# lukasino1214/soc_real_time_renderer

Hardware: AMD Instinct MI355X
Metric: frames/sec + ms/pass, Sponza 3840x2160 deferred+SSAO+TAA (higher is better)
Workload: dtype f32 (fp16/unorm8/d32 storage)

## Files before the change

### soc_real_time_renderer_amd/csrc/bloom.hip

```cpp
#include <cstdlib>
#include <type_traits>

#include "bloom_common.hpp"

namespace soc {

namespace {

__global__ __launch_bounds__(kWorkgroup) void bloom_down_generic(DImg src, DImg dst, float sxt, float syt) {
    const int x = blockIdx.x * BX + threadIdx.x, y = blockIdx.y * BY + threadIdx.y;
    if (x >= dst.w || y >= dst.h) return;
    const float u = centre_uv(x, dst.w), v = centre_uv(y, dst.h);
    const float X = sxt, Y = syt;
    auto S = [&](float uu, float vv) {
        return tap(src, axis_from_fixed(fixed_from_uv(uu, src.w), src.w), axis_from_fixed(fixed_from_uv(vv, src.h), src.h));
    };
    f3 a = S(u - 2 * X, v + 2 * Y), b = S(u, v + 2 * Y), c = S(u + 2 * X, v + 2 * Y);
    f3 d = S(u - 2 * X, v), e = S(u, v), f = S(u + 2 * X, v);
    f3 g = S(u - 2 * X, v - 2 * Y), h = S(u, v - 2 * Y), i = S(u + 2 * X, v - 2 * Y);
    f3 j = S(u - X, v + Y), k = S(u + X, v + Y), l = S(u - X, v - Y), m = S(u + X, v - Y);
    store_rgb1(dst, x, y, SOC_DOWN13(a, b, c, d, e, f, g, h, i, j, k, l, m));
}

__global__ __launch_bounds__(kWorkgroup) void bloom_up_generic(DImg src, DImg dst, float X, float Y) {
    const int x = blockIdx.x * BX + threadIdx.x, y = blockIdx.y * BY + threadIdx.y;
    if (x >= dst.w || y >= dst.h) return;
    const float u = centre_uv(x, dst.w), v = centre_uv(y, dst.h);
    auto S = [&](float uu, float vv) {
        return tap(src, axis_from_fixed(fixed_from_uv(uu, src.w), src.w), axis_from_fixed(fixed_from_uv(vv, src.h), src.h));
    };
    f3 a = S(u - X, v + Y), b = S(u, v + Y), c = S(u + X, v + Y);
    f3 d = S(u - X, v), e = S(u, v), f = S(u + X, v);
    f3 g = S(u - X, v - Y), h = S(u, v - Y), i = S(u + X, v - Y);
    store_rgb1(dst, x, y, SOC_UP9(a, b, c, d, e, f, g, h, i));
}

__global__ __launch_bounds__(kWorkgroup) void bloom_up_double(DImg src, DImg dst) {
    const int x = blockIdx.x * BX + threadIdx.x, y = blockIdx.y * BY + threadIdx.y;
    if (x >= dst.w || y >= dst.h) return;
    auto AX = [&](int k) { return axis_from_fixed(128 * x - 64 + 256 * k, src.w); };
    auto AY = [&](int k) { return axis_from_fixed(128 * y - 64 + 256 * k, src.h); };
    const Axis xm = AX(-1), x0 = AX(0), xp = AX(1), ym = AY(-1), y0 = AY(0), yp = AY(1);
    f3 a = tap(src, xm, yp), b = tap(src, x0, yp), c = tap(src, xp, yp);
    f3 d = tap(src, xm, y0), e = tap(src, x0, y0), f = tap(src, xp, y0);
    f3 g = tap(src, xm, ym), h = tap(src, x0, ym), i = tap(src, xp, ym);
    store_rgb1(dst, x, y, SOC_UP9(a, b, c, d, e, f, g, h, i));
}

__global__ __launch_bounds__(kWorkgroup) void bloom_down_same_q(DImg src, DImg dst, bool vec) {
    const int m = blockIdx.x * BX + threadIdx.x, n = blockIdx.y * BY + threadIdx.y;
    const int X0 = 2 * m, Y0 = 2 * n;
    if (X0 >= dst.w || Y0 >= dst.h) return;
    uint2 T[6][6];
#pragma unroll
    for (int r = 0; r < 6; ++r)
#pragma unroll
        for (int c = 0; c < 6; ++c) T[r][c] = texel_clamped(src, X0 - 2 + c, Y0 - 2 + r);
    float out[2][2][3];
    auto run = [&](auto CH) {
        constexpr int C = decltype(CH)::value;
        float V[6][6];
#pragma unroll
        for (int r = 0; r < 6; ++r)
#pragma unroll
            for (int c = 0; c < 6; ++c) V[r][c] = chan<C>(T[r][c]);
#pragma unroll
        for (int py = 0; py < 2; ++py)
#pragma unroll
            for (int px = 0; px < 2; ++px) {
                auto P = [&](int ox, int oy) { return V[oy + 2 + py][ox + 2 + px]; };
                out[py][px][C] = down13(P(-2, 2), P(0, 2), P(2, 2), P(-2, 0), P(0, 0), P(2, 0), P(-2, -2), P(0, -2),
                                        P(2, -2), P(-1, 1), P(1, 1), P(-1, -1), P(1, -1));
            }
    };
    run(std::integral_constant<int, 0>{});
    run(std::integral_constant<int, 1>{});
    run(std::integral_constant<int, 2>{});
    store_quad_row(dst, X0, Y0, out[0], vec);
    store_quad_row(dst, X0, Y0 + 1, out[1], vec);
}

__global__ __launch_bounds__(kWorkgroup) void bloom_up_same_q(DImg src, DImg dst, bool vec) {
    const int m = blockIdx.x * BX + threadIdx.x, n = blockIdx.y * BY + threadIdx.y;
    const int X0 = 2 * m, Y0 = 2 * n;
    if (X0 >= dst.w || Y0 >= dst.h) return;
    uint2 T[4][4];
#pragma unroll
    for (int r = 0; r < 4; ++r)
#pragma unroll
        for (int c = 0; c < 4; ++c) T[r][c] = texel_clamped(src, X0 - 1 + c, Y0 - 1 + r);
    float out[2][2][3];
    auto run = [&](auto CH) {
        constexpr int C = decltype(CH)::value;
#pragma unroll
        for (int py = 0; py < 2; ++py)
#pragma unroll
            for (int px = 0; px < 2; ++px) {
                auto P = [&](int ox, int oy) { return chan<C>(T[oy + 1 + py][ox + 1 + px]); };
                out[py][px][C] = up9(P(-1, 1), P(0, 1), P(1, 1), P(-1, 0), P(0, 0), P(1, 0), P(-1, -1), P(0, -1), P(1, -1));
            }
    };
    run(std::integral_constant<int, 0>{});
    run(std::integral_constant<int, 1>{});
    run(std::integral_constant<int, 2>{});
    store_quad_row(dst, X0, Y0, out[0], vec);
    store_quad_row(dst, X0, Y0 + 1, out[1], vec);
}

__global__ __launch_bounds__(kWorkgroup) void bloom_down_half_w(DImg src, DImg dst) {
    const int x = blockIdx.x * BX + threadIdx.x, y = blockIdx.y * BY + threadIdx.y;
    if (x >= dst.w || y >= dst.h) return;
    const bool interior = 2 * x - 2 >= 0 && 2 * x + 3 <= src.w - 1 && 2 * y - 2 >= 0 && 2 * y + 3 <= src.h - 1;
    if (!interior) {
        auto AX = [&](int k) { return axis_from_fixed(256 * (2 * x + k) + 128, src.w); };
        auto AY = [&](int k) { return axis_from_fixed(256 * (2 * y + k) + 128, src.h); };
        const Axis xm2 = AX(-2), xm1 = AX(-1), x0 = AX(0), xp1 = AX(1), xp2 = AX(2);
        const Axis ym2 = AY(-2), ym1 = AY(-1), y0 = AY(0), yp1 = AY(1), yp2 = AY(2);
        f3 a = tap(src, xm2, yp2), b = tap(src, x0, yp2), c = tap(src, xp2, yp2);
        f3 d = tap(src, xm2, y0), e = tap(src, x0, y0), f = tap(src, xp2, y0);
        f3 g = tap(src, xm2, ym2), h = tap(src, x0, ym2), i = tap(src, xp2, ym2);
        f3 j = tap(src, xm1, yp1), k = tap(src, xp1, yp1), l = tap(src, xm1, ym1), m = tap(src, xp1, ym1);
        store_rgb1(dst, x, y, SOC_DOWN13(a, b, c, d, e, f, g, h, i, j, k, l, m));
        return;
    }
    uint2 T[6][6];
    const uint2* base = row_ptr<uint2>(src, 2 * y - 2) + (2 * x - 2);
    const int pitch8 = src.pitch / 8;
#pragma unroll
    for (int r = 0; r < 6; ++r)
#pragma unroll
        for (int c = 0; c < 6; ++c) T[r][c] = base[r * pitch8 + c];
    float out[3];
    auto run = [&](auto CH) {
        constexpr int C = decltype(CH)::value;
        float Hl[6][5];
#pragma unroll
        for (int r = 0; r < 6; ++r)
#pragma unroll
            for (int k = 0; k < 5; ++k) Hl[r][k] = lerp_c(chan<C>(T[r][k]), chan<C>(T[r][k + 1]), 0.5f);
        auto S = [&](int kx, int ky) { return lerp_c(Hl[ky + 2][kx + 2], Hl[ky + 3][kx + 2], 0.5f); };
        out[C] = down13(S(-2, 2), S(0, 2), S(2, 2), S(-2, 0), S(0, 0), S(2, 0), S(-2, -2), S(0, -2), S(2, -2), S(-1, 1),
                        S(1, 1), S(-1, -1), S(1, -1));
    };
    run(std::integral_constant<int, 0>{});
    run(std::integral_constant<int, 1>{});
    run(std::integral_constant<int, 2>{});
    store_rgb1_c(dst, x, y, out[0], out[1], out[2]);
}

__global__ __launch_bounds__(kWorkgroup) void bloom_up_double_q(DImg src, DImg dst, bool vec) {
    const int m = blockIdx.x * BX + threadIdx.x, n = blockIdx.y * BY + threadIdx.y;
    if (m >= src.w || n >= src.h) return;
    const int X0 = 2 * m, Y0 = 2 * n;
    const bool interior = m - 2 >= 0 && m + 2 <= src.w - 1 && n - 2 >= 0 && n + 2 <= src.h - 1;
    if (!interior) {
#pragma unroll 1
        for (int k = 0; k < 4; ++k) {
                const int px = k & 1, py = k >> 1;
                const int x = X0 + px, y = Y0 + py;
                auto AX = [&](int k) { return axis_from_fixed(128 * x - 64 + 256 * k, src.w); };
                auto AY = [&](int k) { return axis_from_fixed(128 * y - 64 + 256 * k, src.h); };
                const Axis xm = AX(-1), x0 = AX(0), xp = AX(1), ym = AY(-1), y0 = AY(0), yp = AY(1);
                f3 a = tap(src, xm, yp), b = tap(src, x0, yp), c = tap(src, xp, yp);
                f3 d = tap(src, xm, y0), e = tap(src, x0, y0), f = tap(src, xp, y0);
                f3 g = tap(src, xm, ym), h = tap(src, x0, ym), i = tap(src, xp, ym);
                store_rgb1(dst, x, y, SOC_UP9(a, b, c, d, e, f, g, h, i));
            }
        return;
    }
    uint2 T[5][5];
    const uint2* base = row_ptr<uint2>(src, n - 2) + (m - 2);
    const int pitch8 = src.pitch / 8;
#pragma unroll
    for (int r = 0; r < 5; ++r)
#pragma unroll
        for (int c = 0; c < 5; ++c) T[r][c] = base[r * pitch8 + c];
    float out[2][2][3];
    auto run = [&](auto CH) {
        constexpr int C = decltype(CH)::value;
        float V[5][5];
#pragma unroll
        for (int r = 0; r < 5; ++r)
#pragma unroll
            for (int c = 0; c < 5; ++c) V[r][c] = chan<C>(T[r][c]);
        float H0[5][3], H1[5][3];
#pragma unroll
        for (int r = 0; r < 5; ++r)
#pragma unroll
            for (int k = 0; k < 3; ++k) {
                H0[r][k] = t_w34(V[r][k], V[r][k + 1]);
                H1[r][k] = t_w14(V[r][k + 1], V[r][k + 2]);
            }
#pragma unroll
        for (int px = 0; px < 2; ++px) {
            const float (&Hl)[5][3] = px ? H1 : H0;
            float S0[3][3], S1[3][3];
#pragma unroll
            for (int ky = -1; ky <= 1; ++ky)
#pragma unroll
                for (int kx = -1; kx <= 1; ++kx) {
                    const float p = v_prod(Hl[ky + 2][kx + 1]);
                    S0[ky + 1][kx + 1] = __builtin_fmaf(Hl[ky + 1][kx + 1], 0.0625f, p);
                    S1[ky + 1][kx + 1] = __builtin_fmaf(Hl[ky + 3][kx + 1], 0.0625f, p);
                }
            out[0][px][C] = up9(S0[2][0], S0[2][1], S0[2][2], S0[1][0], S0[1][1], S0[1][2], S0[0][0], S0[0][1], S0[0][2]);
            out[1][px][C] = up9(S1[2][0], S1[2][1], S1[2][2], S1[1][0], S1[1][1], S1[1][2], S1[0][0], S1[0][1], S1[0][2]);
        }
        __builtin_amdgcn_sched_barrier(0);
    };
    run(std::integral_constant<int, 0>{});
    run(std::integral_constant<int, 1>{});
    run(std::integral_constant<int, 2>{});
    store_quad_row(dst, X0, Y0, out[0], vec);
    store_quad_row(dst, X0, Y0 + 1, out[1], vec);
}

constexpr int kFastMax = 8192;

long quad_min_px() {
    static const long v = [] {
        const char* e = getenv("SOC_BLOOM_QUAD_MIN_PX");
        return e ? atol(e) : 1L << 20;
    }();
    return v;
}

bool vec16(const soc_img& im) { return im.pitch_bytes % 16 == 0 && reinterpret_cast<uintptr_t>(im.data) % 16 == 0; }

}

int launch_bloom_down(const soc_img& hi, const soc_img& lo, hipStream_t s, int force_generic) {
    dim3 blk(BX, BY), grd(ceil_div(lo.width, BX), ceil_div(lo.height, BY));
    DImg src = dimg(hi), dst = dimg(lo);
    const bool small = hi.width <= kFastMax && hi.height <= kFastMax;
    if (!force_generic && small && hi.width == lo.width && hi.height == lo.height) {
        dim3 g2(ceil_div(ceil_div(lo.width, 2), BX), ceil_div(ceil_div(lo.height, 2), BY));
        launch("bloom_down_same_q", kWorkgroup, bloom_down_same_q, g2, blk, 0, s, src, dst, vec16(lo));
    } else if (!force_generic && small && hi.width == 2 * lo.width && hi.height == 2 * lo.height) {
        launch("bloom_down_half_w", kWorkgroup, bloom_down_half_w, grd, blk, 0, s, src, dst);
    } else {
        launch("bloom_down_generic", kWorkgroup, bloom_down_generic, grd, blk, 0, s, src, dst, 1.0f / (float)hi.width, 1.0f / (float)hi.height);
    }
    return check_launch("bloom_downsample");
}

int launch_bloom_up(const soc_img& lo, const soc_img& hi, hipStream_t s, int force_generic) {
    dim3 blk(BX, BY), grd(ceil_div(hi.width, BX), ceil_div(hi.height, BY));
    DImg src = dimg(lo), dst = dimg(hi);
    const bool small = hi.width <= kFastMax && hi.height <= kFastMax;
    if (!force_generic && small && hi.width == lo.width && hi.height == lo.height) {
        dim3 g2(ceil_div(ceil_div(hi.width, 2), BX), ceil_div(ceil_div(hi.height, 2), BY));
        launch("bloom_up_same_q", kWorkgroup, bloom_up_same_q, g2, blk, 0, s, src, dst, vec16(hi));
    } else if (!force_generic && small && hi.width == 2 * lo.width && hi.height == 2 * lo.height) {
        if ((long)hi.width * hi.height < quad_min_px()) {
            launch("bloom_up_double", kWorkgroup, bloom_up_double, grd, blk, 0, s, src, dst);
        } else {
            dim3 g2(ceil_div(lo.width, BX), ceil_div(lo.height, BY));
            launch("bloom_up_double_q", kWorkgroup, bloom_up_double_q, g2, blk, 0, s, src, dst, vec16(hi));
        }
    } else {
        launch("bloom_up_generic", kWorkgroup, bloom_up_generic, grd, blk, 0, s, src, dst, 1.0f / (float)lo.width, 1.0f / (float)lo.height);
    }
    return check_launch("bloom_upsample");
}

}

using namespace soc;

static int bloom_args(const soc_img& a, const soc_img& b, const char* pass) {
    int rc = check_img(a, SOC_FMT_RGBA16F, pass, "source");
    if (rc) return rc;
    rc = check_img(b, SOC_FMT_RGBA16F, pass, "target");
    if (rc) return rc;
    if (a.data == b.data) return set_error(SOC_E_INVALID_ARG, "%s: source and target alias", pass);
    return SOC_OK;
}

extern "C" int soc_bloom_downsample(const soc_globals* g, soc_img higher_mip, soc_img lower_mip, soc_stream stream) {
    (void)g;
    int rc = bloom_args(higher_mip, lower_mip, "soc_bloom_downsample");
    if (rc) return rc;
    return launch_bloom_down(higher_mip, lower_mip, hs(stream), 0);
}

extern "C" int soc_bloom_upsample(const soc_globals* g, soc_img lower_mip, soc_img higher_mip, soc_stream stream) {
    (void)g;
    int rc = bloom_args(lower_mip, higher_mip, "soc_bloom_upsample");
    if (rc) return rc;
    return launch_bloom_up(lower_mip, higher_mip, hs(stream), 0);
}

extern "C" int soc_debug_bloom_generic(int32_t up, soc_img a, soc_img b, soc_stream stream) {
    int rc = bloom_args(a, b, "soc_debug_bloom_generic");
    if (rc) return rc;
    return up ? launch_bloom_up(a, b, hs(stream), 1) : launch_bloom_down(a, b, hs(stream), 1);
}

extern "C" int soc_bloom_weighted_stage(const soc_globals* g, soc_img emissive, const soc_img* mips, int32_t mip_count,
                                        soc_img output, int32_t stage, soc_stream stream) {
    (void)g;
    static const char* P = "soc_bloom_weighted_stage";
    if (!mips) return set_error(SOC_E_INVALID_ARG, "%s: null mips", P);
    if (stage < 0 || stage > 4) return set_error(SOC_E_INVALID_ARG, "%s: stage %d not in 0..4", P, stage);
    int rc = check_img(emissive, SOC_FMT_RGBA16F, P, "emissive");
    if (!rc) rc = check_img(output, SOC_FMT_RGBA16F, P, "output");
    for (int i = 0; !rc && i < mip_count; ++i) rc = check_img(mips[i], SOC_FMT_RGBA16F, P, "mip");
    if (rc) return rc;
    if (!bloom_fused_applicable(emissive, mips, mip_count, output))
        return set_error(SOC_E_UNSUPPORTED, "%s: needs 4 mips halving exactly from the emissive extent (<= 8192)", P);
    if ((stage == 0 || stage == 4) && output.data == mips[1].data)
        return set_error(SOC_E_INVALID_ARG, "%s: output aliases mip 1", P);
    return launch_bloom_weighted(emissive, mips, output, hs(stream), stage);
}

extern "C" int soc_bloom_chain(const soc_globals* g, soc_img emissive, const soc_img* mips, int32_t mip_count,
                               soc_stream stream) {
    if (!mips || mip_count < 1) return set_error(SOC_E_INVALID_ARG, "soc_bloom_chain: need >= 1 mip");
    int rc = soc_bloom_downsample(g, emissive, mips[0], stream);
    for (int i = 0; !rc && i < mip_count - 1; ++i) rc = soc_bloom_downsample(g, mips[i], mips[i + 1], stream);
    for (int i = mip_count - 1; !rc && i > 0; --i) rc = soc_bloom_upsample(g, mips[i], mips[i - 1], stream);
    if (!rc) rc = soc_bloom_upsample(g, mips[0], emissive, stream);
    return rc;
}
```

### soc_real_time_renderer_amd/csrc/bloom_w.hip

```cpp
#include "bloom_w.hpp"

namespace soc {
bool bloom_fused_applicable(const soc_img& emissive, const soc_img* mips, int mip_count, const soc_img& output) {
    if (mip_count != 4 || output.width != emissive.width || output.height != emissive.height) return false;
    if (emissive.width > 8192 || emissive.height > 8192) return false;
    if (mips[0].width != emissive.width || mips[0].height != emissive.height) return false;
    for (int i = 1; i < 4; ++i)
        if (mips[i - 1].width != 2 * mips[i].width || mips[i - 1].height != 2 * mips[i].height || mips[i].width < 2 ||
            mips[i].height < 2)
            return false;
    return true;
}
}

namespace soc {
namespace {

__device__ __forceinline__ void store2(const DImg& im, int x, int y, uint2 a, uint2 b, bool vec) {
    uint2* row = row_ptr_w<uint2>(im, y);
    if (vec && x + 1 < im.w) {
        *reinterpret_cast<uint4*>(row + x) = uint4{a.x, a.y, b.x, b.y};
        return;
    }
    row[x] = a;
    if (x + 1 < im.w) row[x + 1] = b;
}

template <int TW>
__device__ __forceinline__ C3 down11(const uint2 (*t)[TW], int cx, int cy) {
    C3 a{0.0f, 0.0f, 0.0f};
    madd(a, t[cy][cx], 0.125f);
    madd(a, t[cy - 2][cx - 2], 0.03125f);
    madd(a, t[cy - 2][cx + 2], 0.03125f);
    madd(a, t[cy + 2][cx - 2], 0.03125f);
    madd(a, t[cy + 2][cx + 2], 0.03125f);
    madd(a, t[cy - 2][cx], 0.0625f);
    madd(a, t[cy][cx - 2], 0.0625f);
    madd(a, t[cy][cx + 2], 0.0625f);
    madd(a, t[cy + 2][cx], 0.0625f);
    madd(a, t[cy - 1][cx - 1], 0.125f);
    madd(a, t[cy - 1][cx + 1], 0.125f);
    madd(a, t[cy + 1][cx - 1], 0.125f);
    madd(a, t[cy + 1][cx + 1], 0.125f);
    return a;
}

__device__ __forceinline__ constexpr float d21_w(int i, int j) {
    constexpr int A[6] = {1, 1, 2, 2, 1, 1}, B[6] = {0, 1, 1, 1, 1, 0};
    return (float)(A[i] * A[j] + 4 * B[i] * B[j]) * (1.0f / 128.0f);
}
template <int TW>
__device__ __forceinline__ C3 down21(const uint2 (*t)[TW], int c0, int r0) {
    C3 a{0.0f, 0.0f, 0.0f};
#pragma unroll
    for (int j = 0; j < 6; ++j)
#pragma unroll
        for (int i = 0; i < 6; ++i) madd(a, t[r0 + j][c0 + i], d21_w(i, j));
    return a;
}

template <int TW>
__device__ __forceinline__ void up12_pair(const uint2 (*t)[TW], int c0, int r0, int py, C3& even, C3& odd) {
    even = C3{0.0f, 0.0f, 0.0f};
    odd = C3{0.0f, 0.0f, 0.0f};
#pragma unroll
    for (int j = 0; j < 4; ++j) {
        const float wy = u12_w(py, j);
#pragma unroll
        for (int i = 0; i < 5; ++i) {
            const uint2 v = t[r0 + j][c0 + i];
            if (i < 4) madd(even, v, u12_w(0, i) * wy);
            if (i > 0) madd(odd, v, u12_w(1, i - 1) * wy);
        }
    }
}

template <int TW>
__device__ __forceinline__ void up11_pair(const uint2 (*t)[TW], int cx, int cy, C3& a, C3& b) {
    a = C3{0.0f, 0.0f, 0.0f};
    b = C3{0.0f, 0.0f, 0.0f};
    constexpr float w[3] = {1.0f, 2.0f, 1.0f};
#pragma unroll
    for (int j = 0; j < 3; ++j)
#pragma unroll
        for (int i = 0; i < 4; ++i) {
            const uint2 v = t[cy - 1 + j][cx - 1 + i];
            if (i < 3) madd(a, v, w[i] * w[j] * (1.0f / 16.0f));
            if (i > 0) madd(b, v, w[i - 1] * w[j] * (1.0f / 16.0f));
        }
}

template <int MODE>
struct W1 {
    static constexpr int OW = MODE ? 30 : 32, OH = MODE == 2 ? 16 : 8;
    static constexpr int MW = 2 * OW + 4, MH = 2 * OH + 4;
    static constexpr int EW = MW + 4, EH = MH + 4;
    static constexpr int RUN = MH / 4;
    static_assert(!MODE || (MW == 64 && MH % 4 == 0), "down11_runs: 64 columns x 2 row parities x 2 runs");
};

template <int TW, int MW, int RUN>
__device__ __forceinline__ void down11_runs(const uint2 (*t)[TW], uint2 (*mt)[MW], int c, int r, int cx) {
    uint2 e0[3], o1[2], e2[3], o3[2], e4[3];
    const int cy0 = r + 2;
    auto even = [&](int y, uint2 (&e)[3]) { e[0] = t[y][cx - 2]; e[1] = t[y][cx]; e[2] = t[y][cx + 2]; };
    auto odd = [&](int y, uint2 (&o)[2]) { o[0] = t[y][cx - 1]; o[1] = t[y][cx + 1]; };
    even(cy0 - 2, e0);
    odd(cy0 - 1, o1);
    even(cy0, e2);
    odd(cy0 + 1, o3);
    even(cy0 + 2, e4);
#pragma unroll
    for (int j = 0; j < RUN; ++j) {
        C3 a{0.0f, 0.0f, 0.0f};
        madd(a, e2[1], 0.125f);
        madd(a, e0[0], 0.03125f);
        madd(a, e0[2], 0.03125f);
        madd(a, e4[0], 0.03125f);
        madd(a, e4[2], 0.03125f);
        madd(a, e0[1], 0.0625f);
        madd(a, e2[0], 0.0625f);
        madd(a, e2[2], 0.0625f);
        madd(a, e4[1], 0.0625f);
        madd(a, o1[0], 0.125f);
        madd(a, o1[1], 0.125f);
        madd(a, o3[0], 0.125f);
        madd(a, o3[1], 0.125f);
        mt[r + 2 * j][c] = pack3(a);
        if (j < RUN - 1) {
#pragma unroll
            for (int k = 0; k < 3; ++k) {
                e0[k] = e2[k];
                e2[k] = e4[k];
            }
            o1[0] = o3[0];
            o1[1] = o3[1];
            const int cy = cy0 + 2 * (j + 1);
            odd(cy + 1, o3);
            even(cy + 2, e4);
        }
    }
}

template <int TW>
__device__ __forceinline__ void down21_vpair(const uint2 (*t)[TW], int c0, int r0, C3& a, C3& b) {
    a = C3{0.0f, 0.0f, 0.0f};
    b = C3{0.0f, 0.0f, 0.0f};
#pragma unroll
    for (int j = 0; j < 8; ++j) {
        uint2 v[6];
#pragma unroll
        for (int i = 0; i < 6; ++i) v[i] = t[r0 + j][c0 + i];
#pragma unroll
        for (int i = 0; i < 6; ++i) {
            if (j < 6) madd(a, v[i], d21_w(i, j));
            if (j >= 2) madd(b, v[i], d21_w(i, j - 2));
        }
        asm volatile("" : "+v"(a.r), "+v"(a.g), "+v"(a.b), "+v"(b.r), "+v"(b.g), "+v"(b.b)::"memory");
    }
}

template <int MODE, bool ZS>
__global__ __launch_bounds__(kWorkgroup) void bloomw_down01p(DImg E, DImg M1, int ntx, int nty) {
    constexpr int W1_OW = W1<MODE>::OW, W1_OH = W1<MODE>::OH, W1_MW = W1<MODE>::MW, W1_MH = W1<MODE>::MH,
                  W1_EW = W1<MODE>::EW, W1_EH = W1<MODE>::EH, RUN = W1<MODE>::RUN;
    static_assert(kWorkgroup == 256, "four waves: one vote word each");
    __shared__ uint2 et[W1_EH][W1_EW];
    __shared__ uint2 mt[W1_MH][W1_MW];
    __shared__ uint4 zv[2];
    constexpr int NT = W1_EW * W1_EH, KR = (NT + 255) / 256;
    const int tid = threadIdx.x, n = ntx * nty, G = (int)gridDim.x;
    int er[KR], ec[KR];
#pragma unroll
    for (int k = 0; k < KR; ++k) {
        const int i = tid + 256 * k;
        er[k] = i / W1_EW;
        ec[k] = i - er[k] * W1_EW;
    }
    auto tile_origin = [&](int t, int& X0, int& Y0) {
        const int q = n >> 3, r = n & 7, k = t & 7;
        const int id = k * q + min(k, r) + (t >> 3);
        const int ty = id / ntx;
        X0 = (id - ty * ntx) * W1_OW;
        Y0 = ty * W1_OH;
    };
    uint2 v[KR];
    auto fetch = [&](int t) {
        int X0, Y0;
        tile_origin(t, X0, Y0);
        const int ex0 = 2 * X0 - 4, ey0 = 2 * Y0 - 4;
#pragma unroll
        for (int k = 0; k < KR; ++k)
            if (tid + 256 * k < NT)
                v[k] = row_ptr<uint2>(E, clampi(ey0 + er[k], 0, E.h - 1))[clampi(ex0 + ec[k], 0, E.w - 1)];
    };
    auto vote = [&](int slot) {
        uint32_t nz = 0u;
#pragma unroll
        for (int k = 0; k < KR; ++k)
            if (tid + 256 * k < NT) nz |= v[k].x | (v[k].y & 0xffffu);
        const bool any = __ballot(nz != 0u) != 0ull;
        if ((tid & 63) == 0) reinterpret_cast<uint32_t*>(&zv[slot])[tid >> 6] = any ? 1u : 0u;
    };
    auto voted = [&](int slot) {
        const uint4 z = zv[slot];
        return __builtin_amdgcn_readfirstlane((int)(z.x | z.y | z.z | z.w)) == 0;
    };
    int t = (int)blockIdx.x;
    int slot = 0;
    const uint2 zpx = pack3(C3{0.0f, 0.0f, 0.0f});
    if (t < n) fetch(t);
    for (; t < n; t += G) {
#pragma unroll
        for (int k = 0; k < KR; ++k)
            if (tid + 256 * k < NT) et[er[k]][ec[k]] = v[k];
        if constexpr (ZS) vote(slot);
        __syncthreads();
        if (t + G < n) fetch(t + G);
        int X0, Y0;
        tile_origin(t, X0, Y0);
        if constexpr (ZS) {
            const bool zero = voted(slot);
            slot ^= 1;
            if (zero) {
                if constexpr (MODE == 2) {
                    if (tid < W1_OW * W1_OH / 2) {
                        const int q = tid / W1_OW, ox = tid - q * W1_OW;
                        const int X = X0 + ox, Y = Y0 + 2 * q;
                        if (X < M1.w && Y < M1.h) row_ptr_w<uint2>(M1, Y)[X] = zpx;
                        if (X < M1.w && Y + 1 < M1.h) row_ptr_w<uint2>(M1, Y + 1)[X] = zpx;
                    }
                } else {
                    const int oy = tid / W1_OW, ox = tid - oy * W1_OW;
                    const int X = X0 + ox, Y = Y0 + oy;
                    if (oy < W1_OH && X < M1.w && Y < M1.h) row_ptr_w<uint2>(M1, Y)[X] = zpx;
                }
                continue;
            }
        }
        const int mx0 = 2 * X0 - 2, my0 = 2 * Y0 - 2, ex0 = mx0 - 2, ey0 = my0 - 2;
        if (MODE && my0 >= 0 && my0 + W1_MH <= E.h) {
            const int c = tid & 63, par = (tid >> 6) & 1, half = tid >> 7;
            if constexpr (MODE != 0)
                down11_runs<W1_EW, W1_MW, RUN>(et, mt, c, par + 2 * RUN * half, clampi(mx0 + c, 0, E.w - 1) - ex0);
        } else
        for (int i = tid; i < W1_MW * W1_MH; i += 256) {
            const int r = i / W1_MW, c = i - r * W1_MW;
            const int cx = clampi(mx0 + c, 0, E.w - 1) - ex0, cy = clampi(my0 + r, 0, E.h - 1) - ey0;
            mt[r][c] = pack3(down11<W1_EW>(et, cx, cy));
        }
        __syncthreads();
        if constexpr (MODE == 2) {
            if (tid < W1_OW * W1_OH / 2) {
                const int q = tid / W1_OW, ox = tid - q * W1_OW;
                const int X = X0 + ox, Y = Y0 + 2 * q;
                C3 a, b;
                down21_vpair<W1_MW>(mt, 2 * ox, 4 * q, a, b);
                if (X < M1.w && Y < M1.h) row_ptr_w<uint2>(M1, Y)[X] = pack3(a);
                if (X < M1.w && Y + 1 < M1.h) row_ptr_w<uint2>(M1, Y + 1)[X] = pack3(b);
            }
        } else {
            const int oy = tid / W1_OW, ox = tid - oy * W1_OW;
            const int X = X0 + ox, Y = Y0 + oy;
            if (oy < W1_OH && X < M1.w && Y < M1.h) row_ptr_w<uint2>(M1, Y)[X] = pack3(down21<W1_MW>(mt, 2 * ox, 2 * oy));
        }
        __syncthreads();
    }
}

constexpr int W2_OW = 16, W2_OH = 8;
constexpr int W2_MW = 2 * W2_OW + 4, W2_MH = 2 * W2_OH + 4;
constexpr int W2_SW = 2 * W2_MW + 4, W2_SH = 2 * W2_MH + 4;

template <int TW, int MW, int K>
__device__ __forceinline__ void down21_runs(const uint2 (*t)[TW], uint2 (*mt)[MW], int c, int r0, int n, int sc) {
    C3 acc[K];
#pragma unroll
    for (int e = 0; e < K; ++e) acc[e] = C3{0.0f, 0.0f, 0.0f};
#pragma unroll
    for (int R = 0; R < 6 + 2 * (K - 1); ++R) {
        if (R >= 6 + 2 * (n - 1)) continue;
        uint2 v[6];
#pragma unroll
        for (int i = 0; i < 6; ++i) v[i] = t[2 * r0 + R][sc + i];
#pragma unroll
        for (int e = 0; e < K; ++e) {
            const int j = R - 2 * e;
            if (j >= 0 && j < 6) {
#pragma unroll
                for (int i = 0; i < 6; ++i) madd(acc[e], v[i], d21_w(i, j));
            }
        }
#pragma unroll
        for (int e = 0; e < K; ++e) asm volatile("" : "+v"(acc[e].r), "+v"(acc[e].g), "+v"(acc[e].b)::"memory");
    }
#pragma unroll
    for (int e = 0; e < K; ++e)
        if (e < n) mt[r0 + e][c] = pack3(acc[e]);
}

template <bool REG>
__global__ __launch_bounds__(kWorkgroup) void bloomw_down23(DImg S1, DImg M3, int W2, int H2, int swz) {
    __shared__ uint2 st[W2_SH][W2_SW];
    __shared__ uint2 mt[W2_MH][W2_MW];
    const int tid = threadIdx.x;
    int tbx, tby;
    xcd_order(swz, tbx, tby);
    const int X0 = tbx * W2_OW, Y0 = tby * W2_OH;
    const int mx0 = 2 * X0 - 2, my0 = 2 * Y0 - 2, sx0 = 2 * mx0 - 2, sy0 = 2 * my0 - 2;
    load_tile<W2_SW, W2_SH>(S1, sx0, sy0, st, tid);
    __syncthreads();
    constexpr int K = 3, NR = (W2_MH + K - 1) / K;
    static_assert(W2_MW * NR <= 256, "one run per lane");
    if (REG && my0 >= 0 && my0 + W2_MH <= H2) {
        if (tid < W2_MW * NR) {
            const int c = tid % W2_MW, k = tid / W2_MW, r0 = k * K;
            const int qx = clampi(mx0 + c, 0, W2 - 1);
            down21_runs<W2_SW, W2_MW, K>(st, mt, c, r0, min(K, W2_MH - r0), 2 * qx - 2 - sx0);
        }
    } else
    for (int i = tid; i < W2_MW * W2_MH; i += 256) {
        const int r = i / W2_MW, c = i - r * W2_MW;
        const int qx = clampi(mx0 + c, 0, W2 - 1), qy = clampi(my0 + r, 0, H2 - 1);
        mt[r][c] = pack3(down21<W2_SW>(st, 2 * qx - 2 - sx0, 2 * qy - 2 - sy0));
    }
    __syncthreads();
    if (tid < W2_OW * W2_OH) {
        const int ox = tid % W2_OW, oy = tid / W2_OW;
        const int X = X0 + ox, Y = Y0 + oy;
        if (X < M3.w && Y < M3.h) row_ptr_w<uint2>(M3, Y)[X] = pack3(down21<W2_MW>(mt, 2 * ox, 2 * oy));
    }
}

constexpr int U_OW = 64, U_OH = 16;
constexpr int W3_MW = U_OW / 2 + 4, W3_MH = U_OH / 2 + 4;
constexpr int W3_SW = W3_MW / 2 + 4, W3_SH = W3_MH / 2 + 4;

template <int SW, int MW>
__device__ __forceinline__ void up12_into(const uint2 (*s)[SW], int sx0, int sy0, uint2 (*m)[MW], int c, int r, int qx, int qy,
                                          int Wq, int Hq) {
    const int cy = clampi(qy, 0, Hq - 1), py = cy & 1;
    const int q0 = clampi(qx, 0, Wq - 1), q1 = clampi(qx + 1, 0, Wq - 1);
    const int r0 = (cy >> 1) - 2 + py - sy0;
    if ((q0 & 1) == 0 && q1 == q0 + 1) {
        C3 e, o;
        up12_pair<SW>(s, (q0 >> 1) - 2 - sx0, r0, py, e, o);
        m[r][c] = pack3(e);
        m[r][c + 1] = pack3(o);
    } else {
#pragma unroll
        for (int k = 0; k < 2; ++k) {
            const int q = k ? q1 : q0;
            C3 e, o;
            up12_pair<SW>(s, ((q & ~1) >> 1) - 2 - sx0, r0, py, e, o);
            m[r][c + k] = pack3((q & 1) ? o : e);
        }
    }
}

__global__ __launch_bounds__(kWorkgroup) void bloomw_up32(DImg S3, DImg M1, int W2, int H2, bool vec, int swz) {
    __shared__ uint2 st[W3_SH][W3_SW];
    __shared__ uint2 mt[W3_MH][W3_MW];
    const int tid = threadIdx.x;
    int tbx, tby;
    xcd_order(swz, tbx, tby);
    const int X0 = tbx * U_OW, Y0 = tby * U_OH;
    const int mx0 = X0 / 2 - 2, my0 = Y0 / 2 - 2;
    const int sx0 = mx0 / 2 - 2, sy0 = my0 / 2 - 2;
    load_tile<W3_SW, W3_SH>(S3, sx0, sy0, st, tid);
    __syncthreads();
    for (int i = tid; i < (W3_MW / 2) * W3_MH; i += 256) {
        const int r = i / (W3_MW / 2), c = 2 * (i - r * (W3_MW / 2));
        up12_into<W3_SW, W3_MW>(st, sx0, sy0, mt, c, r, mx0 + c, my0 + r, W2, H2);
    }
    __syncthreads();
    for (int i = tid; i < (U_OW / 2) * U_OH; i += 256) {
        const int r = i / (U_OW / 2), pc = i - r * (U_OW / 2);
        const int x = X0 + 2 * pc, y = Y0 + r;
        if (x >= M1.w || y >= M1.h) continue;
        const int py = y & 1;
        C3 e, o;
        up12_pair<W3_MW>(mt, (x >> 1) - 2 - mx0, (y >> 1) - 2 + py - my0, py, e, o);
        store2(M1, x, y, pack3(e), pack3(o), vec);
    }
}

struct P3u {
    float r[W3_MH][U_OW], g[W3_MH][U_OW], b[W3_MH][U_OW];
};
template <bool RUNS>
__global__ __launch_bounds__(kWorkgroup) void bloomw_up32s(DImg S3, DImg M1, int W2, int H2, bool vec, int swz) {
    __shared__ uint2 st[W3_SH][W3_SW];
    __shared__ uint2 mt[W3_MH][W3_MW];
    __shared__ P3u hp;
    const int tid = threadIdx.x;
    int tbx, tby;
    xcd_order(swz, tbx, tby);
    const int X0 = tbx * U_OW, Y0 = tby * U_OH;
    const int mx0 = X0 / 2 - 2, my0 = Y0 / 2 - 2;
    const int sx0 = mx0 / 2 - 2, sy0 = my0 / 2 - 2;
    load_tile<W3_SW, W3_SH>(S3, sx0, sy0, st, tid);
    __syncthreads();
    for (int i = tid; i < W3_SH * W3_MW; i += 256) {
        const int sr = i / W3_MW, c = i - sr * W3_MW;
        const int q = clampi(mx0 + c, 0, W2 - 1), px = q & 1, c0 = (q >> 1) - 2 + px - sx0;
        C3 a{0.0f, 0.0f, 0.0f};
#pragma unroll
        for (int k = 0; k < 4; ++k) madd(a, st[sr][c0 + k], u12_w(px, k));
        hp.r[sr][c] = a.r;
        hp.g[sr][c] = a.g;
        hp.b[sr][c] = a.b;
    }
    __syncthreads();
    for (int i = tid; i < W3_MH * W3_MW; i += 256) {
        const int r = i / W3_MW, c = i - r * W3_MW;
        const int cy = clampi(my0 + r, 0, H2 - 1), py = cy & 1, r0 = (cy >> 1) - 2 + py - sy0;
        C3 a{0.0f, 0.0f, 0.0f};
#pragma unroll
        for (int k = 0; k < 4; ++k) {
            const float w = u12_w(py, k);
            a.r = __builtin_fmaf(hp.r[r0 + k][c], w, a.r);
            a.g = __builtin_fmaf(hp.g[r0 + k][c], w, a.g);
            a.b = __builtin_fmaf(hp.b[r0 + k][c], w, a.b);
        }
        mt[r][c] = pack3(a);
    }
    __syncthreads();
    for (int i = tid; i < W3_MH * U_OW; i += 256) {
        const int r = i / U_OW, ox = i - r * U_OW;
        const int x = X0 + ox, px = x & 1, c0 = (x >> 1) - 2 + px - mx0;
        C3 a{0.0f, 0.0f, 0.0f};
#pragma unroll
        for (int k = 0; k < 4; ++k) madd(a, mt[r][c0 + k], u12_w(px, k));
        hp.r[r][ox] = a.r;
        hp.g[r][ox] = a.g;
        hp.b[r][ox] = a.b;
    }
    __syncthreads();
    if constexpr (RUNS) {
        static_assert(U_OW == 64 && U_OH == 16, "64 columns x 4 runs of 4 output rows");
        const int ox = tid & 63, m = tid >> 6, x = X0 + ox;
        float hr[6], hg[6], hb[6];
#pragma unroll
        for (int k = 0; k < 6; ++k) {
            hr[k] = hp.r[2 * m + k][ox];
            hg[k] = hp.g[2 * m + k][ox];
            hb[k] = hp.b[2 * m + k][ox];
        }
#pragma unroll
        for (int i = 0; i < 4; ++i) {
            const int y = Y0 + 4 * m + i, py = i & 1, rr = (i >> 1) + (i & 1);
            C3 a{0.0f, 0.0f, 0.0f};
#pragma unroll
            for (int j = 0; j < 4; ++j) {
                const float w = u12_w(py, j);
                a.r = __builtin_fmaf(hr[rr + j], w, a.r);
                a.g = __builtin_fmaf(hg[rr + j], w, a.g);
                a.b = __builtin_fmaf(hb[rr + j], w, a.b);
            }
            if (x < M1.w && y < M1.h) row_ptr_w<uint2>(M1, y)[x] = pack3(a);
        }
        return;
    }
    for (int i = tid; i < (U_OW / 2) * U_OH; i += 256) {
        const int r = i / (U_OW / 2), pc = i - r * (U_OW / 2);
        const int x = X0 + 2 * pc, y = Y0 + r;
        if (x >= M1.w || y >= M1.h) continue;
        const int py = y & 1, r0 = (y >> 1) - 2 + py - my0;
        C3 o[2];
#pragma unroll
        for (int k = 0; k < 2; ++k) {
            const int c = 2 * pc + k;
            C3 a{0.0f, 0.0f, 0.0f};
#pragma unroll
            for (int j = 0; j < 4; ++j) {
                const float w = u12_w(py, j);
                a.r = __builtin_fmaf(hp.r[r0 + j][c], w, a.r);
                a.g = __builtin_fmaf(hp.g[r0 + j][c], w, a.g);
                a.b = __builtin_fmaf(hp.b[r0 + j][c], w, a.b);
            }
            o[k] = a;
        }
        store2(M1, x, y, pack3(o[0]), pack3(o[1]), vec);
    }
}

constexpr int W4_MW = U_OW + 2, W4_MH = U_OH + 2;
constexpr int W4_SW = U_OW / 2 + 6, W4_SH = U_OH / 2 + 6;

__global__ __launch_bounds__(kWorkgroup) void bloomw_up10(DImg S1, DImg O, bool vec, int swz) {
    __shared__ uint2 st[W4_SH][W4_SW];
    __shared__ uint2 mt[W4_MH][W4_MW + 2];
    const int tid = threadIdx.x;
    int tbx, tby;
    xcd_order(swz, tbx, tby);
    const int X0 = tbx * U_OW, Y0 = tby * U_OH;
    const int mx0 = X0 - 1, my0 = Y0 - 1;
    const int sx0 = X0 / 2 - 3, sy0 = Y0 / 2 - 3;
    const int W0 = O.w, H0 = O.h;
    load_tile<W4_SW, W4_SH>(S1, sx0, sy0, st, tid);
    __syncthreads();
    for (int i = tid; i < (W4_MW / 2) * W4_MH; i += 256) {
        const int r = i / (W4_MW / 2), k = i - r * (W4_MW / 2);
        const int c = 2 * k + 1;
        up12_into<W4_SW, W4_MW + 2>(st, sx0, sy0, mt, c, r, mx0 + c, my0 + r, W0, H0);
    }
    for (int r = tid; r < W4_MH; r += 256) {
        const int cy = clampi(my0 + r, 0, H0 - 1), py = cy & 1;
        const int q = clampi(mx0, 0, W0 - 1);
        C3 e, o;
        up12_pair<W4_SW>(st, ((q & ~1) >> 1) - 2 - sx0, (cy >> 1) - 2 + py - sy0, py, e, o);
        mt[r][0] = pack3((q & 1) ? o : e);
    }
    __syncthreads();
    for (int i = tid; i < (U_OW / 2) * U_OH; i += 256) {
        const int r = i / (U_OW / 2), pc = i - r * (U_OW / 2);
        const int x = X0 + 2 * pc, y = Y0 + r;
        if (x >= O.w || y >= O.h) continue;
        C3 a, b;
        up11_pair<W4_MW + 2>(mt, x - mx0, y - my0, a, b);
        store2(O, x, y, pack3(a), pack3(b), vec);
    }
}

__global__ __launch_bounds__(kWorkgroup) void bloomw_up10s(DImg S1, DImg O, bool vec, int swz, bool zs) {
    __shared__ Up10Tile<U_OW, U_OH> t;
    const int tid = threadIdx.x;
    int tbx, tby;
    xcd_order(swz, tbx, tby);
    const int X0 = tbx * U_OW, Y0 = tby * U_OH;
    const bool zero = t.build(S1, X0, Y0, O.w, O.h, tid, zs);
    const uint2 zpx = pack3(C3{0.0f, 0.0f, 0.0f});
    for (int i = tid; i < (U_OW / 2) * U_OH; i += 256) {
        const int r = i / (U_OW / 2), pc = i - r * (U_OW / 2);
        const int x = X0 + 2 * pc, y = Y0 + r;
        if (x >= O.w || y >= O.h) continue;
        if (zero) {
            store2(O, x, y, zpx, zpx, vec);
            continue;
        }
        C3 o[2];
        t.out(r, 2 * pc, o);
        store2(O, x, y, pack3(o[0]), pack3(o[1]), vec);
    }
}

#ifndef SOC_BLOOM_UP10_ROWS
#define SOC_BLOOM_UP10_ROWS 16
#endif
constexpr int R_OW = 62, R_TH = SOC_BLOOM_UP10_ROWS;
__device__ __forceinline__ uint32_t up_from_left(uint32_t v) {
    return (uint32_t)__builtin_amdgcn_update_dpp(0, (int)v, 0x138, 0xf, 0xf, false);
}
__device__ __forceinline__ uint32_t up_from_right(uint32_t v) {
    return (uint32_t)__builtin_amdgcn_update_dpp(0, (int)v, 0x130, 0xf, 0xf, false);
}
template <bool ZS>
__global__ __launch_bounds__(kWorkgroup) void bloomw_up10r(DImg S1, DImg O, int nwx, int nwaves) {
    const int lane = (int)(threadIdx.x & 63);
    const int wid = (int)blockIdx.x * (kWorkgroup / 64) + (int)(threadIdx.x >> 6);
    if (wid >= nwaves) return;
    const int W0 = O.w, H0 = O.h, W1 = S1.w, H1 = S1.h;
    const int wx = wid % nwx, Y0 = (wid / nwx) * R_TH;
    const int x = wx * R_OW - 1 + lane;
    const int cx = clampi(x, 0, W0 - 1);
    const int px = cx & 1, c0 = (cx >> 1) - 2 + px;
    int tc[4];
    float wk[4];
#pragma unroll
    for (int k = 0; k < 4; ++k) {
        tc[k] = clampi(c0 + k, 0, W1 - 1);
        wk[k] = px ? u12_w(1, k) : u12_w(0, k);
    }
    auto taps = [&](int s, uint2 (&t)[4]) {
        const uint2* row = row_ptr<uint2>(S1, clampi(s, 0, H1 - 1));
#pragma unroll
        for (int k = 0; k < 4; ++k) t[k] = row[tc[k]];
    };
    auto h12 = [&](const uint2 (&t)[4]) {
        C3 a{0.0f, 0.0f, 0.0f};
#pragma unroll
        for (int k = 0; k < 4; ++k) madd(a, t[k], wk[k]);
        return a;
    };
    auto rgb_or = [&](const uint2 (&t)[4]) {
        return t[0].x | t[1].x | t[2].x | t[3].x | ((t[0].y | t[1].y | t[2].y | t[3].y) & 0xffffu);
    };
    C3 ring[5];
    uint2 pend[4];
    uint32_t nz = 0u;
    int base = (max(Y0 - 1, 0) >> 1) - 2;
#pragma unroll
    for (int i = 0; i < 5; ++i) {
        taps(base + i, pend);
        ring[i] = h12(pend);
        if constexpr (ZS) nz |= rgb_or(pend);
    }
    taps(base + 5, pend);
    auto hrow = [&](int cy) {
        const int jb = (cy >> 1) - 2;
        if (jb > base) {
#pragma unroll
            for (int i = 0; i < 4; ++i) ring[i] = ring[i + 1];
            ring[4] = h12(pend);
            base = jb;
            taps(base + 5, pend);
        }
        const int py = cy & 1;
        C3 a{0.0f, 0.0f, 0.0f};
#pragma unroll
        for (int k = 0; k < 4; ++k) {
            const float w = u12_w(py, k);
            const C3 h = py ? ring[k + 1] : ring[k];
            a.r = __builtin_fmaf(h.r, w, a.r);
            a.g = __builtin_fmaf(h.g, w, a.g);
            a.b = __builtin_fmaf(h.b, w, a.b);
        }
        const uint2 m = pack3(a);
        const uint2 l = uint2{up_from_left(m.x), up_from_left(m.y)}, r = uint2{up_from_right(m.x), up_from_right(m.y)};
        C3 hs{0.0f, 0.0f, 0.0f};
        madd(hs, l, 1.0f);
        madd(hs, m, 2.0f);
        madd(hs, r, 1.0f);
        return hs;
    };
    const bool out_lane = lane >= 1 && lane <= R_OW && x < W0;
    int y0 = Y0;
    if constexpr (ZS) {
        if (__ballot(nz != 0u) == 0ull) {
            const uint2 zpx = pack3(C3{0.0f, 0.0f, 0.0f});
            const int ns = min(Y0 + R_TH, H0) - Y0 + 2;
            int s = 0;
            for (; s < ns; ++s) {
                const int jb = (clampi(Y0 - 1 + s, 0, H0 - 1) >> 1) - 2;
                if (jb > base) {
                    if (__ballot(rgb_or(pend) != 0u) != 0ull) break;
                    base = jb;
                    taps(base + 5, pend);
                }
                if (s >= 2 && out_lane) row_ptr_w<uint2>(O, Y0 + s - 2)[x] = zpx;
            }
            y0 = Y0 + max(s - 2, 0);
        }
    }
    C3 hq0 = hrow(max(y0 - 1, 0)), hq1 = hrow(min(y0, H0 - 1));
    for (int y = y0; y < min(Y0 + R_TH, H0); ++y) {
        const C3 hq2 = hrow(min(y + 1, H0 - 1));
        C3 o;
        o.r = __builtin_fmaf(hq2.r, 1.0f / 16.0f, __builtin_fmaf(hq1.r, 2.0f / 16.0f, hq0.r * (1.0f / 16.0f)));
        o.g = __builtin_fmaf(hq2.g, 1.0f / 16.0f, __builtin_fmaf(hq1.g, 2.0f / 16.0f, hq0.g * (1.0f / 16.0f)));
        o.b = __builtin_fmaf(hq2.b, 1.0f / 16.0f, __builtin_fmaf(hq1.b, 2.0f / 16.0f, hq0.b * (1.0f / 16.0f)));
        if (out_lane) row_ptr_w<uint2>(O, y)[x] = pack3(o);
        hq0 = hq1;
        hq1 = hq2;
    }
}

template <int MODE, bool ZS>
int down01p_resident_set() {
    constexpr int kMaxDevices = 64;
    static int cached[kMaxDevices] = {};
    int dev = 0, cus = 256, per = 0;
    (void)hipGetDevice(&dev);
    if (dev >= 0 && dev < kMaxDevices && cached[dev]) return cached[dev];
    (void)hipDeviceGetAttribute(&cus, hipDeviceAttributeMultiprocessorCount, dev);
    (void)hipOccupancyMaxActiveBlocksPerMultiprocessor(&per, bloomw_down01p<MODE, ZS>, 256, 0);
    const int n = std::max(per, 1) * cus;
    if (dev >= 0 && dev < kMaxDevices) cached[dev] = n;
    return n;
}

bool a16(const soc_img& im) { return im.pitch_bytes % 16 == 0 && reinterpret_cast<uintptr_t>(im.data) % 16 == 0; }

}

int launch_bloom_weighted(const soc_img& emissive, const soc_img* mips, const soc_img& output, hipStream_t s, int stage) {
    const DImg E = dimg(emissive), M1 = dimg(mips[1]), M3 = dimg(mips[3]), O = dimg(output);
    const int swz = 1;
    const bool zero_skip = tuning_knob("SOC_BLOOM_ZERO_SKIP", 1) != 0;
    if (stage == 0 || stage == 1) {
        auto w1 = [&](auto mode, auto zs) {
            constexpr int R = decltype(mode)::value;
            constexpr bool Z = decltype(zs)::value;
            const int ntx = ceil_div(mips[1].width, W1<R>::OW), nty = ceil_div(mips[1].height, W1<R>::OH);
            const int grid = std::max(8, (std::min(ntx * nty, down01p_resident_set<R, Z>()) / 8) * 8);
            launch("bloomw_down01p", kWorkgroup, bloomw_down01p<R, Z>, grid, kWorkgroup, 0, s, E, M1, ntx, nty);
        };
        auto w1z = [&](auto mode) {
            if (zero_skip) w1(mode, std::true_type{});
            else w1(mode, std::false_type{});
        };
        const int mode = tuning_knob("SOC_BLOOM_W1_REG", 1);
        if (mode == 2) w1z(std::integral_constant<int, 2>{});
        else if (mode == 1) w1z(std::integral_constant<int, 1>{});
        else w1z(std::integral_constant<int, 0>{});
    }
    if (stage == 0 || stage == 2) {
        dim3 g(ceil_div(mips[3].width, W2_OW), ceil_div(mips[3].height, W2_OH));
        if (tuning_knob("SOC_BLOOM_W2_REG", 1))
            launch("bloomw_down23", kWorkgroup, bloomw_down23<true>, g, kWorkgroup, 0, s, M1, M3, mips[2].width, mips[2].height, swz);
        else
            launch("bloomw_down23", kWorkgroup, bloomw_down23<false>, g, kWorkgroup, 0, s, M1, M3, mips[2].width, mips[2].height, swz);
    }
    if (stage == 0 || stage == 3) {
        dim3 g(ceil_div(mips[1].width, U_OW), ceil_div(mips[1].height, U_OH));
        if (tuning_knob("SOC_BLOOM_UP_SEP", 1))
            if (tuning_knob("SOC_BLOOM_W3_RUNS", 1))
                launch("bloomw_up32s", kWorkgroup, bloomw_up32s<true>, g, kWorkgroup, 0, s, M3, M1, mips[2].width, mips[2].height, a16(mips[1]), swz);
            else
                launch("bloomw_up32s", kWorkgroup, bloomw_up32s<false>, g, kWorkgroup, 0, s, M3, M1, mips[2].width, mips[2].height, a16(mips[1]), swz);
        else
            launch("bloomw_up32", kWorkgroup, bloomw_up32, g, kWorkgroup, 0, s, M3, M1, mips[2].width, mips[2].height, a16(mips[1]), swz);
    }
    if (stage == 0 || stage == 4) {
        dim3 g(ceil_div(output.width, U_OW), ceil_div(output.height, U_OH));
        if (tuning_knob("SOC_BLOOM_UP10_REG", 1)) {
            const int nwx = ceil_div(output.width, R_OW), nwaves = nwx * ceil_div(output.height, R_TH);
            if (zero_skip)
                launch("bloomw_up10r", kWorkgroup, bloomw_up10r<true>, ceil_div(nwaves, kWorkgroup / 64), kWorkgroup, 0, s, M1, O, nwx, nwaves);
            else
                launch("bloomw_up10r", kWorkgroup, bloomw_up10r<false>, ceil_div(nwaves, kWorkgroup / 64), kWorkgroup, 0, s, M1, O, nwx, nwaves);
        } else if (tuning_knob("SOC_BLOOM_UP_SEP", 1))
            launch("bloomw_up10s", kWorkgroup, bloomw_up10s, g, kWorkgroup, 0, s, M1, O, a16(output), swz, zero_skip);
        else
            launch("bloomw_up10", kWorkgroup, bloomw_up10, g, kWorkgroup, 0, s, M1, O, a16(output), swz);
    }
    return check_launch("bloom_weighted");
}

}
```

### soc_real_time_renderer_amd/csrc/bloom_w.hpp

```cpp
#pragma once

#include "soc_internal.hpp"

namespace soc {
namespace {

__device__ __forceinline__ int clampi(int v, int lo, int hi) { return min(max(v, lo), hi); }

struct C3 {
    float r, g, b;
};
__device__ __forceinline__ float lo16(uint32_t u) { return (float)__builtin_bit_cast(_Float16, (uint16_t)(u & 0xffffu)); }
__device__ __forceinline__ float hi16(uint32_t u) { return (float)__builtin_bit_cast(_Float16, (uint16_t)(u >> 16)); }
__device__ __forceinline__ void madd(C3& a, uint2 t, float w) {
    a.r = __builtin_fmaf(lo16(t.x), w, a.r);
    a.g = __builtin_fmaf(hi16(t.x), w, a.g);
    a.b = __builtin_fmaf(lo16(t.y), w, a.b);
}
__device__ __forceinline__ uint2 pack3(const C3& c) { return pack_h4(f4{c.r, c.g, c.b, 1.0f}); }

template <int TW, int TH>
__device__ __forceinline__ uint32_t load_tile(const DImg& im, int ox, int oy, uint2 (*t)[TW], int tid) {
    constexpr int N = TW * TH;
    auto at = [&](int i) {
        const int r = i / TW, c = i - r * TW;
        return row_ptr<uint2>(im, clampi(oy + r, 0, im.h - 1)) + clampi(ox + c, 0, im.w - 1);
    };
    uint32_t nz = 0u;
    for (int i0 = tid; i0 < N; i0 += 4 * 256) {
        const int i1 = i0 + 256, i2 = i1 + 256, i3 = i2 + 256;
        const uint2 a = *at(i0);
        uint2 b = uint2{0u, 0u}, c = b, d = b;
        if (i1 < N) b = *at(i1);
        if (i2 < N) c = *at(i2);
        if (i3 < N) d = *at(i3);
        t[i0 / TW][i0 % TW] = a;
        if (i1 < N) t[i1 / TW][i1 % TW] = b;
        if (i2 < N) t[i2 / TW][i2 % TW] = c;
        if (i3 < N) t[i3 / TW][i3 % TW] = d;
        nz |= a.x | b.x | c.x | d.x | ((a.y | b.y | c.y | d.y) & 0xffffu);
    }
    return nz;
}

__device__ __forceinline__ constexpr float u12_w(int parity, int k) {
    constexpr int E[4] = {1, 5, 7, 3}, O[4] = {3, 7, 5, 1};
    return (float)(parity ? O[k] : E[k]) * (1.0f / 16.0f);
}

template <int OW, int OH>
struct Up10Tile {
    static constexpr int MW = OW + 2, MH = OH + 2;
    static constexpr int SW = OW / 2 + 6, SH = OH / 2 + 6;
    static constexpr int HR = SH > MH ? SH : MH;
    union {
        uint2 st[SH][SW];
        uint2 mt[MH][MW];
    };
    float hr[HR][MW], hg[HR][MW], hb[HR][MW];
    uint32_t zv[4];

    __device__ __forceinline__ bool build(const DImg& S1, int X0, int Y0, int W0, int H0, int tid, bool zs) {
        const int mx0 = X0 - 1, my0 = Y0 - 1;
        const int sx0 = X0 / 2 - 3, sy0 = Y0 / 2 - 3;
        const uint32_t nz = load_tile<SW, SH>(S1, sx0, sy0, st, tid);
        if (zs) {
            const bool any = __ballot(nz != 0u) != 0ull;
            if ((tid & 63) == 0) zv[tid >> 6] = any ? 1u : 0u;
        }
        __syncthreads();
        if (zs && __builtin_amdgcn_readfirstlane((int)(zv[0] | zv[1] | zv[2] | zv[3])) == 0) return true;
        for (int i = tid; i < SH * MW; i += 256) {
            const int sr = i / MW, c = i - sr * MW;
            const int q = clampi(mx0 + c, 0, W0 - 1), px = q & 1, c0 = (q >> 1) - 2 + px - sx0;
            C3 a{0.0f, 0.0f, 0.0f};
#pragma unroll
            for (int k = 0; k < 4; ++k) madd(a, st[sr][c0 + k], u12_w(px, k));
            hr[sr][c] = a.r;
            hg[sr][c] = a.g;
            hb[sr][c] = a.b;
        }
        __syncthreads();
        for (int i = tid; i < MH * MW; i += 256) {
            const int r = i / MW, c = i - r * MW;
            const int cy = clampi(my0 + r, 0, H0 - 1), py = cy & 1, r0 = (cy >> 1) - 2 + py - sy0;
            C3 a{0.0f, 0.0f, 0.0f};
#pragma unroll
            for (int k = 0; k < 4; ++k) {
                const float w = u12_w(py, k);
                a.r = __builtin_fmaf(hr[r0 + k][c], w, a.r);
                a.g = __builtin_fmaf(hg[r0 + k][c], w, a.g);
                a.b = __builtin_fmaf(hb[r0 + k][c], w, a.b);
            }
            mt[r][c] = pack3(a);
        }
        __syncthreads();
        for (int i = tid; i < MH * OW; i += 256) {
            const int r = i / OW, c = i - r * OW;
            C3 a{0.0f, 0.0f, 0.0f};
            madd(a, mt[r][c], 1.0f);
            madd(a, mt[r][c + 1], 2.0f);
            madd(a, mt[r][c + 2], 1.0f);
            hr[r][c] = a.r;
            hg[r][c] = a.g;
            hb[r][c] = a.b;
        }
        __syncthreads();
        return false;
    }
    __device__ __forceinline__ void out(int r, int c, C3 (&o)[2]) const {
#pragma unroll
        for (int k = 0; k < 2; ++k) {
            const int cc = c + k;
            o[k].r = __builtin_fmaf(hr[r + 2][cc], 1.0f / 16.0f, __builtin_fmaf(hr[r + 1][cc], 2.0f / 16.0f, hr[r][cc] * (1.0f / 16.0f)));
            o[k].g = __builtin_fmaf(hg[r + 2][cc], 1.0f / 16.0f, __builtin_fmaf(hg[r + 1][cc], 2.0f / 16.0f, hg[r][cc] * (1.0f / 16.0f)));
            o[k].b = __builtin_fmaf(hb[r + 2][cc], 1.0f / 16.0f, __builtin_fmaf(hb[r + 1][cc], 2.0f / 16.0f, hb[r][cc] * (1.0f / 16.0f)));
        }
    }
};

}
}
```

### soc_real_time_renderer_amd/csrc/capi.cpp

```cpp
#include <hip/hip_runtime.h>

#include <cmath>
#include <cstdarg>
#include <cstdlib>
#include <cstdio>
#include <cstring>
#include <functional>
#include <string>
#include <mutex>
#include <vector>

#include "soc_internal.hpp"

namespace soc {

static thread_local std::string t_error;

int set_error(int code, const char* fmt, ...) {
    char buf[512];
    va_list ap;
    va_start(ap, fmt);
    vsnprintf(buf, sizeof buf, fmt, ap);
    va_end(ap);
    t_error = buf;
// ... 302 lines not shown
    const float Vec3[4] = {m(1, 3), m(0, 3), m(0, 3), m(0, 3)};
    float Inv[4][4];
    for (int i = 0; i < 4; ++i) {
        Inv[0][i] = Vec1[i] * Fac0[i] - Vec2[i] * Fac1[i] + Vec3[i] * Fac2[i];
        Inv[1][i] = Vec0[i] * Fac0[i] - Vec2[i] * Fac3[i] + Vec3[i] * Fac4[i];
        Inv[2][i] = Vec0[i] * Fac1[i] - Vec1[i] * Fac3[i] + Vec3[i] * Fac5[i];
        Inv[3][i] = Vec0[i] * Fac2[i] - Vec1[i] * Fac4[i] + Vec2[i] * Fac5[i];
    }
    const float SignA[4] = {+1.0f, -1.0f, +1.0f, -1.0f}, SignB[4] = {-1.0f, +1.0f, -1.0f, +1.0f};
    float Inverse[4][4];
    for (int i = 0; i < 4; ++i) {
        Inverse[0][i] = Inv[0][i] * SignA[i];
        Inverse[1][i] = Inv[1][i] * SignB[i];
        Inverse[2][i] = Inv[2][i] * SignA[i];
        Inverse[3][i] = Inv[3][i] * SignB[i];
    }
    const float Row0[4] = {Inverse[0][0], Inverse[1][0], Inverse[2][0], Inverse[3][0]};
    const float Dot0[4] = {m(0, 0) * Row0[0], m(0, 1) * Row0[1], m(0, 2) * Row0[2], m(0, 3) * Row0[3]};
    const float Dot1 = (Dot0[0] + Dot0[1]) + (Dot0[2] + Dot0[3]);
    const float OneOverDeterminant = 1.0f / Dot1;
    for (int c = 0; c < 4; ++c)
        for (int r = 0; r < 4; ++r) out[c * 4 + r] = Inverse[c][r] * OneOverDeterminant;
#undef m
}

static inline float radians(float deg) { return deg * 0.01745329251994329576923690768489f; }

static V3h rotate_x(V3h v, float a) { float c = std::cos(a), s = std::sin(a); return V3h{v.x, v.y * c - v.z * s, v.y * s + v.z * c}; }
static V3h rotate_y(V3h v, float a) { float c = std::cos(a), s = std::sin(a); return V3h{v.x * c + v.z * s, v.y, -v.x * s + v.z * c}; }
static V3h rotate_z(V3h v, float a) { float c = std::cos(a), s = std::sin(a); return V3h{v.x * c - v.y * s, v.x * s + v.y * c, v.z}; }

extern "C" void soc_tuning_reload(void) {
    std::lock_guard<std::mutex> lock(g_knob_mu);
    g_knobs.clear();
}

extern "C" int soc_globals_init_defaults(soc_globals* g, int32_t width, int32_t height) {
    if (!g || width <= 0 || height <= 0) return set_error(SOC_E_INVALID_ARG, "soc_globals_init_defaults: bad args");
    std::memset(g, 0, sizeof *g);
    g->terrain_offset[0] = g->terrain_offset[1] = g->terrain_offset[2] = 0.0f;
    g->terrain_scale[0] = g->terrain_scale[1] = 100.0f;
    g->terrain_height_scale = 70.0f;
    g->terrain_midpoint = 0.2f;
    g->terrain_delta = 8.0f;
    g->terrain_min_depth = 1.0f;
    g->terrain_max_depth = 100.0f;
    g->terrain_min_tess_level = 1;
    g->terrain_max_tess_level = 3;
    g->ssao_bias = 0.025f;
    g->ssao_radius = 0.3f;
    g->ssao_kernel_size = 26;
    g->ambient[0] = g->ambient[1] = g->ambient[2] = 0.1f;
    g->ambient_occlussion_strength = 1.2f;
    g->emissive_bloom_strength = 2.0f;
    g->focal_length = 5.0f;
    g->plane_in_focus = 1.0f;
    g->aperture = 8.0f;
    g->adjustment_speed = 1.0f;
    g->log_min_luminance = -15.0f;
    g->log_max_luminance = 15.0f;
    g->target_luminance = 0.2140f;
    g->elapsed_time = 0.0f;
    g->log_min_luminance = std::log2(g->target_luminance / std::exp2(g->log_min_luminance));
    g->log_max_luminance = std::log2(g->target_luminance / std::exp2(g->log_max_luminance));
    g->saturation = 1.0f;
    g->agxDs_linear_section = 0.18f;
    g->peak = 1.0f;
    g->compression = 0.15f;
    g->frame_counter = 0;
    const V3h light_position{-3.2f, 40.0f, -4.0f};
    const float planes = 16.0f;
    float light_projection[16];
    soc_mat4_ortho_rh_no(light_projection, -planes, planes, -planes, planes, -planes, planes);
    V3h dir{0.0f, -1.0f, 0.0f};
    dir = rotate_x(dir, radians(4.0f));
    dir = rotate_y(dir, radians(0.0f));
    dir = rotate_z(dir, radians(0.0f));
    const float eye[3] = {light_position.x, light_position.y, light_position.z};
    const float center[3] = {light_position.x + dir.x, light_position.y + dir.y, light_position.z + dir.z};
    const float up[3] = {0.0f, -1.0f, 0.0f};
    float light_view[16], pv[16];
    soc_mat4_look_at_rh(light_view, eye, center, up);
    mat4_mul_host(pv, light_projection, light_view);
    std::memcpy(g->sun_info.projection_matrix, light_projection, sizeof light_projection);
    std::memcpy(g->sun_info.view_matrix, light_view, sizeof light_view);
    std::memcpy(g->sun_info.projection_view_matrix, pv, sizeof pv);
    for (int r = 0; r < 4; ++r) g->sun_info.terrain_y_clip_trick[r] = pv[1 * 4 + r];
    g->sun_info.position[0] = light_position.x; g->sun_info.position[1] = light_position.y; g->sun_info.position[2] = light_position.z;
    g->sun_info.direction[0] = dir.x; g->sun_info.direction[1] = dir.y; g->sun_info.direction[2] = dir.z;
    g->sun_info.exponential_factor = -80.0f;
    g->sun_info.darkening_factor = 1.0f;
    g->sun_info.bias = 0.0001f;
    g->sun_info.intensity = 1.0f;
    g->resolution[0] = width;
    g->resolution[1] = height;
    g->camera_near_clip = 0.1f;
    g->camera_far_clip = 1000.0f;
    return SOC_OK;
}

extern "C" int soc_globals_frame_update(soc_globals* g, const soc_camera* cam, int32_t width, int32_t height, float delta_time,
                                        uint32_t* jitter_index) {
    if (!g || !cam || !jitter_index || width <= 0 || height <= 0)
        return set_error(SOC_E_INVALID_ARG, "soc_globals_frame_update: bad args");
    float proj[16];
    const float aspect = (float)width / (float)height;
    soc_mat4_perspective_rh_no(proj, radians(cam->fov_degrees), aspect, cam->near_clip, cam->far_clip);
    proj[1 * 4 + 1] *= -1.0f;
    float ry = cam->rotation[1];
    const float MAX_ROT = 1.56825555556f;
    if (ry > MAX_ROT) ry = MAX_ROT;
    if (ry < -MAX_ROT) ry = -MAX_ROT;
    const float rx = cam->rotation[0];
    const V3h fwd = normalize(V3h{std::cos(rx) * std::cos(ry), -std::sin(ry), std::sin(rx) * std::cos(ry)});
    const float eye[3] = {cam->position[0], cam->position[1], cam->position[2]};
    const float center[3] = {eye[0] + fwd.x, eye[1] + fwd.y, eye[2] + fwd.z};
    const float up[3] = {0.0f, 1.0f, 0.0f};
    float view[16];
    soc_mat4_look_at_rh(view, eye, center, up);
    const float gr = 1.32471795724474602596f, a1 = 1.0f / gr, a2 = 1.0f / (gr * gr);
    auto gmod = [](float x, float y) { return x - y * std::floor(x / y); };
    const float idx = (float)(*jitter_index);
    float jx = gmod(0.5f + a1 * (idx + 1.0f), 1.0f) - 0.5f;
    float jy = gmod(0.5f + a2 * (idx + 1.0f), 1.0f) - 0.5f;
    jx = jx * (1.0f / (float)width);
    jy = jy * (1.0f / (float)height);
    *jitter_index = (*jitter_index + 1) % 32;
    proj[3 * 4 + 0] += jx;
    proj[3 * 4 + 1] += jy;
    float inv_proj[16], inv_view[16], pv[16], inv_pv[16];
    soc_mat4_inverse(inv_proj, proj);
    soc_mat4_inverse(inv_view, view);
    mat4_mul_host(pv, proj, view);
    mat4_mul_host(inv_pv, inv_proj, inv_view);
    std::memcpy(g->camera_previous_projection_matrix, g->camera_projection_matrix, 64);
    std::memcpy(g->camera_previous_inverse_projection_matrix, g->camera_inverse_projection_matrix, 64);
    std::memcpy(g->camera_previous_view_matrix, g->camera_view_matrix, 64);
    std::memcpy(g->camera_previous_inverse_view_matrix, g->camera_inverse_view_matrix, 64);
    std::memcpy(g->camera_previous_projection_view_matrix, g->camera_projection_view_matrix, 64);
    std::memcpy(g->camera_previous_inverse_projection_view_matrix, g->camera_inverse_projection_view_matrix, 64);
    std::memcpy(g->terrain_previous_y_clip_trick, g->terrain_y_clip_trick, 16);
    std::memcpy(g->previous_jitter, g->jitter, 8);
    std::memcpy(g->camera_projection_matrix, proj, 64);
    std::memcpy(g->camera_inverse_projection_matrix, inv_proj, 64);
    std::memcpy(g->camera_view_matrix, view, 64);
    std::memcpy(g->camera_inverse_view_matrix, inv_view, 64);
    std::memcpy(g->camera_projection_view_matrix, pv, 64);
    std::memcpy(g->camera_inverse_projection_view_matrix, inv_pv, 64);
    for (int r = 0; r < 4; ++r) g->terrain_y_clip_trick[r] = pv[1 * 4 + r];
    g->jitter[0] = jx;
    g->jitter[1] = jy;
    g->camera_near_clip = cam->near_clip;
    g->camera_far_clip = cam->far_clip;
    g->resolution[0] = width;
    g->resolution[1] = height;
    for (int i = 0; i < 3; ++i) g->camera_position[i] = cam->position[i];
    g->delta_time = delta_time;
    g->elapsed_time += delta_time;
    g->frame_counter++;
    return SOC_OK;
}

static void quat_euler_to_mat4(float out[16], const float euler_rad[3]) {
    const float cx = std::cos(euler_rad[0] * 0.5f), cy = std::cos(euler_rad[1] * 0.5f), cz = std::cos(euler_rad[2] * 0.5f);
    const float sx = std::sin(euler_rad[0] * 0.5f), sy = std::sin(euler_rad[1] * 0.5f), sz = std::sin(euler_rad[2] * 0.5f);
    const float w = cx * cy * cz + sx * sy * sz;
    const float x = sx * cy * cz - cx * sy * sz;
    const float y = cx * sy * cz + sx * cy * sz;
    const float z = cx * cy * sz - sx * sy * cz;
    const float qxx = x * x, qyy = y * y, qzz = z * z, qxz = x * z, qxy = x * y, qyz = y * z, qwx = w * x, qwy = w * y,
                qwz = w * z;
    ident(out);
    out[0 * 4 + 0] = 1.0f - 2.0f * (qyy + qzz);
    out[0 * 4 + 1] = 2.0f * (qxy + qwz);
    out[0 * 4 + 2] = 2.0f * (qxz - qwy);
    out[1 * 4 + 0] = 2.0f * (qxy - qwz);
    out[1 * 4 + 1] = 1.0f - 2.0f * (qxx + qzz);
    out[1 * 4 + 2] = 2.0f * (qyz + qwx);
    out[2 * 4 + 0] = 2.0f * (qxz + qwy);
    out[2 * 4 + 1] = 2.0f * (qyz - qwx);
    out[2 * 4 + 2] = 1.0f - 2.0f * (qxx + qyy);
}

extern "C" int soc_scene_update(soc_globals* g, const soc_entity* e, int32_t count, float* model_matrices,
                                float* normal_matrices) {
    if (!g || count < 0 || (count > 0 && !e)) return set_error(SOC_E_INVALID_ARG, "soc_scene_update: bad arguments");
    int np = 0, ns = 0;
    for (int i = 0; i < count; ++i) {
        np += (e[i].components & SOC_ENTITY_POINT_LIGHT) ? 1 : 0;
        ns += (e[i].components & SOC_ENTITY_SPOT_LIGHT) ? 1 : 0;
    }
    if (np > SOC_MAX_POINT_LIGHTS || ns > SOC_MAX_SPOT_LIGHTS)
        return set_error(SOC_E_SHAPE, "soc_scene_update: %d point / %d spot lights exceed %d / %d", np, ns,
                         SOC_MAX_POINT_LIGHTS, SOC_MAX_SPOT_LIGHTS);
    g->point_light_count = 0;
    g->spot_light_count = 0;
    for (int i = 0; i < count; ++i) {
        const soc_entity& t = e[i];
        if (model_matrices || normal_matrices) {
            float T[16], R[16], S[16], TR[16], M[16], inv[16];
            ident(T);
            T[12] = t.position[0];
            T[13] = t.position[1];
            T[14] = t.position[2];
            const float eul[3] = {radians(t.rotation[0]), radians(t.rotation[1]), radians(t.rotation[2])};
            quat_euler_to_mat4(R, eul);
            ident(S);
            S[0] = t.scale[0];
            S[5] = t.scale[1];
            S[10] = t.scale[2];
            mat4_mul_host(TR, T, R);
            mat4_mul_host(M, TR, S);
            if (model_matrices) std::memcpy(model_matrices + 16 * i, M, sizeof M);
            if (normal_matrices) {
                soc_mat4_inverse(inv, M);
                for (int c = 0; c < 4; ++c)
                    for (int r = 0; r < 4; ++r) normal_matrices[16 * i + c * 4 + r] = inv[r * 4 + c];
            }
        }
        if (t.components & SOC_ENTITY_POINT_LIGHT) {
            soc_point_light& L = g->point_lights[g->point_light_count++];
            for (int k = 0; k < 3; ++k) {
                L.position[k] = t.position[k];
                L.color[k] = t.color[k];
            }
            L.intensity = t.intensity;
        }
        if (t.components & SOC_ENTITY_SPOT_LIGHT) {
            V3h dir{0.0f, -1.0f, 0.0f};
            dir = rotate_x(dir, radians(t.rotation[0]));
            dir = rotate_y(dir, radians(t.rotation[1]));
            dir = rotate_z(dir, radians(t.rotation[2]));
            soc_spot_light& L = g->spot_lights[g->spot_light_count++];
            for (int k = 0; k < 3; ++k) {
                L.position[k] = t.position[k];
                L.color[k] = t.color[k];
            }
            L.direction[0] = dir.x;
            L.direction[1] = dir.y;
            L.direction[2] = dir.z;
            L.intensity = t.intensity;
            L.cut_off = std::cos(radians(t.cut_off));
            L.outer_cut_off = std::cos(radians(t.outer_cut_off));
        }
    }
    return SOC_OK;
}

extern "C" int soc_upload_globals(const soc_globals* g, soc_globals* d_globals, soc_stream stream) {
    if (!g || !d_globals) return set_error(SOC_E_INVALID_ARG, "soc_upload_globals: null argument");
    hipError_t e = hipMemcpyAsync(d_globals, g, sizeof(soc_globals), hipMemcpyHostToDevice, hs(stream));
    if (e != hipSuccess) return set_error(SOC_E_HIP, "soc_upload_globals: %s", hipGetErrorString(e));
    return SOC_OK;
}

struct soc_renderer {
    using PassFn = std::function<int(const soc_globals*, hipStream_t)>;
    struct Pass {
        std::string name, group;
        int phase = SOC_PHASE_PRE_EXPOSURE;
        uint64_t reads = 0, writes = 0;
        uint32_t flags = 0;
        PassFn run;
        std::function<bool()> skip;
        std::vector<int> deps;
        std::vector<int> carry;
        bool signal = false;
        bool timed = false;
        std::vector<hipEvent_t> ev0, ev1;
        int next = 0, count = 0, last = -1;
        hipEvent_t done = nullptr;
        bool done_recorded = false;
    };
    struct UserPass {
        soc_pass_desc desc;
        std::string name, group, before;
        soc_pass_callback fn = nullptr;
        void* user = nullptr;
        bool ssr = false, before_prefix = false;
        soc_img ssr_mr{}, ssr_target{}, ssr_steps{};
    };
    soc_frame_images img{};
    soc_raster_scene scene{};
    bool has_scene = false;
    std::vector<Pass> passes;
    std::vector<UserPass> user_passes;
    uint32_t flags = 0;
    int hist = 0;
    uint64_t total_pixels = 0;
    int wide = 0;
    soc_globals* staging = nullptr;
    hipEvent_t staging_ev[4] = {nullptr, nullptr, nullptr, nullptr};
    int staging_slot = 0;
    bool async = true;
    int side_device = -1;
    hipStream_t side = nullptr;
    hipEvent_t fork_ev = nullptr, join_ev = nullptr;
    hipStream_t lane_q[2] = {nullptr, nullptr};
    int side_queue = -1;
    int probe_frames = 0;
    hipEvent_t probe_ev[16] = {};
    hipEvent_t switch_ev = nullptr;
    uint32_t* hist_scratch = nullptr;
    void* shadow_ws = nullptr;
    size_t shadow_ws_bytes = 0;
    bool fold_in_resolve = false;
    bool sky_split = false, sky_split_active = false;
    bool bloom_in_comp = false;
    bool bloom_in_comp_ok = false;
    bool main_after_side = true;
    bool inputs_ordered = false;
    soc::CloudState clouds_state;
};

namespace {
using PassFn = soc_renderer::PassFn;

uint64_t res_mask(std::initializer_list<int> ids) {
    uint64_t m = 0;
    for (int i : ids) m |= 1ull << i;
    return m;
}

uint64_t widen_velocity(const soc_renderer* r, uint64_t m) {
    const uint64_t both = (1ull << SOC_RES_VELOCITY) | (1ull << SOC_RES_PREVIOUS_VELOCITY);
    return (r->flags & SOC_RENDERER_VELOCITY_SLOTS) && (m & both) ? m | both : m;
}

soc_img frame_velocity(const soc_renderer* r) {
    return (r->flags & SOC_RENDERER_VELOCITY_SLOTS) ? r->img.history_velocity[1 - r->hist] : r->img.velocity;
}

bool sky_lane_high(const soc_renderer* r) {
    return r->side_queue == 1 || (r->side_queue == -1 && r->lane_q[0] && r->side == r->lane_q[0]);
}
bool bloom_in_comp_active(const soc_renderer* r) {
    return r->bloom_in_comp && r->bloom_in_comp_ok && (sky_lane_high(r) || tuning_knob("SOC_RENDERER_BLOOM_IN_COMP_ANY_LANE", 0));
}

soc_renderer::Pass& add_pass(soc_renderer* r, std::string name, std::string group, int phase, uint64_t reads,
                             uint64_t writes, PassFn fn, uint32_t flags = 0) {
    soc_renderer::Pass p;
    p.name = std::move(name);
    p.group = std::move(group);
    p.phase = phase;
    p.reads = widen_velocity(r, reads);
    p.writes = widen_velocity(r, writes);
    p.flags = flags;
    p.run = std::move(fn);
    r->passes.push_back(std::move(p));
    return r->passes.back();
}

int ensure_hist_scratch(soc_renderer* r, hipStream_t s) {
    if (r->hist_scratch) return SOC_OK;
    if (hipMalloc((void**)&r->hist_scratch, SOC_HISTOGRAM_SCRATCH_WORDS * sizeof(uint32_t)) != hipSuccess) {
        r->hist_scratch = nullptr;
        return set_error(SOC_E_HIP, "soc_renderer_execute: histogram scratch allocation failed");
    }
    if (hipMemsetAsync(r->hist_scratch, 0, SOC_HISTOGRAM_SCRATCH_WORDS * sizeof(uint32_t), s) != hipSuccess)
        return set_error(SOC_E_HIP, "soc_renderer_execute: histogram scratch clear failed");
    return SOC_OK;
}

void build_raster_passes(soc_renderer* r) {
    if (!r->has_scene) return;
    const int pre = SOC_PHASE_PRE_EXPOSURE;
    add_pass(r, "DepthPrepass", "Depth Prepass", pre, 0, res_mask({SOC_RES_VISIBILITY}),
             [r](const soc_globals* g, hipStream_t s) {
                 const soc_img& d = r->img.depth;
                 return soc_raster_visibility(&r->scene.mesh, g->camera_projection_view_matrix, SOC_CULL_FRONT,
                                              r->scene.visibility, d.width, d.height, 1, r->scene.workspace, (soc_stream)s);
             });
    const bool shadow_lane = r->shadow_ws && tuning_knob("SOC_RENDERER_SHADOW_LANE", 1);
    if (r->scene.shadow)
        add_pass(r, "SunShadowDraw", "Shadows", pre, 0, res_mask({SOC_RES_SUN_SHADOW}),
                 [r, shadow_lane](const soc_globals* g, hipStream_t s) {
                     return soc_raster_depth(&r->scene.mesh, g->sun_info.projection_view_matrix, SOC_CULL_BACK, 1.25f,
                                             1.75f, r->img.shadow, shadow_lane ? r->shadow_ws : r->scene.workspace,
                                             (soc_stream)s);
                 }, shadow_lane ? SOC_PASS_ASYNC : 0);
    add_pass(r, "GBufferGeneration", "Rendering G-Buffer", pre, res_mask({SOC_RES_VISIBILITY}),
             res_mask({SOC_RES_ALBEDO, SOC_RES_EMISSIVE, SOC_RES_NORMAL, SOC_RES_VELOCITY, SOC_RES_DEPTH}),
             [r](const soc_globals* g, hipStream_t s) {
                 const soc_frame_images& I = r->img;
                 return soc_gbuffer_resolve(g, &r->scene.mesh, r->scene.materials, r->scene.material_count,
                                            r->scene.visibility, I.depth, I.albedo, I.emissive, I.normal,
                                            frame_velocity(r), r->scene.workspace, (soc_stream)s);
             });
}

void build_passes(soc_renderer* r) {
    auto& I = r->img;
    const int pre = SOC_PHASE_PRE_EXPOSURE;
    const int nm = 4;
    const soc_img& bloom_dst = I.bloom_output.data ? I.bloom_output : I.emissive;
    const int dst_res = I.bloom_output.data ? SOC_RES_BLOOM_OUTPUT : SOC_RES_EMISSIVE;
    const int mip[4] = {SOC_RES_BLOOM_MIP0, SOC_RES_BLOOM_MIP1, SOC_RES_BLOOM_MIP2, SOC_RES_BLOOM_MIP3};
    const bool chain_ok = bloom_fused_applicable(I.emissive, I.bloom_mips, nm, bloom_dst);
    r->bloom_in_comp = false;
    if (chain_ok && !(r->flags & (SOC_RENDERER_EXACT_BLOOM | SOC_RENDERER_UNFUSED_BLOOM))) {
        static const char* names[4] = {"BloomDownsample - 0+1", "BloomDownsample - 2+3", "BloomUpsample - 3+2",
                                       "BloomUpsample - 1+0"};
        const uint64_t rd[4] = {res_mask({SOC_RES_EMISSIVE}), res_mask({mip[1]}), res_mask({mip[3]}), res_mask({mip[1]})};
        const uint64_t wr[4] = {res_mask({mip[1]}), res_mask({mip[3]}), res_mask({mip[1]}), res_mask({dst_res})};
        soc_globals gres{};
        gres.resolution[0] = I.color.width;
        gres.resolution[1] = I.color.height;
        r->bloom_in_comp = (r->flags & SOC_RENDERER_BLOOM_IN_COMPOSITION) && !(r->flags & SOC_RENDERER_UNFUSED_HISTOGRAM) &&
                           soc::composition_pair_applicable(&gres, I.color, I.albedo, bloom_dst, I.normal, I.depth, I.clouds);
        for (int st = 1; st <= 4; ++st)
            add_pass(r, names[st - 1], "Bloom", pre, rd[st - 1], wr[st - 1], [r, st](const soc_globals* g, hipStream_t s) {
                if (st == 4 && bloom_in_comp_active(r)) return (int)SOC_OK;
                const soc_img& dst = r->img.bloom_output.data ? r->img.bloom_output : r->img.emissive;
                return soc_bloom_weighted_stage(g, r->img.emissive, r->img.bloom_mips, 4, dst, st, (soc_stream)s);
            });
        return;
    }
    add_pass(r, "BloomDownsample - 0", "Bloom", pre, res_mask({SOC_RES_EMISSIVE}), res_mask({mip[0]}),
             [r](const soc_globals* g, hipStream_t s) {
                 return soc_bloom_downsample(g, r->img.emissive, r->img.bloom_mips[0], (soc_stream)s);
             });
    for (int i = 0; i < nm - 1; ++i)
        add_pass(r, "BloomDownsample - " + std::to_string(i + 1), "Bloom", pre, res_mask({mip[i]}),
                 res_mask({mip[i + 1]}), [r, i](const soc_globals* g, hipStream_t s) {
                     return soc_bloom_downsample(g, r->img.bloom_mips[i], r->img.bloom_mips[i + 1], (soc_stream)s);
                 });
    for (int i = nm - 1; i > 0; --i)
        add_pass(r, "BloomUpsample - " + std::to_string(i), "Bloom", pre, res_mask({mip[i]}), res_mask({mip[i - 1]}),
                 [r, i](const soc_globals* g, hipStream_t s) {
                     return soc_bloom_upsample(g, r->img.bloom_mips[i], r->img.bloom_mips[i - 1], (soc_stream)s);
                 });
    add_pass(r, "BloomUpsample - 0", "Bloom", pre, res_mask({mip[0]}), res_mask({dst_res}),
             [r](const soc_globals* g, hipStream_t s) {
                 const soc_img& dst = r->img.bloom_output.data ? r->img.bloom_output : r->img.emissive;
                 return soc_bloom_upsample(g, r->img.bloom_mips[0], dst, (soc_stream)s);
             });
}

void build_passes_tail(soc_renderer* r) {
    auto& I = r->img;
    const int pre = SOC_PHASE_PRE_EXPOSURE, post = SOC_PHASE_POST_EXPOSURE;
    const int em_res = I.bloom_output.data ? SOC_RES_BLOOM_OUTPUT : SOC_RES_EMISSIVE;
    add_pass(r, "SSAOGeneration", "Ambient Occlusion", pre, res_mask({SOC_RES_DEPTH, SOC_RES_NORMAL}),
             res_mask({SOC_RES_SSAO}), [r](const soc_globals* g, hipStream_t s) {
                 return soc_ssao_generation(g, r->img.depth, r->img.normal, r->img.ssao, r->img.ssao_noise_table,
                                            (soc_stream)s);
             });
    add_pass(r, "SSAOBlur", "Ambient Occlusion", pre, res_mask({SOC_RES_SSAO}), res_mask({SOC_RES_SSAO_BLUR}),
             [r](const soc_globals* g, hipStream_t s) { return soc_ssao_blur(g, r->img.ssao, r->img.ssao_blur, (soc_stream)s); });
    const bool fused_hist = !(r->flags & SOC_RENDERER_UNFUSED_HISTOGRAM);
    const soc_img& em_img = I.bloom_output.data ? I.bloom_output : I.emissive;
    soc_globals gres{};
    gres.resolution[0] = I.color.width;
    gres.resolution[1] = I.color.height;
    r->sky_split = fused_hist && !(r->flags & SOC_RENDERER_NO_SKY_SPLIT) &&
                   soc::composition_pair_applicable(&gres, I.color, I.albedo, em_img, I.normal, I.depth, I.clouds);
    const uint64_t sky_w = r->sky_split ? res_mask({SOC_RES_SKY_COLOR, SOC_RES_SKY_HISTOGRAM_PARTIALS}) : 0;
    const uint64_t parts = res_mask({SOC_RES_HISTOGRAM_PARTIALS}) | (r->sky_split ? res_mask({SOC_RES_SKY_HISTOGRAM_PARTIALS}) : 0);
    add_pass(r, "CloudRendering", "Sky Rendering", pre, res_mask({SOC_RES_DEPTH, SOC_RES_NOISE}), res_mask({SOC_RES_CLOUDS}),
             [r](const soc_globals* g, hipStream_t s) {
                 const bool sky_bound = sky_lane_high(r) && tuning_knob("SOC_RENDERER_SKY_BOUND_VARIANTS", 1);
                 return soc::cloud_rendering_launch(g, r->img.depth, r->img.noise, r->img.clouds, r->img.clouds_workspace,
                                                    (soc_stream)s, sky_bound, &r->clouds_state);
             }, SOC_PASS_ASYNC);
    if (r->sky_split)
        add_pass(r, "SkyCompose", "Sky Rendering", pre, res_mask({SOC_RES_CLOUDS, SOC_RES_DEPTH}), sky_w,
                 [r](const soc_globals* g, hipStream_t s) {
                     return soc::sky_compose_launch(g, r->img.color, r->img.depth, r->img.clouds, r->hist_scratch,
                                                    (soc_stream)s);
                 }, SOC_PASS_ASYNC);
    const uint64_t comp_reads = res_mask({SOC_RES_ALBEDO, em_res, SOC_RES_NORMAL, SOC_RES_DEPTH, SOC_RES_SSAO_BLUR,
                                          SOC_RES_SUN_SHADOW}) | (r->bloom_in_comp ? res_mask({SOC_RES_BLOOM_MIP1}) : 0) |
                                (r->sky_split ? 0 : res_mask({SOC_RES_CLOUDS}));
    if (fused_hist) {
        add_pass(r, "Composition+GenerateLuminanceHistogram", "Composition", pre, comp_reads,
                 res_mask({SOC_RES_COLOR, SOC_RES_HISTOGRAM_PARTIALS}), [r](const soc_globals* g, hipStream_t s) {
                     const auto& I = r->img;
                     const soc_img& em = I.bloom_output.data ? I.bloom_output : I.emissive;
                     return soc::composition_luminance_histogram(g, I.d_globals, I.color, I.albedo, em, I.normal, I.depth,
                                                                 I.ssao_blur, I.shadow, I.clouds, I.auto_exposure,
                                                                 r->hist_scratch, false, (soc_stream)s,
                                                                 r->sky_split_active,
                                                                 bloom_in_comp_active(r) ? &I.bloom_mips[1] : nullptr);
                 });
        auto& fold = add_pass(r, "LuminanceHistogramFold", "Auto Exposure", pre, parts,
                              res_mask({SOC_RES_AUTO_EXPOSURE}) | parts,
                              [r](const soc_globals* g, hipStream_t s) {
                                  (void)g;
                                  return soc::histogram_fold_launch(r->hist_scratch, r->img.auto_exposure, (soc_stream)s);
                              });
        fold.skip = [r] { return r->fold_in_resolve; };
    } else {
        add_pass(r, "Composition", "Composition", pre, comp_reads, res_mask({SOC_RES_COLOR}),
                 [r](const soc_globals* g, hipStream_t s) {
                     const auto& I = r->img;
                     const soc_img& em = I.bloom_output.data ? I.bloom_output : I.emissive;
                     return soc_composition(g, I.d_globals, I.color, I.albedo, em, I.normal, I.depth, I.ssao_blur,
                                            I.shadow, I.clouds, (soc_stream)s);
                 });
        add_pass(r, "GenerateLuminanceHistogram", "Auto Exposure", pre, res_mask({SOC_RES_COLOR}),
                 res_mask({SOC_RES_AUTO_EXPOSURE}), [r](const soc_globals* g, hipStream_t s) {
                     return soc_generate_luminance_histogram(g, r->img.color, r->img.auto_exposure, (soc_stream)s);
                 });
    }
    add_pass(r, "ResolveLuminanceHistogram", "Auto Exposure", post, res_mask({SOC_RES_AUTO_EXPOSURE}) | parts,
             res_mask({SOC_RES_AUTO_EXPOSURE}) | parts, [r](const soc_globals* g, hipStream_t s) {
                 return soc::resolve_luminance_histogram(g, r->img.auto_exposure, r->total_pixels, r->wide,
                                                         r->fold_in_resolve ? r->hist_scratch : nullptr, (soc_stream)s);
             });
    const bool vslots = r->flags & SOC_RENDERER_VELOCITY_SLOTS;
    const uint64_t taa_reads = res_mask({SOC_RES_COLOR, SOC_RES_PREVIOUS_COLOR, SOC_RES_VELOCITY,
                                         SOC_RES_PREVIOUS_VELOCITY, SOC_RES_DEPTH}) |
                               (r->sky_split ? res_mask({SOC_RES_SKY_COLOR}) : 0);
    const uint64_t taa_writes = vslots ? res_mask({SOC_RES_RESOLVED}) : res_mask({SOC_RES_RESOLVED, SOC_RES_PREVIOUS_VELOCITY});
    const bool fuse_tm = !(r->flags & SOC_RENDERER_UNFUSED_TONEMAP) &&
                         (I.output.format == SOC_FMT_RGBA8_UNORM || I.output.format == SOC_FMT_RGBA8_SRGB);
    if (fuse_tm) {
        add_pass(r, "TemporalAntiAliasing+ToneMapping", "Temporal Anti-Aliasing", post,
                 taa_reads | res_mask({SOC_RES_AUTO_EXPOSURE}), taa_writes | res_mask({SOC_RES_OUTPUT}),
                 [r](const soc_globals* g, hipStream_t s) {
                     const auto& I = r->img;
                     const int p = r->hist, q = 1 - r->hist;
                     const bool slots = r->flags & SOC_RENDERER_VELOCITY_SLOTS;
                     return soc_temporal_antialiasing_tone_mapping(g, I.history_color[q], I.color, I.history_color[p],
                                                                   frame_velocity(r), I.history_velocity[p], I.depth,
                                                                   slots ? soc_img{} : I.history_velocity[q],
                                                                   I.auto_exposure, I.output, (soc_stream)s);
                 });
    } else {
        add_pass(r, "TemporalAntiAliasing", "Temporal Anti-Aliasing", post, taa_reads, taa_writes,
                 [r](const soc_globals* g, hipStream_t s) {
                     const auto& I = r->img;
                     const int p = r->hist, q = 1 - r->hist;
                     const bool slots = r->flags & SOC_RENDERER_VELOCITY_SLOTS;
                     return soc_temporal_antialiasing(g, I.history_color[q], I.color, I.history_color[p],
                                                      frame_velocity(r), I.history_velocity[p], I.depth,
                                                      slots ? soc_img{} : I.history_velocity[q], (soc_stream)s);
                 });
        add_pass(r, "ToneMapping", "Tone Mapping", post, res_mask({SOC_RES_RESOLVED, SOC_RES_AUTO_EXPOSURE}),
                 res_mask({SOC_RES_OUTPUT}), [r](const soc_globals* g, hipStream_t s) {
                     const auto& I = r->img;
                     return soc_tone_mapping(g, I.history_color[1 - r->hist], I.auto_exposure, I.output, (soc_stream)s);
                 });
    }
}

soc_frame_images callback_view(const soc_renderer* r) {
    soc_frame_images v = r->img;
    const int p = r->hist, q = 1 - r->hist;
    v.history_color[0] = r->img.history_color[p];
    v.history_color[1] = r->img.history_color[q];
    v.history_velocity[0] = r->img.history_velocity[p];
    v.history_velocity[1] = r->img.history_velocity[q];
    v.velocity = frame_velocity(r);
    return v;
}

uint64_t desc_mask(const int32_t* ids, int32_t n) {
    uint64_t m = 0;
    for (int i = 0; i < n; ++i) m |= 1ull << ids[i];
    return m;
}

uint64_t widen_sky(const soc_renderer* r, uint64_t m) {
    if (!r->sky_split) return m;
    if (m & (1ull << SOC_RES_COLOR)) m |= 1ull << SOC_RES_SKY_COLOR;
    if (m & (1ull << SOC_RES_HISTOGRAM_PARTIALS)) m |= 1ull << SOC_RES_SKY_HISTOGRAM_PARTIALS;
    return m;
}

int insert_user_passes(soc_renderer* r) {
    for (auto& up : r->user_passes) {
        soc_renderer::Pass p;
        p.name = up.name;
        p.group = up.group;
        p.phase = up.desc.phase;
        p.reads = widen_velocity(r, widen_sky(r, desc_mask(up.desc.reads, up.desc.read_count)));
        p.writes = widen_velocity(r, widen_sky(r, desc_mask(up.desc.writes, up.desc.write_count)));
        p.flags = up.desc.flags;
        const soc_pass_callback fn = up.fn;
        void* user = up.user;
        if (up.ssr) {
            const soc_img mr = up.ssr_mr, target = up.ssr_target, steps = up.ssr_steps;
            p.run = [r, mr, target, steps](const soc_globals* g, hipStream_t s) {
                return soc_screen_space_reflection(g, r->img.depth, r->img.normal, r->img.albedo, mr, target, steps,
                                                   (soc_stream)s);
            };
        } else {
            p.run = [r, fn, user](const soc_globals* g, hipStream_t s) {
                const soc_frame_images v = callback_view(r);
                const int32_t rc = fn(user, g, &v, (soc_stream)s);
                return rc ? set_error(rc, "caller pass failed with %d", (int)rc) : (int)SOC_OK;
            };
        }
        size_t at = r->passes.size();
        if (!up.before.empty()) {
            at = r->passes.size() + 1;
            for (size_t i = 0; i < r->passes.size(); ++i)
                if (up.before_prefix ? r->passes[i].name.compare(0, up.before.size(), up.before) == 0
                                     : r->passes[i].name == up.before) { at = i; break; }
            if (at > r->passes.size())
                return set_error(SOC_E_INVALID_ARG, "soc_renderer_add_pass: no pass named \"%s\"", up.before.c_str());
            if (r->passes[at].phase != p.phase)
                return set_error(SOC_E_INVALID_ARG, "soc_renderer_add_pass: \"%s\" is in another phase", up.before.c_str());
        } else {
            for (size_t i = 0; i < r->passes.size(); ++i)
                if (r->passes[i].phase > p.phase) { at = i; break; }
        }
        r->passes.insert(r->passes.begin() + (long)at, std::move(p));
    }
    return SOC_OK;
}

int prev_frame_resource(int b) {
    if (b == SOC_RES_PREVIOUS_COLOR) return SOC_RES_RESOLVED;
    if (b == SOC_RES_RESOLVED) return SOC_RES_PREVIOUS_COLOR;
    return b;
}

void derive_dependencies(soc_renderer* r) {
    const int n = (int)r->passes.size();
    for (int i = 0; i < n; ++i) {
        auto& p = r->passes[i];
        p.deps.clear();
        p.carry.clear();
        std::vector<char> dep(n, 0), carry(n, 0);
        for (int b = 0; b < SOC_RES_COUNT; ++b) {
            const uint64_t bit = 1ull << b;
            if (!((p.reads | p.writes) & bit)) continue;
            bool writer = false;
            for (int j = i - 1; j >= 0 && !writer; --j) {
                const auto& q = r->passes[j];
                if (q.writes & bit) { dep[j] = 1; writer = true; }
                else if ((p.writes & bit) && (q.reads & bit)) dep[j] = 1;
            }
            if (writer) continue;
            const uint64_t pbit = 1ull << prev_frame_resource(b);
            for (int j = n - 1; j >= i; --j) {
                const auto& q = r->passes[j];
                if (q.writes & pbit) { carry[j] = 1; break; }
                if ((p.writes & bit) && (q.reads & pbit)) carry[j] = 1;
            }
        }
        for (int j = 0; j < n; ++j) {
            if (dep[j]) p.deps.push_back(j);
            if (carry[j]) p.carry.push_back(j);
        }
    }
}

void destroy_pass_events(soc_renderer* r) {
    for (auto& p : r->passes) {
        for (auto e : p.ev0) (void)hipEventDestroy(e);
        for (auto e : p.ev1) (void)hipEventDestroy(e);
        if (p.done) (void)hipEventDestroy(p.done);
    }
}

void derive_signals(soc_renderer* r) {
    const int n = (int)r->passes.size();
    for (auto& p : r->passes) p.signal = false;
    for (int i = 0; i < n; ++i) {
        const bool li = (r->passes[i].flags & SOC_PASS_ASYNC) != 0;
        for (int j : r->passes[i].deps)
            if (((r->passes[j].flags & SOC_PASS_ASYNC) != 0) != li) r->passes[j].signal = true;
        if (!li)
            for (int j : r->passes[i].carry)
                if ((r->passes[j].flags & SOC_PASS_ASYNC) != 0) r->passes[j].signal = true;
    }
}

int build_graph(soc_renderer* r) {
    r->inputs_ordered = false;
    destroy_pass_events(r);
    r->passes.clear();
    build_raster_passes(r);
    build_passes(r);
    build_passes_tail(r);
    int rc = insert_user_passes(r);
    derive_dependencies(r);
    derive_signals(r);
    return rc;
}
}

extern "C" soc_renderer* soc_renderer_create(const soc_frame_images* images, uint32_t flags) {
    if (!images) {
        set_error(SOC_E_INVALID_ARG, "soc_renderer_create: null images");
        return nullptr;
    }
    if (!images->auto_exposure) {
        set_error(SOC_E_INVALID_ARG, "soc_renderer_create: auto_exposure buffer required");
        return nullptr;
    }
    if ((flags & SOC_RENDERER_VELOCITY_SLOTS) &&
        (!images->history_velocity[0].data || !images->history_velocity[1].data ||
         images->history_velocity[0].data == images->history_velocity[1].data)) {
        set_error(SOC_E_INVALID_ARG, "soc_renderer_create: SOC_RENDERER_VELOCITY_SLOTS needs two distinct history_velocity images");
        return nullptr;
    }
    soc_renderer* r = new soc_renderer();
    r->img = *images;
    r->flags = flags;
    r->async = !(flags & SOC_RENDERER_SERIAL);
    (void)build_graph(r);
    if ((flags & SOC_RENDERER_TIMING) && soc_renderer_set_pass_timing(r, -1, 1) != SOC_OK) {
        soc_renderer_destroy(r);
        return nullptr;
    }
    return r;
}

static void destroy_side_lane(soc_renderer* r);

extern "C" void soc_renderer_destroy(soc_renderer* r) {
    if (!r) return;
    destroy_pass_events(r);
    for (auto& e : r->staging_ev)
        if (e) (void)hipEventDestroy(e);
    if (r->staging) (void)hipHostFree(r->staging);
    destroy_side_lane(r);
    if (r->hist_scratch) (void)hipFree(r->hist_scratch);
    if (r->shadow_ws) (void)hipFree(r->shadow_ws);
    delete r;
}

static int upload_lights(soc_renderer* r, const soc_globals* g, hipStream_t s) {
    if (!r->img.d_globals) return set_error(SOC_E_INVALID_ARG, "soc_renderer_execute: lights need frame d_globals");
    if (!r->staging) {
        if (hipHostMalloc((void**)&r->staging, 4 * sizeof(soc_globals), 0) != hipSuccess)
            return set_error(SOC_E_HIP, "soc_renderer_execute: hipHostMalloc failed");
        for (auto& e : r->staging_ev)
            if (hipEventCreateWithFlags(&e, hipEventDisableTiming) != hipSuccess)
                return set_error(SOC_E_HIP, "soc_renderer_execute: hipEventCreate failed");
    }
    const int slot = r->staging_slot;
    r->staging_slot = (slot + 1) & 3;
    (void)hipEventSynchronize(r->staging_ev[slot]);
    std::memcpy(&r->staging[slot], g, sizeof(soc_globals));
    hipError_t e = hipMemcpyAsync(r->img.d_globals, &r->staging[slot], sizeof(soc_globals), hipMemcpyHostToDevice, s);
    if (e != hipSuccess) return set_error(SOC_E_HIP, "soc_renderer_execute: globals upload: %s", hipGetErrorString(e));
    (void)hipEventRecord(r->staging_ev[slot], s);
    return SOC_OK;
}

static unsigned device_event_flags() {
    return (unsigned)hipEventDisableTiming |
           (tuning_knob("SOC_RENDERER_EVENT_FENCE", 0) == 1 ? (unsigned)hipEventDisableSystemFence : 0u);
}

static int run_pass(soc_renderer::Pass& p, const soc_globals* g, hipStream_t s) {
    const int slot = p.next;
    if (p.timed) (void)hipEventRecord(p.ev0[slot], s);
    int rc = p.run(g, s);
    if (rc) return rc;
    if (p.timed) {
        (void)hipEventRecord(p.ev1[slot], s);
        p.last = slot;
        p.next = (slot + 1) % SOC_RENDERER_TIMING_RING;
        if (p.count < SOC_RENDERER_TIMING_RING) p.count++;
    }
    return SOC_OK;
}

static void destroy_side_lane(soc_renderer* r) {
    for (hipEvent_t* e : {&r->fork_ev, &r->join_ev, &r->switch_ev})
        if (*e) { (void)hipEventDestroy(*e); *e = nullptr; }
    for (auto& e : r->probe_ev)
        if (e) { (void)hipEventDestroy(e); e = nullptr; }
    if (r->lane_q[0] || r->lane_q[1]) {
        for (auto& q : r->lane_q)
            if (q) { (void)hipStreamDestroy(q); q = nullptr; }
    } else if (r->side) {
        (void)hipStreamDestroy(r->side);
    }
    r->side = nullptr;
    r->side_queue = -1;
    r->probe_frames = 0;
}

static int ensure_side_lane(soc_renderer* r) {
    int dev = 0;
    if (hipGetDevice(&dev) != hipSuccess) return set_error(SOC_E_HIP, "soc_renderer_execute: hipGetDevice failed");
    if (r->side && r->side_device == dev) return SOC_OK;
    if (r->side) {
        destroy_side_lane(r);
        r->clouds_state.reset();
        for (auto& p : r->passes)
            if (p.done) { (void)hipEventDestroy(p.done); p.done = nullptr; p.done_recorded = false; }
    }
    const int sq_flags = (r->flags & SOC_RENDERER_SKY_LANE_HIGH) ? 1 : (r->flags & SOC_RENDERER_SKY_LANE_PROBE) ? 3 : 2;
    int sq = tuning_knob("SOC_RENDERER_SIDE_QUEUE", sq_flags);
    int least = 0, greatest = 0;
    if (hipDeviceGetStreamPriorityRange(&least, &greatest) != hipSuccess || least == greatest) sq = 0;
    hipError_t se = hipSuccess;
    if (sq == 3) {
        se = hipStreamCreateWithPriority(&r->lane_q[0], hipStreamNonBlocking, greatest);
        if (se == hipSuccess) se = hipStreamCreateWithPriority(&r->lane_q[1], hipStreamNonBlocking, least);
        if (se == hipSuccess) se = hipEventCreateWithFlags(&r->switch_ev, device_event_flags());
        for (auto& e : r->probe_ev)
            if (se == hipSuccess) se = hipEventCreate(&e);
        r->side = r->lane_q[0];
        r->side_queue = -1;
        r->probe_frames = 0;
    } else if (const int cus = tuning_knob("SOC_RENDERER_SKY_CUS", 0); cus > 0 && cus < 32) {
        int dev_cus = 256;
        (void)hipDeviceGetAttribute(&dev_cus, hipDeviceAttributeMultiprocessorCount, dev);
        const int layout = tuning_knob("SOC_RENDERER_SKY_CU_LAYOUT", 0);
        std::vector<uint32_t> mask((size_t)(dev_cus + 31) / 32, 0u);
        for (int i = 0; i < dev_cus; ++i)
            if ((layout ? i % 32 : (i / 8) % 32) < cus) mask[(size_t)i / 32] |= 1u << (i % 32);
        se = hipExtStreamCreateWithCUMask(&r->side, (uint32_t)mask.size(), mask.data());
        r->side_queue = 0;
    } else if (sq == 1 || sq == 2) {
        se = hipStreamCreateWithPriority(&r->side, hipStreamNonBlocking, sq == 2 ? least : greatest);
        r->side_queue = sq;
    } else {
        se = hipStreamCreateWithFlags(&r->side, hipStreamNonBlocking);
        r->side_queue = 0;
    }
    if (se != hipSuccess ||
        hipEventCreateWithFlags(&r->fork_ev, hipEventDisableTiming) != hipSuccess ||
        hipEventCreateWithFlags(&r->join_ev, hipEventDisableTiming) != hipSuccess) {
        destroy_side_lane(r);
        return set_error(SOC_E_HIP, "soc_renderer_execute: second lane stream/event creation failed");
    }
    r->side_device = dev;
    return SOC_OK;
}

static int switch_side_lane(soc_renderer* r, hipStream_t q) {
    if (q == r->side) return SOC_OK;
    if (hipEventRecord(r->switch_ev, r->side) != hipSuccess || hipStreamWaitEvent(q, r->switch_ev, 0) != hipSuccess)
        return set_error(SOC_E_HIP, "soc_renderer_execute: second lane switch failed");
    r->side = q;
    return SOC_OK;
}

static int probe_window(const soc_renderer* r) {
    const long long px = (long long)r->img.color.width * r->img.color.height;
    if (px <= 0) return 32;
    return (int)std::min<long long>(128, std::max<long long>(32, 32LL * 8294400LL / px));
}
constexpr int kProbeStart = 16, kProbeWins = 8;
static int probe_end(const soc_renderer* r) { return kProbeStart + kProbeWins * probe_window(r); }

static int frame_lane_probe(soc_renderer* r, hipStream_t s) {
    if (r->side_queue != -1 || !r->lane_q[0]) return SOC_OK;
    const int kStart = kProbeStart, kWindow = probe_window(r), kSkip = 8, kEnd = probe_end(r);
    constexpr int kWins = kProbeWins;
    constexpr bool kHigh[kWins] = {true, false, false, true, true, false, false, true};
    const int f = r->probe_frames;
    if (f <= kEnd) {
        if (f >= kStart) {
            const int w = (f - kStart) / kWindow, o = (f - kStart) % kWindow;
            int slot = -1;
            if (o == kSkip && w < kWins) slot = 2 * w;
            else if (o == 0 && w > 0) slot = 2 * (w - 1) + 1;
            if (slot >= 0 && hipEventRecord(r->probe_ev[slot], s) != hipSuccess)
                return set_error(SOC_E_HIP, "soc_renderer_execute: lane probe event failed");
            if (o == 0 && w < kWins) {
                int rc = switch_side_lane(r, r->lane_q[kHigh[w] ? 0 : 1]);
                if (rc) return rc;
            }
        }
        r->probe_frames++;
        return SOC_OK;
    }
    if (hipEventQuery(r->probe_ev[2 * kWins - 1]) != hipSuccess) {
        (void)hipGetLastError();
        return SOC_OK;
    }
    float hi = 0.0f, lo = 0.0f;
    for (int w = 0; w < kWins; ++w) {
        float t = 0.0f;
        if (hipEventElapsedTime(&t, r->probe_ev[2 * w], r->probe_ev[2 * w + 1]) != hipSuccess) {
            (void)hipGetLastError();
            r->side_queue = 2;
            return switch_side_lane(r, r->lane_q[1]);
        }
        (kHigh[w] ? hi : lo) += t;
    }
    r->side_queue = (hi < 0.98f * lo) ? 1 : 2;
    return switch_side_lane(r, r->lane_q[r->side_queue - 1]);
}

static int static_lane(const soc_renderer* r, int i) {
    return (r->async && (r->passes[i].flags & SOC_PASS_ASYNC)) ? 1 : 0;
}

static int abort_frame(soc_renderer* r, hipStream_t s, bool forked, int rc) {
    if (forked && r->side && hipEventRecord(r->join_ev, r->side) == hipSuccess &&
        hipStreamWaitEvent(s, r->join_ev, 0) == hipSuccess)
        r->main_after_side = true;
    else if (forked)
        r->main_after_side = false;
    if (r->hist_scratch) (void)hipMemsetAsync(r->hist_scratch, 0, SOC_HISTOGRAM_SCRATCH_WORDS * sizeof(uint32_t), s);
    if (r->img.auto_exposure)
        (void)hipMemsetAsync(r->img.auto_exposure->histogram_buckets, 0, sizeof(r->img.auto_exposure->histogram_buckets), s);
    return rc;
}

extern "C" int soc_renderer_execute(soc_renderer* r, const soc_globals* g, int32_t phase, soc_stream stream) {
    if (!r || !g) return set_error(SOC_E_INVALID_ARG, "soc_renderer_execute: null argument");
    hipStream_t s = hs(stream);
    r->fold_in_resolve = (phase & SOC_PHASE_ALL) == SOC_PHASE_ALL && !(r->flags & SOC_RENDERER_UNFUSED_HISTOGRAM);
    if (phase & SOC_PHASE_PRE_EXPOSURE) {
        const soc_img& em = r->img.bloom_output.data ? r->img.bloom_output : r->img.emissive;
        const bool pair_ok = soc::composition_pair_applicable(g, r->img.color, r->img.albedo, em, r->img.normal,
                                                             r->img.depth, r->img.clouds);
        r->sky_split_active = r->sky_split && pair_ok;
        r->bloom_in_comp_ok = pair_ok;
        if (r->sky_split && !r->sky_split_active)
            return set_error(SOC_E_SHAPE, "soc_renderer_execute: globals resolution %dx%d differs from the frame images %dx%d",
                             g->resolution[0], g->resolution[1], r->img.color.width, r->img.color.height);
        if (!(r->flags & SOC_RENDERER_UNFUSED_HISTOGRAM)) {
            int rc = ensure_hist_scratch(r, s);
            if (rc) return rc;
        }
    }
    if ((phase & SOC_PHASE_PRE_EXPOSURE) && (g->point_light_count || g->spot_light_count)) {
        int rc = upload_lights(r, g, s);
        if (rc) return rc;
    }
    const int n = (int)r->passes.size();
    std::vector<int> lane(n, -1);
    bool lanes = false;
    for (int i = 0; i < n; ++i) {
        const auto& p = r->passes[i];
        if (!(p.phase & phase) || (p.skip && p.skip())) continue;
        lane[i] = static_lane(r, i);
        lanes |= lane[i] == 1;
    }
    std::vector<std::vector<int>> deps(n);
    for (int i = 0; i < n; ++i) {
        const auto& p = r->passes[i];
        if (lane[i] < 0 && !(p.phase & phase)) continue;
        for (int j : p.deps) {
            if (lane[j] >= 0) deps[i].push_back(j);
            else if (r->passes[j].phase & phase) deps[i].insert(deps[i].end(), deps[j].begin(), deps[j].end());
        }
    }
    std::vector<std::vector<int>> ext(n);
    for (int i = 0; i < n; ++i) {
        if (lane[i] < 0) continue;
        const auto& p = r->passes[i];
        for (int j : p.carry)
            if (static_lane(r, j) != lane[i]) ext[i].push_back(j);
        for (int j : p.deps)
            if (lane[j] < 0 && !(r->passes[j].phase & phase) && static_lane(r, j) != lane[i]) ext[i].push_back(j);
    }
    bool forked_wait = false;
    if (lanes) {
        int rc = ensure_side_lane(r);
        if (!rc && (phase & SOC_PHASE_PRE_EXPOSURE)) rc = frame_lane_probe(r, s);
        if (rc) return rc;
        if (hipEventRecord(r->fork_ev, s) != hipSuccess)
            return set_error(SOC_E_HIP, "soc_renderer_execute: second lane fork failed");
    }
    std::vector<int> order(n);
    for (int i = 0; i < n; ++i) order[i] = i;
    const int ao_pos = tuning_knob("SOC_RENDERER_SSAO_FIRST", -1);
    if (ao_pos) {
        std::vector<int> ao, rest;
        for (int i = 0; i < n; ++i) (r->passes[i].group == "Ambient Occlusion" ? ao : rest).push_back(i);
        bool free = !ao.empty();
        for (int a : ao)
            for (int j : deps[a])
                if (r->passes[j].group != "Ambient Occlusion") free = false;
        if (free) {
            size_t at = 0;
            if (ao_pos >= 2) at = std::min(rest.size(), (size_t)(ao_pos - 1));
            if (ao_pos < 0)
                for (size_t k = 0; k < rest.size(); ++k)
                    if (r->passes[rest[k]].group == "Bloom") at = k;
            order.assign(rest.begin(), rest.begin() + at);
            order.insert(order.end(), ao.begin(), ao.end());
            order.insert(order.end(), rest.begin() + at, rest.end());
        }
    }
    std::vector<char> needs_fork(n, 0);
    bool pre_fork = true;
    for (int oi = 0; oi < n; ++oi) {
        const int i = order[oi];
        if (lane[i] != 1) continue;
        bool carry_main = false;
        for (int j : r->passes[i].carry) carry_main |= static_lane(r, j) == 0;
        if (!(r->flags & SOC_RENDERER_STATIC_INPUTS) || !r->inputs_ordered || carry_main) pre_fork = false;
        needs_fork[i] = !pre_fork;
    }
    std::vector<int> pos(n, -1);
    int next_pos[2] = {0, 0}, waited[2] = {-1, -1};
    for (int oi = 0; oi < n; ++oi) {
        const int i = order[oi];
        if (lane[i] < 0) continue;
        auto& p = r->passes[i];
        const int L = lane[i];
        hipStream_t ls = L ? r->side : s;
        if (L == 1 && needs_fork[i] && !forked_wait) {
            if (hipStreamWaitEvent(r->side, r->fork_ev, 0) != hipSuccess)
                return abort_frame(r, s, lanes, set_error(SOC_E_HIP, "soc_renderer_execute: second lane fork failed"));
            forked_wait = true;
        }
        for (int j : deps[i])
            if (lane[j] != L && pos[j] > waited[L]) {
                if (hipStreamWaitEvent(ls, r->passes[j].done, 0) != hipSuccess)
                    return abort_frame(r, s, lanes, set_error(SOC_E_HIP, "soc_renderer_execute: %s: cross-lane wait failed", p.name.c_str()));
                waited[L] = pos[j];
            }
        for (int j : ext[i])
            if (L == 0 && !r->main_after_side && r->passes[j].done_recorded &&
                hipStreamWaitEvent(ls, r->passes[j].done, 0) != hipSuccess)
                return abort_frame(r, s, lanes, set_error(SOC_E_HIP, "soc_renderer_execute: %s: ring-edge wait failed", p.name.c_str()));
        static const char* probe_skip = getenv("SOC_RENDERER_PROBE_SKIP_PASS");
        int rc = (probe_skip && p.name == probe_skip) ? (int)SOC_OK : run_pass(p, g, ls);
        if (rc) return abort_frame(r, s, lanes, rc);
        pos[i] = next_pos[L]++;
        if (p.signal) {
            if (!p.done && hipEventCreateWithFlags(&p.done, device_event_flags()) != hipSuccess)
                return abort_frame(r, s, lanes, set_error(SOC_E_HIP, "soc_renderer_execute: hipEventCreate failed"));
            if (hipEventRecord(p.done, ls) != hipSuccess)
                return abort_frame(r, s, lanes, set_error(SOC_E_HIP, "soc_renderer_execute: %s: event record failed", p.name.c_str()));
            p.done_recorded = true;
        }
    }
    const bool side_joined = waited[0] >= next_pos[1] - 1;
    if (lanes && !side_joined &&
        (hipEventRecord(r->join_ev, r->side) != hipSuccess || hipStreamWaitEvent(s, r->join_ev, 0) != hipSuccess))
        return abort_frame(r, s, lanes, set_error(SOC_E_HIP, "soc_renderer_execute: second lane join failed"));
    r->main_after_side = true;
    r->inputs_ordered = true;
    if (phase & SOC_PHASE_POST_EXPOSURE) r->hist = 1 - r->hist;
    return SOC_OK;
}

static hipError_t shadow_ws_alloc(void** p, size_t n) {
    if (tuning_knob("SOC_TEST_FAIL_SHADOW_WS", 0)) return hipMalloc(p, (size_t)1 << 62);
    return hipMalloc(p, n);
}

extern "C" int soc_renderer_set_raster_scene(soc_renderer* r, const soc_raster_scene* scene) {
    if (!r) return set_error(SOC_E_INVALID_ARG, "soc_renderer_set_raster_scene: null renderer");
    if (scene) {
        if (!scene->materials || scene->material_count <= 0 || !scene->visibility || !scene->workspace ||
            !scene->mesh.positions || !scene->mesh.normals || !scene->mesh.uvs || !scene->mesh.indices)
            return set_error(SOC_E_INVALID_ARG, "soc_renderer_set_raster_scene: incomplete scene");
        if (scene->shadow && !r->img.shadow.data)
            return set_error(SOC_E_INVALID_ARG, "soc_renderer_set_raster_scene: shadow pass needs images.shadow");
    }
    if (scene && scene->shadow) {
        const size_t need = soc_raster_workspace_size(scene->mesh.vertex_count, scene->mesh.triangle_count);
        if (need > r->shadow_ws_bytes) {
            if (r->shadow_ws) (void)hipFree(r->shadow_ws);
            r->shadow_ws = nullptr;
            r->shadow_ws_bytes = 0;
            if (shadow_ws_alloc(&r->shadow_ws, need) != hipSuccess) {
                r->shadow_ws = nullptr;
                (void)hipGetLastError();
            } else {
                r->shadow_ws_bytes = need;
            }
        }
    }
    r->has_scene = scene != nullptr;
    if (scene) r->scene = *scene;
    int rc = build_graph(r);
    if (rc) return rc;
    if (r->flags & SOC_RENDERER_TIMING) return soc_renderer_set_pass_timing(r, -1, 1);
    return SOC_OK;
}

static int register_user_pass(soc_renderer* r, const soc_pass_desc* d, soc_renderer::UserPass up, const char* before) {
    if (d->phase != SOC_PHASE_PRE_EXPOSURE && d->phase != SOC_PHASE_POST_EXPOSURE)
        return set_error(SOC_E_INVALID_ARG, "soc_renderer_add_pass: %s: phase must be PRE or POST", d->name);
    if (d->read_count < 0 || d->read_count > SOC_PASS_MAX_USES || d->write_count < 0 || d->write_count > SOC_PASS_MAX_USES)
        return set_error(SOC_E_INVALID_ARG, "soc_renderer_add_pass: %s: at most %d reads / writes", d->name, SOC_PASS_MAX_USES);
    for (int i = 0; i < d->read_count + d->write_count; ++i) {
        const int id = i < d->read_count ? d->reads[i] : d->writes[i - d->read_count];
        if (id < 0 || id >= SOC_RES_COUNT)
            return set_error(SOC_E_INVALID_ARG, "soc_renderer_add_pass: %s: bad resource id %d", d->name, id);
    }
    for (const auto& p : r->passes)
        if (p.name == d->name) return set_error(SOC_E_INVALID_ARG, "soc_renderer_add_pass: duplicate pass name \"%s\"", d->name);
    up.desc = *d;
    up.name = d->name;
    up.group = d->group ? d->group : "";
    up.before = before ? before : "";
    up.desc.name = nullptr;
    up.desc.group = nullptr;
    r->user_passes.push_back(up);
    int rc = build_graph(r);
    if (rc) {
        r->user_passes.pop_back();
        (void)build_graph(r);
        return rc;
    }
    if (r->flags & SOC_RENDERER_TIMING) return soc_renderer_set_pass_timing(r, -1, 1);
    return SOC_OK;
}

extern "C" int soc_renderer_add_pass(soc_renderer* r, const soc_pass_desc* d, soc_pass_callback fn, void* user,
                                     const char* before) {
    if (!r || !d || !fn || !d->name || !d->name[0])
        return set_error(SOC_E_INVALID_ARG, "soc_renderer_add_pass: null renderer, descriptor, callback or name");
    soc_renderer::UserPass up;
    up.fn = fn;
    up.user = user;
    return register_user_pass(r, d, up, before);
}

extern "C" int soc_renderer_add_screen_space_reflection(soc_renderer* r, soc_img metallic_roughness, soc_img target,
                                                        soc_img steps, int32_t metallic_roughness_resource,
                                                        int32_t target_resource, uint32_t pass_flags, const char* before) {
    const char* fn = "soc_renderer_add_screen_space_reflection";
    if (!r) return set_error(SOC_E_INVALID_ARG, "%s: null renderer", fn);
    if (pass_flags & ~(uint32_t)SOC_PASS_ASYNC) return set_error(SOC_E_INVALID_ARG, "%s: pass_flags must be 0 or SOC_PASS_ASYNC", fn);
    for (int32_t id : {metallic_roughness_resource, target_resource})
        if (id < SOC_RES_USER0 || id >= SOC_RES_COUNT)
            return set_error(SOC_E_INVALID_ARG, "%s: bad resource id %d (SOC_RES_USER0 .. SOC_RES_USER0 + 31)", fn, id);
    if (metallic_roughness_resource == target_resource)
        return set_error(SOC_E_INVALID_ARG, "%s: the metallic-roughness image and the target need two resource ids", fn);
    int rc = check_img(metallic_roughness, SOC_FMT_RGBA16F, fn, "metallic_roughness");
    if (!rc) rc = check_img(target, SOC_FMT_RGBA16F, fn, "target");
    if (!rc && steps.data) rc = check_img(steps, SOC_FMT_R8_UNORM, fn, "steps");
    if (rc) return rc;
    const soc_img* same[] = {&metallic_roughness, &target, &steps};
    for (const soc_img* im : same)
        if (im->data && (im->width != r->img.depth.width || im->height != r->img.depth.height))
            return set_error(SOC_E_SHAPE, "%s: image is %dx%d, the frame's depth %dx%d", fn, im->width, im->height,
                             r->img.depth.width, r->img.depth.height);
    soc_pass_desc d{};
    d.name = "ScreenSpaceReflection";
    d.group = "Screen Space Reflections";
    d.phase = SOC_PHASE_PRE_EXPOSURE;
    d.flags = pass_flags;
    d.read_count = 4;
    d.reads[0] = SOC_RES_ALBEDO;
    d.reads[1] = SOC_RES_NORMAL;
    d.reads[2] = SOC_RES_DEPTH;
    d.reads[3] = metallic_roughness_resource;
    d.write_count = 1;
    d.writes[0] = target_resource;
    soc_renderer::UserPass up;
    up.ssr = true;
    up.ssr_mr = metallic_roughness;
    up.ssr_target = target;
    up.ssr_steps = steps;
    up.before_prefix = before == nullptr;
    return register_user_pass(r, &d, up, before ? before : "CloudRendering");
}

extern "C" int soc_renderer_pass_uses(const soc_renderer* r, int32_t i, uint64_t* reads, uint64_t* writes) {
    if (!r || i < 0 || i >= (int32_t)r->passes.size() || !reads || !writes)
        return set_error(SOC_E_INVALID_ARG, "soc_renderer_pass_uses: bad arguments");
    *reads = r->passes[i].reads;
    *writes = r->passes[i].writes;
    return SOC_OK;
}

extern "C" int32_t soc_renderer_pass_dependencies(const soc_renderer* r, int32_t i, int32_t* out, int32_t cap) {
    if (!r || i < 0 || i >= (int32_t)r->passes.size() || cap < 0 || (cap > 0 && !out))
        return set_error(SOC_E_INVALID_ARG, "soc_renderer_pass_dependencies: bad arguments");
    const auto& d = r->passes[i].deps;
    for (int k = 0; k < (int)d.size() && k < cap; ++k) out[k] = d[k];
    return (int32_t)d.size();
}

extern "C" int32_t soc_renderer_pass_carry_dependencies(const soc_renderer* r, int32_t i, int32_t* out, int32_t cap) {
    if (!r || i < 0 || i >= (int32_t)r->passes.size() || cap < 0 || (cap > 0 && !out))
        return set_error(SOC_E_INVALID_ARG, "soc_renderer_pass_carry_dependencies: bad arguments");
    const auto& d = r->passes[i].carry;
    for (int k = 0; k < (int)d.size() && k < cap; ++k) out[k] = d[k];
    return (int32_t)d.size();
}

extern "C" int32_t soc_renderer_pass_lane(const soc_renderer* r, int32_t i) {
    if (!r || i < 0 || i >= (int32_t)r->passes.size()) return set_error(SOC_E_INVALID_ARG, "soc_renderer_pass_lane: bad index");
    return (r->passes[i].flags & SOC_PASS_ASYNC) ? 1 : 0;
}

extern "C" int soc_renderer_set_async(soc_renderer* r, int32_t enable) {
    if (!r) return set_error(SOC_E_INVALID_ARG, "soc_renderer_set_async: null renderer");
    if (r->async != (enable != 0)) {
        r->inputs_ordered = false;
    }
    r->async = enable != 0;
    return SOC_OK;
}

extern "C" int soc_renderer_invalidate_cloud_tables(soc_renderer* r) {
    if (!r) return set_error(SOC_E_INVALID_ARG, "soc_renderer_invalidate_cloud_tables: null renderer");
    r->clouds_state.reset();
    return SOC_OK;
}

extern "C" int soc_renderer_set_exposure_pixels(soc_renderer* r, uint64_t total_pixels, int32_t wide_accumulator) {
    if (!r) return set_error(SOC_E_INVALID_ARG, "soc_renderer_set_exposure_pixels: null renderer");
    r->total_pixels = total_pixels;
    r->wide = wide_accumulator;
    return SOC_OK;
}

extern "C" int32_t soc_renderer_pass_count(const soc_renderer* r) { return r ? (int32_t)r->passes.size() : 0; }

extern "C" const char* soc_renderer_pass_name(const soc_renderer* r, int32_t i) {
    if (!r || i < 0 || i >= (int32_t)r->passes.size()) return nullptr;
    return r->passes[i].name.c_str();
}

extern "C" const char* soc_renderer_pass_group(const soc_renderer* r, int32_t i) {
    if (!r || i < 0 || i >= (int32_t)r->passes.size()) return nullptr;
    return r->passes[i].group.c_str();
}

extern "C" float soc_renderer_pass_ms(soc_renderer* r, int32_t i) {
    if (!r || i < 0 || i >= (int32_t)r->passes.size()) return -1.0f;
    auto& p = r->passes[i];
    if (!p.timed || p.last < 0) return -1.0f;
    float ms = -1.0f;
    if (hipEventElapsedTime(&ms, p.ev0[p.last], p.ev1[p.last]) != hipSuccess) return -1.0f;
    return ms;
}
// ... 109 lines not shown
```

### soc_real_time_renderer_amd/csrc/composition.hip

```cpp
#include <type_traits>

#include "bloom_w.hpp"
#include "luminance.hpp"
#include "soc_internal.hpp"

#ifndef SOC_COMP_PROFILE
#define SOC_COMP_PROFILE 0
#endif

namespace soc {
namespace {

struct CompParams {
    Mat4 inv_proj, inv_view, sun_pv;
    Mat4 sun_clip;
    float sun_dir[3], ambient[3], cam[3];
    float ef, df, emissive_strength, ao_strength;
    uint32_t npl, nsl;
    int swz;
    uint32_t* bins;
    float lmin, lrange;
    BinFast bf;
    const soc_globals* __restrict__ dg;
    int sky_external;
    float rw, rh;
    int bloom_zero_skip;
};

__device__ __forceinline__ float fast_pow(float x, float y) {
    return __builtin_amdgcn_exp2f(y * __builtin_amdgcn_logf(x));
}

typedef float f2v __attribute__((ext_vector_type(2)));
template <class T> struct V3 { T x, y, z; };
__device__ __forceinline__ float bcv(float s, float) { return s; }
__device__ __forceinline__ f2v bcv(float s, f2v) { return f2v{s, s}; }
__device__ __forceinline__ float vfma(float a, float b, float c) { return __builtin_fmaf(a, b, c); }
__device__ __forceinline__ f2v vfma(f2v a, f2v b, f2v c) { return __builtin_elementwise_fma(a, b, c); }
__device__ __forceinline__ float vrsq(float x) { return __builtin_amdgcn_rsqf(x); }
__device__ __forceinline__ f2v vrsq(f2v x) { return f2v{__builtin_amdgcn_rsqf(x.x), __builtin_amdgcn_rsqf(x.y)}; }
__device__ __forceinline__ float vsqrt(float x) { return __builtin_amdgcn_sqrtf(x); }
__device__ __forceinline__ f2v vsqrt(f2v x) { return f2v{__builtin_amdgcn_sqrtf(x.x), __builtin_amdgcn_sqrtf(x.y)}; }
__device__ __forceinline__ float vexp2(float x) { return __builtin_amdgcn_exp2f(x); }
__device__ __forceinline__ f2v vexp2(f2v x) { return f2v{__builtin_amdgcn_exp2f(x.x), __builtin_amdgcn_exp2f(x.y)}; }
__device__ __forceinline__ float vabs(float x) { return fabsf(x); }
__device__ __forceinline__ f2v vabs(f2v x) { return f2v{fabsf(x.x), fabsf(x.y)}; }
__device__ __forceinline__ float vmax0(float x) { return fmaxf(x, 0.0f); }
__device__ __forceinline__ f2v vmax0(f2v x) { return f2v{fmaxf(x.x, 0.0f), fmaxf(x.y, 0.0f)}; }
__device__ __forceinline__ float vclamp01(float x) { return clampf(x, 0.0f, 1.0f); }
__device__ __forceinline__ f2v vclamp01(f2v x) { return f2v{clampf(x.x, 0.0f, 1.0f), clampf(x.y, 0.0f, 1.0f)}; }
__device__ __forceinline__ float vneg_pi(float x, float r) { return x < 0.0f ? 3.14159265358979f - r : r; }
__device__ __forceinline__ f2v vneg_pi(f2v x, f2v r) {
    const f2v q = f2v{3.14159265358979f, 3.14159265358979f} - r;
    return f2v{x.x < 0.0f ? q.x : r.x, x.y < 0.0f ? q.y : r.y};
}
__device__ __forceinline__ float vnan_outside1(float x, float r) { return fabsf(x) > 1.0f ? __builtin_nanf("") : r; }
__device__ __forceinline__ f2v vnan_outside1(f2v x, f2v r) {
    return f2v{fabsf(x.x) > 1.0f ? __builtin_nanf("") : r.x, fabsf(x.y) > 1.0f ? __builtin_nanf("") : r.y};
}
__device__ __forceinline__ float vdiv(float a, float b) { return a / b; }
__device__ __forceinline__ f2v vdiv(f2v a, float b) { return f2v{a.x / b, a.y / b}; }
template <class T> __device__ __forceinline__ T vdot(const V3<T>& a, const V3<T>& b) {
    return vfma(a.z, b.z, vfma(a.y, b.y, a.x * b.x));
}

template <class T>
__device__ __forceinline__ T acos_fast(T x) {
    const T a = vabs(x);
    T r = bcv(-0.0012624911f, x);
    r = vfma(r, a, bcv(0.0066700901f, x));
    r = vfma(r, a, bcv(-0.0170881256f, x));
    r = vfma(r, a, bcv(0.0308918810f, x));
    r = vfma(r, a, bcv(-0.0501743046f, x));
    r = vfma(r, a, bcv(0.0889789874f, x));
    r = vfma(r, a, bcv(-0.2145988016f, x));
    r = vfma(r, a, bcv(1.5707963050f, x));
    r = r * vsqrt(bcv(1.0f, x) - a);
    return vneg_pi(x, r);
}

#ifndef SOC_COMP_SPEC_POLY
#define SOC_COMP_SPEC_POLY 1
#endif
template <class T>
__device__ __forceinline__ T spec_exp_acos2(T c) {
    constexpr float k[11] = {0.08480516821146011f,  0.26642516255378723f,  0.33367738127708435f,   0.21618370711803436f,
                             0.07947526127099991f,  0.017337322235107422f, 0.0017174964305013418f, -0.00019129738211631775f,
                             0.0007113117026165128f, 0.00020575939561240375f, -0.00034820116707123816f};
    T r = bcv(k[10], c);
#pragma unroll
    for (int i = 9; i >= 0; --i) r = vfma(r, c, bcv(k[i], c));
    return vnan_outside1(c, r);
}

template <class T>
__device__ __forceinline__ V3<T> light_sum(const soc_globals* __restrict__ dg, uint32_t npl, uint32_t nsl, const V3<T>& n,
                                           const V3<T>& pos, f3 cam) {
    const T z = pos.x;
    const V3<T> vd0 = {bcv(cam.x, z) - pos.x, bcv(cam.y, z) - pos.y, bcv(cam.z, z) - pos.z};
    const T vk = vrsq(vdot(vd0, vd0));
    const V3<T> view_dir = {vd0.x * vk, vd0.y * vk, vd0.z * vk};
    V3<T> acc = {bcv(0.0f, z), bcv(0.0f, z), bcv(0.0f, z)};
    const T nlog2e = bcv(-1.44269504088896f, z);
    auto shade_light = [&](const float* lp, T& inv, V3<T>& ld) {
        const V3<T> l = {bcv(lp[0], z) - pos.x, bcv(lp[1], z) - pos.y, bcv(lp[2], z) - pos.z};
        inv = vrsq(vdot(l, l));
        ld = V3<T>{l.x * inv, l.y * inv, l.z * inv};
        const V3<T> h = {ld.x + view_dir.x, ld.y + view_dir.y, ld.z + view_dir.z};
        const T c = vdot(h, n) * vrsq(vdot(h, h));
        const T diffuse = vmax0(vdot(n, ld));
        if (SOC_COMP_SPEC_POLY) return (diffuse + spec_exp_acos2(c)) * (inv * inv);
        const T nh = acos_fast(c);
        return (diffuse + vexp2((nh * nh) * nlog2e)) * (inv * inv);
    };
    auto add = [&](const float* col, T s) {
        acc = V3<T>{vfma(bcv(col[0], z), s, acc.x), vfma(bcv(col[1], z), s, acc.y), vfma(bcv(col[2], z), s, acc.z)};
    };
#ifndef SOC_COMP_LIGHT_UNROLL
#define SOC_COMP_LIGHT_UNROLL 2
#endif
#pragma unroll SOC_COMP_LIGHT_UNROLL
    for (uint32_t i = 0; i < npl; ++i) {
        const soc_point_light& L = dg->point_lights[i];
        T inv;
        V3<T> ld;
        const T s = shade_light(L.position, inv, ld) * bcv(L.intensity, z);
        add(L.color, s);
    }
#pragma unroll 2
    for (uint32_t i = 0; i < nsl; ++i) {
        const soc_spot_light& L = dg->spot_lights[i];
        T inv;
        V3<T> ld;
        const T b = shade_light(L.position, inv, ld);
        const float sdx = -L.direction[0], sdy = -L.direction[1], sdz = -L.direction[2];
        const float sk = __builtin_amdgcn_rsqf(__builtin_fmaf(sdz, sdz, __builtin_fmaf(sdy, sdy, sdx * sdx)));
        const T theta = vfma(ld.z, bcv(sdz, z), vfma(ld.y, bcv(sdy, z), ld.x * bcv(sdx, z))) * bcv(sk, z);
        const T intensity = vclamp01(vdiv(theta - bcv(L.outer_cut_off, z), L.cut_off - L.outer_cut_off));
        add(L.color, b * bcv(L.intensity, z) * intensity);
    }
    return acc;
}

struct ShadePre {
    float direct;
    float occl;
    f3 em;
};
template <typename ShadowImg = DImg>
__device__ __forceinline__ ShadePre shade_pre(const CompParams& p, float u, float v, float d, f3 emissive, f3 n, float ssao,
                                              const ShadowImg& shadow) {
    const f4 ndc = f4{u * 2.0f - 1.0f, v * 2.0f - 1.0f, d, 1.0f};
    const f4 sp = mul(p.sun_clip, ndc);
    const float rsw = __builtin_amdgcn_rcpf(sp.w);
    const float pcx = sp.x * rsw * 0.5f + 0.5f;
    const float pcy = sp.y * rsw * 0.5f + 0.5f;
    const float pcz = sp.z * rsw;
    const float sd = (SOC_COMP_PROFILE & 1) ? pcx * 0.001f : sample_f32(shadow, pcx, pcy);
    float e = __expf(p.ef * (pcz - sd));
    if (p.df != 1.0f) e = fast_pow(e, p.df);
    const float sun_shadow = clampf(e, 0.0f, 1.0f);
    ShadePre s;
    s.em = emissive * p.emissive_strength;
    s.occl = fast_pow(ssao, p.ao_strength);
    s.direct = fmaxf(0.0f, dot3(n, -mk3(p.sun_dir[0], p.sun_dir[1], p.sun_dir[2]))) * sun_shadow;
    return s;
}
__device__ __forceinline__ f3 world_pos(const CompParams& p, float u, float v, float d) {
    const f4 ndc = f4{u * 2.0f - 1.0f, v * 2.0f - 1.0f, d, 1.0f};
    f4 vs = mul(p.inv_proj, ndc);
    const float rw = __builtin_amdgcn_rcpf(vs.w);
    vs = f4{vs.x * rw, vs.y * rw, vs.z * rw, 1.0f};
    const f4 ws = mul(p.inv_view, vs);
    return f3{ws.x, ws.y, ws.z};
}
__device__ __forceinline__ f4 shade_post(const CompParams& p, const ShadePre& s, f3 albedo, const f3* lights) {
    f3 direct = f3{s.direct, s.direct, s.direct};
    if (lights)
        direct = f3{__builtin_fmaf(albedo.x, lights->x, direct.x), __builtin_fmaf(albedo.y, lights->y, direct.y),
                    __builtin_fmaf(albedo.z, lights->z, direct.z)};
    const f3 c = (direct + mk3(p.ambient[0], p.ambient[1], p.ambient[2])) * albedo * s.occl + s.em;
    return f4{c.x, c.y, c.z, 1.0f};
}
template <bool LIGHTS = true, typename ShadowImg = DImg>
__device__ __forceinline__ f4 shade(const CompParams& p, float u, float v, float d, f3 albedo, f3 emissive, f3 n,
                                    float ssao, const ShadowImg& shadow) {
    const ShadePre s = shade_pre(p, u, v, d, emissive, n, ssao, shadow);
    if (LIGHTS && (p.npl | p.nsl)) {
        const f3 wp = world_pos(p, u, v, d);
        const V3<float> ls = light_sum(p.dg, p.npl, p.nsl, V3<float>{n.x, n.y, n.z}, V3<float>{wp.x, wp.y, wp.z},
                                       mk3(p.cam[0], p.cam[1], p.cam[2]));
        const f3 l3 = f3{ls.x, ls.y, ls.z};
        return shade_post(p, s, albedo, &l3);
    }
    return shade_post(p, s, albedo, nullptr);
}

constexpr int BX = 64, BY = 4;

#ifndef SOC_COMP_LIGHT_WAVES
#define SOC_COMP_LIGHT_WAVES 6
#endif
template <bool HIST, bool LIGHTS, int NT = 0, bool BL = false>
__global__ __launch_bounds__(kWorkgroup) __attribute__((amdgpu_waves_per_eu(LIGHTS && !BL ? SOC_COMP_LIGHT_WAVES : 1))) void composition_pair(DImg target, DImg albedo, DImg emissive, DImg normal, DImg depth,
                                                        DImg ssao, DImg shadow, DImg clouds, CompParams p, DImg mip1) {
    static_assert(!BL || HIST, "the in-kernel bloom runs in the fused-histogram kernel (no early exit before its barriers)");
    __shared__ uint32_t sh[HIST ? 4 * kBins : 1];
    const int lane = threadIdx.x & 63, wave = threadIdx.x >> 6;
    if (HIST) reinterpret_cast<uint4*>(sh + wave * kBins)[lane] = uint4{0u, 0u, 0u, 0u};
    int bx, by;
    xcd_order(p.swz, bx, by);
    const int x = bx * 32 + (wave & 1) * 16 + (lane & 7) * 2;
    const int y = by * 16 + (wave >> 1) * 8 + (lane >> 3);
    const bool inside = x < target.w && y < target.h;
    if (!HIST && !inside) return;
    uint2 outp[2] = {uint2{0u, 0u}, uint2{0u, 0u}};
    uint32_t own = 3u;
    const BufImg bd = buf_img(depth), ba = buf_img(albedo), be = buf_img(emissive), bn = buf_img(normal);
    const BufImg bt = buf_img(target), bs = buf_img(shadow), bo = buf_img(ssao);
    const float v = centre_uv_rn(y, target.h, p.rh);
    constexpr int ld_aux = (NT & 1) ? 2 : 0;
    float2 d2 = float2{0.0f, 0.0f};
    uint4 a4 = uint4{0u, 0u, 0u, 0u}, e4 = a4, n4 = a4;
    float aop[2] = {0.0f, 0.0f};
    if (inside) {
        d2 = __builtin_bit_cast(float2, __builtin_amdgcn_raw_buffer_load_b64(bd.r, buf_row(bd, y) + x * 4, 0, ld_aux));
        a4 = __builtin_bit_cast(uint4, __builtin_amdgcn_raw_buffer_load_b128(ba.r, buf_row(ba, y) + x * 8, 0, ld_aux));
        if (!BL) e4 = __builtin_bit_cast(uint4, __builtin_amdgcn_raw_buffer_load_b128(be.r, buf_row(be, y) + x * 8, 0, ld_aux));
        n4 = __builtin_bit_cast(uint4, __builtin_amdgcn_raw_buffer_load_b128(bn.r, buf_row(bn, y) + x * 8, 0, ld_aux));
        if (NT & 4) sample_r8_pair(bo, centre_uv_rn(x, target.w, p.rw), centre_uv_rn(x + 1, target.w, p.rw), v, aop[0], aop[1]);
    }
    if constexpr (BL) {
        __shared__ Up10Tile<32, 16> bl;
        const int X0 = bx * 32, Y0 = by * 16;
        if (bl.build(mip1, X0, Y0, target.w, target.h, threadIdx.x, p.bloom_zero_skip != 0)) {
            const uint2 b0 = pack3(C3{0.0f, 0.0f, 0.0f});
            e4 = uint4{b0.x, b0.y, b0.x, b0.y};
        } else {
            C3 o[2];
            bl.out(y - Y0, x - X0, o);
            const uint2 b0 = pack3(o[0]), b1 = pack3(o[1]);
            e4 = uint4{b0.x, b0.y, b1.x, b1.y};
        }
    }
    if (inside) {
        ShadePre pre[2];
        f3 alb[2], nrm[2], wps[2];
        uint32_t lit = 0u;
#pragma unroll
        for (int k = 0; k < 2; ++k) {
            const float u = centre_uv_rn(x + k, target.w, p.rw);
            const float d = k ? d2.y : d2.x;
            const f4 al = unpack_h4(k ? uint2{a4.z, a4.w} : uint2{a4.x, a4.y});
            const f4 em = unpack_h4(k ? uint2{e4.z, e4.w} : uint2{e4.x, e4.y});
            const f4 nn = unpack_h4(k ? uint2{n4.z, n4.w} : uint2{n4.x, n4.y});
            f4 c;
            if (LIGHTS) {
                nrm[k] = f3{nn.x, nn.y, nn.z};
                wps[k] = world_pos(p, u, v, d);
            }
            if (d == 1.0f && p.sky_external) {
                own &= ~(1u << k);
                continue;
            }
            if (d == 1.0f) {
                const f4 cl = fetch_rgba8(clouds, x + k, y);
                c = f4{cl.x, cl.y, cl.z, 1.0f};
            } else {
                const float ao = (SOC_COMP_PROFILE & 2) ? u : (NT & 4) ? aop[k] : sample_r8(bo, u, v);
                if (LIGHTS) {
                    pre[k] = shade_pre(p, u, v, d, f3{em.x, em.y, em.z}, f3{nn.x, nn.y, nn.z}, ao, bs);
                    alb[k] = f3{al.x, al.y, al.z};
                    lit |= 1u << k;
                    continue;
                }
                c = shade<false>(p, u, v, d, f3{al.x, al.y, al.z}, f3{em.x, em.y, em.z}, f3{nn.x, nn.y, nn.z}, ao, bs);
            }
            outp[k] = pack_h4(c);
        }
        if (LIGHTS && lit) {
            const V3<f2v> n2 = {f2v{nrm[0].x, nrm[1].x}, f2v{nrm[0].y, nrm[1].y}, f2v{nrm[0].z, nrm[1].z}};
            const V3<f2v> w2 = {f2v{wps[0].x, wps[1].x}, f2v{wps[0].y, wps[1].y}, f2v{wps[0].z, wps[1].z}};
            const V3<f2v> ls = light_sum(p.dg, p.npl, p.nsl, n2, w2, mk3(p.cam[0], p.cam[1], p.cam[2]));
#pragma unroll
            for (int k = 0; k < 2; ++k)
                if (lit & (1u << k)) {
                    const f3 l3 = k ? f3{ls.x.y, ls.y.y, ls.z.y} : f3{ls.x.x, ls.y.x, ls.z.x};
                    outp[k] = pack_h4(shade_post(p, pre[k], alb[k], &l3));
                }
        }
        const uint4 o = uint4{outp[0].x, outp[0].y, outp[1].x, outp[1].y};
        typedef uint32_t v4w __attribute__((ext_vector_type(4)));
        const int to = buf_row(bt, y) + x * 8;
        if (own == 3u) {
            __builtin_amdgcn_raw_buffer_store_b128(__builtin_bit_cast(v4w, o), bt.r, to, 0, (NT & 2) ? 2 : 0);
        } else {
            typedef uint32_t v2w __attribute__((ext_vector_type(2)));
            if (own & 1u) __builtin_amdgcn_raw_buffer_store_b64(__builtin_bit_cast(v2w, outp[0]), bt.r, to, 0, 0);
            if (own & 2u) __builtin_amdgcn_raw_buffer_store_b64(__builtin_bit_cast(v2w, outp[1]), bt.r, to + 8, 0, 0);
        }
    }
    if (HIST) {
        const f4 c0 = unpack_h4(outp[0]), c1 = unpack_h4(outp[1]);
        uint32_t b0 = lum_bin_fast(c0.x, c0.y, c0.z, p.bf);
        uint32_t b1 = lum_bin_fast(c1.x, c1.y, c1.z, p.bf);
        if (b0 == kBinExact) b0 = lum_bin(c0.x, c0.y, c0.z, p.lmin, p.lrange);
        if (b1 == kBinExact) b1 = lum_bin(c1.x, c1.y, c1.z, p.lmin, p.lrange);
        lane_bin_pair_mask(sh + wave * kBins, b0, b1, inside ? own : 0u);
        __syncthreads();
        const uint32_t n = sh[threadIdx.x] + sh[kBins + threadIdx.x] + sh[2 * kBins + threadIdx.x] + sh[3 * kBins + threadIdx.x];
        if (n) atomicAdd(&p.bins[((blockIdx.y * gridDim.x + blockIdx.x) & 7u) * kBins + threadIdx.x], n);
    }
}

template <bool CP>
__global__ __launch_bounds__(kWorkgroup) void sky_compose_pair(DImg target, DImg depth, DImg clouds, CompParams p) {
    __shared__ uint32_t sh[4 * kBins];
    const int lane = threadIdx.x & 63, wave = threadIdx.x >> 6;
    reinterpret_cast<uint4*>(sh + wave * kBins)[lane] = uint4{0u, 0u, 0u, 0u};
    const int bx = blockIdx.x, by = blockIdx.y;
    const int x = bx * 32 + (wave & 1) * 16 + (lane & 7) * 2;
    const int y = by * 16 + (wave >> 1) * 8 + (lane >> 3);
    const bool inside = x < target.w && y < target.h;
    uint32_t mine = 0u;
    uint2 outp[2] = {uint2{0u, 0u}, uint2{0u, 0u}};
    if (inside) {
        const float2 d2 = row_ptr<float2>(depth, y)[x >> 1];
        const bool s0 = d2.x == 1.0f, s1 = d2.y == 1.0f;
        if (!CP) {
#pragma unroll
            for (int k = 0; k < 2; ++k) {
                if (!(k ? s1 : s0)) continue;
                const f4 cl = fetch_rgba8(clouds, x + k, y);
                outp[k] = pack_h4(f4{cl.x, cl.y, cl.z, 1.0f});
                row_ptr_w<uint2>(target, y)[x + k] = outp[k];
                mine |= 1u << k;
            }
        } else if (s0 || s1) {
            const uint2 cw = row_ptr<uint2>(clouds, y)[x >> 1];
#pragma unroll
            for (int k = 0; k < 2; ++k) {
                if (!(k ? s1 : s0)) continue;
                const f4 cl = unpack_rgba8(k ? cw.y : cw.x);
                outp[k] = pack_h4(f4{cl.x, cl.y, cl.z, 1.0f});
                row_ptr_w<uint2>(target, y)[x + k] = outp[k];
                mine |= 1u << k;
            }
        }
    }
    const f4 c0 = unpack_h4(outp[0]), c1 = unpack_h4(outp[1]);
    uint32_t b0 = lum_bin_fast(c0.x, c0.y, c0.z, p.bf);
    uint32_t b1 = lum_bin_fast(c1.x, c1.y, c1.z, p.bf);
    if (b0 == kBinExact) b0 = lum_bin(c0.x, c0.y, c0.z, p.lmin, p.lrange);
    if (b1 == kBinExact) b1 = lum_bin(c1.x, c1.y, c1.z, p.lmin, p.lrange);
    lane_bin_pair_mask(sh + wave * kBins, b0, b1, mine);
    __syncthreads();
    const uint32_t n = sh[threadIdx.x] + sh[kBins + threadIdx.x] + sh[2 * kBins + threadIdx.x] + sh[3 * kBins + threadIdx.x];
    if (n) atomicAdd(&p.bins[((blockIdx.y * gridDim.x + blockIdx.x) & 7u) * kBins + threadIdx.x], n);
}

__global__ __launch_bounds__(kBins) void histogram_fold(uint32_t* __restrict__ scratch, uint32_t* __restrict__ bins) {
    const int i = threadIdx.x;
    uint32_t s = 0;
#pragma unroll
    for (int k = 0; k < 8; ++k) {
        s += scratch[k * kBins + i];
        scratch[k * kBins + i] = 0u;
    }
    if (s) bins[i] += s;
}

__global__ __launch_bounds__(kWorkgroup) void composition_generic(DImg target, DImg albedo, DImg emissive, DImg normal,
                                                           DImg depth, DImg ssao, DImg shadow, DImg clouds, CompParams p) {
    const int x = blockIdx.x * BX + threadIdx.x, y = blockIdx.y * BY + threadIdx.y;
    if (x >= target.w || y >= target.h) return;
    const float u = centre_uv(x, target.w), v = centre_uv(y, target.h);
    const float d = sample_f32(depth, u, v);
    f4 c;
    if (d == 1.0f) {
        const f4 cl = sample_rgba8(clouds, u, v);
        c = f4{cl.x, cl.y, cl.z, 1.0f};
    } else {
        const f4 al = sample_h4(albedo, u, v), em = sample_h4(emissive, u, v), nn = sample_h4(normal, u, v);
        c = shade(p, u, v, d, f3{al.x, al.y, al.z}, f3{em.x, em.y, em.z}, f3{nn.x, nn.y, nn.z}, sample_r8(ssao, u, v),
                  shadow);
    }
    row_ptr_w<uint2>(target, y)[x] = pack_h4(c);
}

bool aligned16(const soc_img& im) {
    return (reinterpret_cast<uintptr_t>(im.data) & 15u) == 0 && (im.pitch_bytes & 15) == 0;
}

}
}

using namespace soc;

namespace {
int composition_launch(const soc_globals* g, const soc_globals* d_globals, soc_img target, soc_img albedo, soc_img emissive,
                       soc_img normal, soc_img depth, soc_img ssao, soc_img shadow, soc_img clouds, uint32_t* bins,
                       uint32_t* scratch, soc_stream stream, bool fold = true, bool sky_external = false,
                       const soc_img* bloom_mip1 = nullptr) {
    static const char* P = "soc_composition";
    if (!g) return set_error(SOC_E_INVALID_ARG, "%s: null globals", P);
    int rc = check_img(target, SOC_FMT_RGBA16F, P, "target");
    if (!rc) rc = check_img(albedo, SOC_FMT_RGBA16F, P, "albedo");
    if (!rc) rc = check_img(emissive, SOC_FMT_RGBA16F, P, "emissive");
    if (!rc) rc = check_img(normal, SOC_FMT_RGBA16F, P, "normal");
    if (!rc) rc = check_img(depth, SOC_FMT_D32F, P, "depth");
    if (!rc) rc = check_img(ssao, SOC_FMT_R8_UNORM, P, "ssao");
    if (!rc) rc = check_img(shadow, SOC_FMT_D32F, P, "shadow");
    if (!rc) rc = check_img(clouds, SOC_FMT_RGBA8_UNORM, P, "clouds");
    if (rc) return rc;
    CompParams p;
    p.inv_proj = mat4(g->camera_inverse_projection_matrix);
    p.inv_view = mat4(g->camera_inverse_view_matrix);
    mat4_mul_host(p.sun_pv.m, g->sun_info.projection_matrix, g->sun_info.view_matrix);
    {
        float t[16];
        mat4_mul_host(t, p.sun_pv.m, g->camera_inverse_view_matrix);
        mat4_mul_host(p.sun_clip.m, t, g->camera_inverse_projection_matrix);
    }
    for (int i = 0; i < 3; ++i) {
        p.sun_dir[i] = g->sun_info.direction[i];
        p.ambient[i] = g->ambient[i];
        p.cam[i] = g->camera_position[i];
    }
    p.ef = g->sun_info.exponential_factor;
    p.df = g->sun_info.darkening_factor;
    p.emissive_strength = g->emissive_bloom_strength;
    p.ao_strength = g->ambient_occlussion_strength;
    p.npl = g->point_light_count < SOC_MAX_POINT_LIGHTS ? g->point_light_count : SOC_MAX_POINT_LIGHTS;
    p.nsl = g->spot_light_count < SOC_MAX_SPOT_LIGHTS ? g->spot_light_count : SOC_MAX_SPOT_LIGHTS;
    p.dg = d_globals;
    const bool nt = tuning_knob("SOC_COMP_NT", 3) == 3;
    const bool aop = tuning_knob("SOC_COMP_AOP", 1) != 0;
    p.swz = 0;
    p.rw = recip_rn(target.width);
    p.rh = recip_rn(target.height);
    p.bloom_zero_skip = tuning_knob("SOC_BLOOM_ZERO_SKIP", 1) != 0;
    p.bins = nullptr;
    p.sky_external = 0;
    if ((p.npl || p.nsl) && !d_globals)
        return set_error(SOC_E_INVALID_ARG, "%s: frame has lights but no device globals (soc_upload_globals)", P);

    const int W = target.width, H = target.height;
    auto same = [&](const soc_img& im) { return im.width == W && im.height == H; };
    const bool fast = same(albedo) && same(emissive) && same(normal) && same(depth) && same(clouds) && (W % 2 == 0) &&
                      W <= 8192 && H <= 8192 && aligned16(target) && aligned16(albedo) && aligned16(emissive) &&
                      aligned16(normal) && (reinterpret_cast<uintptr_t>(depth.data) & 7u) == 0 && (depth.pitch_bytes & 7) == 0;
    if (bins && !(fast && W == g->resolution[0] && H == g->resolution[1])) return 1;
    if (sky_external && !bins) return set_error(SOC_E_INVALID_ARG, "%s: sky_external needs the fused histogram", P);
    if (bloom_mip1) {
        rc = check_img(*bloom_mip1, SOC_FMT_RGBA16F, P, "bloom mip1");
        if (rc) return rc;
        if (!bins || !fast || bloom_mip1->width * 2 != W || bloom_mip1->height * 2 != H)
            return set_error(SOC_E_SHAPE, "%s: the in-kernel bloom needs the fused histogram's pair path and mip1 = W/2 x H/2", P);
    }
    if (fast) {
        dim3 grd(ceil_div(W, 32), ceil_div(H, 16));
        const bool lights = (p.npl | p.nsl) != 0;
#define SOC_COMP_PAIR(HI, LI) launch("composition_pair", kWorkgroup, composition_pair<HI, LI>, grd, kWorkgroup, 0, hs(stream), dimg(target), dimg(albedo), \
            dimg(emissive), dimg(normal), dimg(depth), dimg(ssao), dimg(shadow), dimg(clouds), p, DImg{})
        if (bins) {
            p.bins = scratch;
            p.sky_external = sky_external ? 1 : 0;
            p.lmin = g->log_min_luminance;
            p.lrange = g->log_max_luminance - g->log_min_luminance;
            p.bf = bin_fast_params(p.lmin, p.lrange);
            if (bloom_mip1 && lights)
                launch("composition_pair", kWorkgroup, composition_pair<true, true, 0, true>, grd, kWorkgroup, 0, hs(stream),
                       dimg(target), dimg(albedo), dimg(emissive), dimg(normal), dimg(depth), dimg(ssao), dimg(shadow),
                       dimg(clouds), p, dimg(*bloom_mip1));
            else if (bloom_mip1)
                launch("composition_pair", kWorkgroup, composition_pair<true, false, 7, true>, grd, kWorkgroup, 0, hs(stream),
                       dimg(target), dimg(albedo), dimg(emissive), dimg(normal), dimg(depth), dimg(ssao), dimg(shadow),
                       dimg(clouds), p, dimg(*bloom_mip1));
            else if (lights) SOC_COMP_PAIR(true, true);
            else if (nt && aop)
                launch("composition_pair", kWorkgroup, composition_pair<true, false, 7>, grd, kWorkgroup, 0, hs(stream), dimg(target), dimg(albedo), dimg(emissive),
                    dimg(normal), dimg(depth), dimg(ssao), dimg(shadow), dimg(clouds), p, DImg{});
            else if (nt)
                launch("composition_pair", kWorkgroup, composition_pair<true, false, 3>, grd, kWorkgroup, 0, hs(stream), dimg(target), dimg(albedo), dimg(emissive),
                    dimg(normal), dimg(depth), dimg(ssao), dimg(shadow), dimg(clouds), p, DImg{});
            else SOC_COMP_PAIR(true, false);
            if (fold) launch("histogram_fold", kBins, histogram_fold, 1, kBins, 0, hs(stream), scratch, bins);
        } else if (nt && !lights && aop) {
            launch("composition_pair", kWorkgroup, composition_pair<false, false, 7>, grd, kWorkgroup, 0, hs(stream), dimg(target), dimg(albedo), dimg(emissive),
                dimg(normal), dimg(depth), dimg(ssao), dimg(shadow), dimg(clouds), p, DImg{});
        } else if (nt && !lights) {
            launch("composition_pair", kWorkgroup, composition_pair<false, false, 3>, grd, kWorkgroup, 0, hs(stream), dimg(target), dimg(albedo), dimg(emissive),
                dimg(normal), dimg(depth), dimg(ssao), dimg(shadow), dimg(clouds), p, DImg{});
        } else {
            if (lights) SOC_COMP_PAIR(false, true);
            else SOC_COMP_PAIR(false, false);
        }
#undef SOC_COMP_PAIR
    } else {
        dim3 blk(BX, BY), grd(ceil_div(W, BX), ceil_div(H, BY));
        launch("composition_generic", kWorkgroup, composition_generic, grd, blk, 0, hs(stream), dimg(target), dimg(albedo), dimg(emissive), dimg(normal),
                                                         dimg(depth), dimg(ssao), dimg(shadow), dimg(clouds), p);
    }
    return check_launch("composition");
}
}

bool soc::composition_pair_applicable(const soc_globals* g, const soc_img& target, const soc_img& albedo,
                                      const soc_img& emissive, const soc_img& normal, const soc_img& depth,
                                      const soc_img& clouds) {
    const int W = target.width, H = target.height;
    auto same = [&](const soc_img& im) { return im.width == W && im.height == H; };
    return g && same(albedo) && same(emissive) && same(normal) && same(depth) && same(clouds) && (W % 2 == 0) &&
           W <= 8192 && H <= 8192 && aligned16(target) && aligned16(albedo) && aligned16(emissive) &&
           aligned16(normal) && (reinterpret_cast<uintptr_t>(depth.data) & 7u) == 0 && (depth.pitch_bytes & 7) == 0 &&
           W == g->resolution[0] && H == g->resolution[1];
}

int soc::sky_compose_launch(const soc_globals* g, soc_img target, soc_img depth, soc_img clouds, uint32_t* scratch,
                            soc_stream stream) {
    if (!g || !scratch) return set_error(SOC_E_INVALID_ARG, "sky compose: null globals / scratch");
    int rc = check_img(target, SOC_FMT_RGBA16F, "sky compose", "target");
    if (!rc) rc = check_img(depth, SOC_FMT_D32F, "sky compose", "depth");
    if (!rc) rc = check_img(clouds, SOC_FMT_RGBA8_UNORM, "sky compose", "clouds");
    if (rc) return rc;
    CompParams p{};
    p.bins = scratch;
    p.lmin = g->log_min_luminance;
    p.lrange = g->log_max_luminance - g->log_min_luminance;
    p.bf = bin_fast_params(p.lmin, p.lrange);
    const dim3 grd(ceil_div(target.width, 32), ceil_div(target.height, 16));
    const bool cp = (clouds.pitch_bytes % 8) == 0 && (reinterpret_cast<uintptr_t>(clouds.data) % 8) == 0 &&
                    tuning_knob("SOC_SKY_COMPOSE_PAIR_LOAD", 1);
    if (cp)
        launch("sky_compose_pair", kWorkgroup, sky_compose_pair<true>, grd, kWorkgroup, 0, hs(stream), dimg(target), dimg(depth),
               dimg(clouds), p);
    else
        launch("sky_compose_pair", kWorkgroup, sky_compose_pair<false>, grd, kWorkgroup, 0, hs(stream), dimg(target), dimg(depth),
               dimg(clouds), p);
    return check_launch("sky_compose");
}

extern "C" int soc_composition(const soc_globals* g, const soc_globals* d_globals, soc_img target, soc_img albedo,
                               soc_img emissive, soc_img normal, soc_img depth, soc_img ssao, soc_img shadow,
                               soc_img clouds, soc_stream stream) {
    return composition_launch(g, d_globals, target, albedo, emissive, normal, depth, ssao, shadow, clouds, nullptr, nullptr,
                              stream);
}

int soc::composition_luminance_histogram(const soc_globals* g, const soc_globals* d_globals, soc_img target,
                                         soc_img albedo, soc_img emissive, soc_img normal, soc_img depth, soc_img ssao,
                                         soc_img shadow, soc_img clouds, soc_auto_exposure* ae, uint32_t* scratch,
                                         bool fold, soc_stream stream, bool sky_external, const soc_img* bloom_mip1) {
    if (!g || !ae || !scratch)
        return set_error(SOC_E_INVALID_ARG, "soc_composition_luminance_histogram: null globals / auto exposure / scratch");
    int rc = composition_launch(g, d_globals, target, albedo, emissive, normal, depth, ssao, shadow, clouds,
                                ae->histogram_buckets, scratch, stream, fold, sky_external, bloom_mip1);
    if (rc <= 0) return rc;
    if (bloom_mip1) return set_error(SOC_E_SHAPE, "composition: the in-kernel bloom needs the pair path");
    if (sky_external) return set_error(SOC_E_INVALID_ARG, "composition: sky_external needs the pair path");
    rc = composition_launch(g, d_globals, target, albedo, emissive, normal, depth, ssao, shadow, clouds, nullptr, nullptr,
                            stream);
    if (rc) return rc;
    return soc_generate_luminance_histogram(g, target, ae, stream);
}

int soc::histogram_fold_launch(uint32_t* scratch, soc_auto_exposure* ae, soc_stream stream) {
    if (!scratch || !ae) return set_error(SOC_E_INVALID_ARG, "histogram fold: null scratch / auto exposure");
    launch("histogram_fold", kBins, histogram_fold, 1, kBins, 0, hs(stream), scratch, ae->histogram_buckets);
    return check_launch("luminance_histogram_fold");
}

extern "C" int soc_composition_luminance_histogram(const soc_globals* g, const soc_globals* d_globals, soc_img target,
                                                   soc_img albedo, soc_img emissive, soc_img normal, soc_img depth,
                                                   soc_img ssao, soc_img shadow, soc_img clouds, soc_auto_exposure* ae,
                                                   uint32_t* scratch, soc_stream stream) {
    return composition_luminance_histogram(g, d_globals, target, albedo, emissive, normal, depth, ssao, shadow, clouds, ae,
                                           scratch, true, stream);
}
```

### soc_real_time_renderer_amd/csrc/soc_internal.hpp

```cpp
#pragma once

#include <hip/hip_runtime.h>
#include <stdint.h>

#include <cstdarg>
#include <cstdio>
#include <string>

#include "../../include/soc_rt.h"
#include "soc_device.hpp"

namespace soc {

int set_error(int code, const char* fmt, ...);
void clear_error();

inline int bytes_per_pixel(int fmt) {
    switch (fmt) {
    case SOC_FMT_RGBA16F: return 8;
    case SOC_FMT_D32F: return 4;
    case SOC_FMT_R8_UNORM: return 1;
    case SOC_FMT_RGBA8_UNORM:
    case SOC_FMT_RGBA8_SRGB: return 4;
    case SOC_FMT_RGBA32F: return 16;
    default: return 0;
    }
}

inline bool img_ok(const soc_img& im) {
    int b = bytes_per_pixel(im.format);
    return im.data != nullptr && im.width > 0 && im.height > 0 && b > 0 && im.pitch_bytes >= im.width * b;
}

int check_img(const soc_img& im, int fmt, const char* pass, const char* what);

inline DImg dimg(const soc_img& im) { return DImg{static_cast<char*>(im.data), im.width, im.height, im.pitch_bytes}; }

inline Mat4 mat4(const float* m) {
    Mat4 r;
    for (int i = 0; i < 16; ++i) r.m[i] = m[i];
    return r;
}

inline hipStream_t hs(soc_stream s) { return reinterpret_cast<hipStream_t>(s); }

int tuning_knob(const char* name, int dflt);
inline float recip_rn(int n) {
    return n >= 1 && n <= 16384 ? 1.0f / (float)n : 0.0f;
}

int check_launch(const char* pass);

bool block_fits(const char* kernel, int bound, dim3 block);
template <typename... P, typename... A>
inline void launch(const char* kernel, int bound, void (*k)(P...), dim3 grid, dim3 block, size_t lds, hipStream_t s,
                   A&&... args) {
    if (!block_fits(kernel, bound, block)) return;
    k<<<grid, block, lds, s>>>(static_cast<P>(args)...);
}

inline unsigned ceil_div(unsigned a, unsigned b) { return (a + b - 1) / b; }

void agx_matrices(float compression, float M[9], float Minv[9]);
void mat4_mul_host(float out[16], const float a[16], const float b[16]);

bool bloom_fused_applicable(const soc_img& emissive, const soc_img* mips, int mip_count, const soc_img& output);
int launch_bloom_weighted(const soc_img& emissive, const soc_img* mips, const soc_img& output, hipStream_t s, int stage);

int composition_luminance_histogram(const soc_globals* g, const soc_globals* d_globals, soc_img target, soc_img albedo,
                                    soc_img emissive, soc_img normal, soc_img depth, soc_img ssao, soc_img shadow,
                                    soc_img clouds, soc_auto_exposure* ae, uint32_t* scratch, bool fold, soc_stream stream,
                                    bool sky_external = false, const soc_img* bloom_mip1 = nullptr);
bool composition_pair_applicable(const soc_globals* g, const soc_img& target, const soc_img& albedo,
                                 const soc_img& emissive, const soc_img& normal, const soc_img& depth,
                                 const soc_img& clouds);
struct CloudState {
    bool od_valid = false, noise_valid = false;
    uint32_t c2_bits = 0;
    const void* noise_data = nullptr;
    int32_t noise_format = 0, noise_pitch = 0;
    void* workspace = nullptr;
    bool blocks_primed = false;
    uint32_t frame = 0;
    void invalidate_tables() { od_valid = noise_valid = false; }
    void reset() { *this = CloudState(); }
};
int cloud_rendering_launch(const soc_globals* g, soc_img depth, soc_img noise, soc_img target, void* workspace,
                           soc_stream stream, bool sky_bound, CloudState* state = nullptr);
int sky_compose_launch(const soc_globals* g, soc_img target, soc_img depth, soc_img clouds, uint32_t* scratch,
                       soc_stream stream);
int histogram_fold_launch(uint32_t* scratch, soc_auto_exposure* ae, soc_stream stream);
int resolve_luminance_histogram(const soc_globals* g, soc_auto_exposure* ae, uint64_t total_pixels, int32_t wide_accumulator,
                                uint32_t* scratch, soc_stream stream);

}
```

Baseline: 1959.

## Propagate per-tile zero flags through the bloom chain to skip zero tiles

The first bloom downsample now writes a per-tile flag marking tiles whose emissive input was all zero. Later stages (down23, up32, up10, and composition) derive conservative flags from the previous stage's flags instead of re-reading texels. When a tile is flagged, they write zeros or skip the emissive load. This cuts memory traffic and arithmetic in scenes with sparse emissive content. The cost is extra flag buffers, a few flag-reduction reads per block, and cross-stage coupling that is disabled whenever user passes write bloom resources.

```diff
diff --git a/soc_real_time_renderer_amd/csrc/bloom.hip b/soc_real_time_renderer_amd/csrc/bloom.hip
--- a/soc_real_time_renderer_amd/csrc/bloom.hip
+++ b/soc_real_time_renderer_amd/csrc/bloom.hip
@@ -297,9 +297,8 @@
     return up ? launch_bloom_up(a, b, hs(stream), 1) : launch_bloom_down(a, b, hs(stream), 1);
 }
 
-extern "C" int soc_bloom_weighted_stage(const soc_globals* g, soc_img emissive, const soc_img* mips, int32_t mip_count,
-                                        soc_img output, int32_t stage, soc_stream stream) {
-    (void)g;
+int soc::bloom_weighted_stage(soc_img emissive, const soc_img* mips, int32_t mip_count, soc_img output, int32_t stage,
+                              soc_stream stream, const BloomFlags* flags) {
     static const char* P = "soc_bloom_weighted_stage";
     if (!mips) return set_error(SOC_E_INVALID_ARG, "%s: null mips", P);
     if (stage < 0 || stage > 4) return set_error(SOC_E_INVALID_ARG, "%s: stage %d not in 0..4", P, stage);
@@ -311,7 +310,13 @@
         return set_error(SOC_E_UNSUPPORTED, "%s: needs 4 mips halving exactly from the emissive extent (<= 8192)", P);
     if ((stage == 0 || stage == 4) && output.data == mips[1].data)
         return set_error(SOC_E_INVALID_ARG, "%s: output aliases mip 1", P);
-    return launch_bloom_weighted(emissive, mips, output, hs(stream), stage);
+    return launch_bloom_weighted(emissive, mips, output, hs(stream), stage, flags);
+}
+
+extern "C" int soc_bloom_weighted_stage(const soc_globals* g, soc_img emissive, const soc_img* mips, int32_t mip_count,
+                                        soc_img output, int32_t stage, soc_stream stream) {
+    (void)g;
+    return soc::bloom_weighted_stage(emissive, mips, mip_count, output, stage, stream, nullptr);
 }
 
 extern "C" int soc_bloom_chain(const soc_globals* g, soc_img emissive, const soc_img* mips, int32_t mip_count,
diff --git a/soc_real_time_renderer_amd/csrc/bloom_w.hip b/soc_real_time_renderer_amd/csrc/bloom_w.hip
--- a/soc_real_time_renderer_amd/csrc/bloom_w.hip
+++ b/soc_real_time_renderer_amd/csrc/bloom_w.hip
@@ -90,14 +90,6 @@
         }
 }
 
-template <int MODE>
-struct W1 {
-    static constexpr int OW = MODE ? 30 : 32, OH = MODE == 2 ? 16 : 8;
-    static constexpr int MW = 2 * OW + 4, MH = 2 * OH + 4;
-    static constexpr int EW = MW + 4, EH = MH + 4;
-    static constexpr int RUN = MH / 4;
-    static_assert(!MODE || (MW == 64 && MH % 4 == 0), "down11_runs: 64 columns x 2 row parities x 2 runs");
-};
 
 template <int TW, int MW, int RUN>
 __device__ __forceinline__ void down11_runs(const uint2 (*t)[TW], uint2 (*mt)[MW], int c, int r, int cx) {
@@ -161,7 +153,7 @@
 }
 
 template <int MODE, bool ZS>
-__global__ __launch_bounds__(kWorkgroup) void bloomw_down01p(DImg E, DImg M1, int ntx, int nty) {
+__global__ __launch_bounds__(kWorkgroup) void bloomw_down01p(DImg E, DImg M1, int ntx, int nty, uint32_t* F1) {
     constexpr int W1_OW = W1<MODE>::OW, W1_OH = W1<MODE>::OH, W1_MW = W1<MODE>::MW, W1_MH = W1<MODE>::MH,
                   W1_EW = W1<MODE>::EW, W1_EH = W1<MODE>::EH, RUN = W1<MODE>::RUN;
     static_assert(kWorkgroup == 256, "four waves: one vote word each");
@@ -183,6 +175,7 @@
         const int ty = id / ntx;
         X0 = (id - ty * ntx) * W1_OW;
         Y0 = ty * W1_OH;
+        return id;
     };
     uint2 v[KR];
     auto fetch = [&](int t) {
@@ -218,10 +211,11 @@
         __syncthreads();
         if (t + G < n) fetch(t + G);
         int X0, Y0;
-        tile_origin(t, X0, Y0);
+        const int id = tile_origin(t, X0, Y0);
         if constexpr (ZS) {
             const bool zero = voted(slot);
             slot ^= 1;
+            if (F1 && tid == 0) F1[id] = zero ? 1u : 0u;
             if (zero) {
                 if constexpr (MODE == 2) {
                     if (tid < W1_OW * W1_OH / 2) {
@@ -268,9 +262,6 @@
     }
 }
 
-constexpr int W2_OW = 16, W2_OH = 8;
-constexpr int W2_MW = 2 * W2_OW + 4, W2_MH = 2 * W2_OH + 4;
-constexpr int W2_SW = 2 * W2_MW + 4, W2_SH = 2 * W2_MH + 4;
 
 template <int TW, int MW, int K>
 __device__ __forceinline__ void down21_runs(const uint2 (*t)[TW], uint2 (*mt)[MW], int c, int r0, int n, int sc) {
@@ -300,7 +291,7 @@
 }
 
 template <bool REG>
-__global__ __launch_bounds__(kWorkgroup) void bloomw_down23(DImg S1, DImg M3, int W2, int H2, int swz) {
+__global__ __launch_bounds__(kWorkgroup) void bloomw_down23(DImg S1, DImg M3, int W2, int H2, int swz, ZeroFlags zf) {
     __shared__ uint2 st[W2_SH][W2_SW];
     __shared__ uint2 mt[W2_MH][W2_MW];
     const int tid = threadIdx.x;
@@ -309,6 +300,10 @@
     const int X0 = tbx * W2_OW, Y0 = tby * W2_OH;
     const int mx0 = 2 * X0 - 2, my0 = 2 * Y0 - 2, sx0 = 2 * mx0 - 2, sy0 = 2 * my0 - 2;
     load_tile<W2_SW, W2_SH>(S1, sx0, sy0, st, tid);
+    if (zf.f1 && tid < 64) {
+        const bool zero = rect_zero(zf.f1, tile_count(S1.w, zf.f1w), w2_f1_rect(tbx, tby, S1.w, S1.h, zf.f1w, zf.f1h));
+        if (tid == 0) zf.f2[tby * tile_count(M3.w, W2_OW) + tbx] = zero ? 1u : 0u;
+    }
     __syncthreads();
     constexpr int K = 3, NR = (W2_MH + K - 1) / K;
     static_assert(W2_MW * NR <= 256, "one run per lane");
@@ -332,9 +327,6 @@
     }
 }
 
-constexpr int U_OW = 64, U_OH = 16;
-constexpr int W3_MW = U_OW / 2 + 4, W3_MH = U_OH / 2 + 4;
-constexpr int W3_SW = W3_MW / 2 + 4, W3_SH = W3_MH / 2 + 4;
 
 template <int SW, int MW>
 __device__ __forceinline__ void up12_into(const uint2 (*s)[SW], int sx0, int sy0, uint2 (*m)[MW], int c, int r, int qx, int qy,
@@ -358,7 +350,12 @@
     }
 }
 
-__global__ __launch_bounds__(kWorkgroup) void bloomw_up32(DImg S3, DImg M1, int W2, int H2, bool vec, int swz) {
+__device__ __forceinline__ void up32_pass_flags(const ZeroFlags& zf, const DImg& S3, const DImg& M1, int tbx, int tby, int tid) {
+    const bool zero = rect_zero(zf.f2, tile_count(S3.w, W2_OW), w3_f2_rect(tbx, tby, S3.w, S3.h));
+    if (tid == 0) zf.f3[tby * tile_count(M1.w, U_OW) + tbx] = zero ? 1u : 0u;
+}
+
+__global__ __launch_bounds__(kWorkgroup) void bloomw_up32(DImg S3, DImg M1, int W2, int H2, bool vec, int swz, ZeroFlags zf) {
     __shared__ uint2 st[W3_SH][W3_SW];
     __shared__ uint2 mt[W3_MH][W3_MW];
     const int tid = threadIdx.x;
@@ -368,6 +365,7 @@
     const int mx0 = X0 / 2 - 2, my0 = Y0 / 2 - 2;
     const int sx0 = mx0 / 2 - 2, sy0 = my0 / 2 - 2;
     load_tile<W3_SW, W3_SH>(S3, sx0, sy0, st, tid);
+    if (zf.f2 && tid < 64) up32_pass_flags(zf, S3, M1, tbx, tby, tid);
     __syncthreads();
     for (int i = tid; i < (W3_MW / 2) * W3_MH; i += 256) {
         const int r = i / (W3_MW / 2), c = 2 * (i - r * (W3_MW / 2));
@@ -389,7 +387,7 @@
     float r[W3_MH][U_OW], g[W3_MH][U_OW], b[W3_MH][U_OW];
 };
 template <bool RUNS>
-__global__ __launch_bounds__(kWorkgroup) void bloomw_up32s(DImg S3, DImg M1, int W2, int H2, bool vec, int swz) {
+__global__ __launch_bounds__(kWorkgroup) void bloomw_up32s(DImg S3, DImg M1, int W2, int H2, bool vec, int swz, ZeroFlags zf) {
     __shared__ uint2 st[W3_SH][W3_SW];
     __shared__ uint2 mt[W3_MH][W3_MW];
     __shared__ P3u hp;
@@ -400,6 +398,7 @@
     const int mx0 = X0 / 2 - 2, my0 = Y0 / 2 - 2;
     const int sx0 = mx0 / 2 - 2, sy0 = my0 / 2 - 2;
     load_tile<W3_SW, W3_SH>(S3, sx0, sy0, st, tid);
+    if (zf.f2 && tid < 64) up32_pass_flags(zf, S3, M1, tbx, tby, tid);
     __syncthreads();
     for (int i = tid; i < W3_SH * W3_MW; i += 256) {
         const int sr = i / W3_MW, c = i - sr * W3_MW;
@@ -523,13 +522,15 @@
     }
 }
 
-__global__ __launch_bounds__(kWorkgroup) void bloomw_up10s(DImg S1, DImg O, bool vec, int swz, bool zs) {
+__global__ __launch_bounds__(kWorkgroup) void bloomw_up10s(DImg S1, DImg O, bool vec, int swz, bool zs, const uint32_t* __restrict__ F3) {
     __shared__ Up10Tile<U_OW, U_OH> t;
     const int tid = threadIdx.x;
     int tbx, tby;
     xcd_order(swz, tbx, tby);
     const int X0 = tbx * U_OW, Y0 = tby * U_OH;
-    const bool zero = t.build(S1, X0, Y0, O.w, O.h, tid, zs);
+    static_assert(Up10Geom<U_OW, U_OH>::SW <= U_OW + 1 && Up10Geom<U_OW, U_OH>::SH <= U_OH + 1, "at most 2 x 2 F3 tiles");
+    const bool flagged = F3 && rect2x2_zero(F3, tile_count(S1.w, U_OW), up10_f3_rect<U_OW, U_OH>(X0, Y0, S1.w, S1.h));
+    const bool zero = t.build(S1, X0, Y0, O.w, O.h, tid, zs, flagged);
     const uint2 zpx = pack3(C3{0.0f, 0.0f, 0.0f});
     for (int i = tid; i < (U_OW / 2) * U_OH; i += 256) {
         const int r = i / (U_OW / 2), pc = i - r * (U_OW / 2);
@@ -545,10 +546,6 @@
     }
 }
 
-#ifndef SOC_BLOOM_UP10_ROWS
-#define SOC_BLOOM_UP10_ROWS 16
-#endif
-constexpr int R_OW = 62, R_TH = SOC_BLOOM_UP10_ROWS;
 __device__ __forceinline__ uint32_t up_from_left(uint32_t v) {
     return (uint32_t)__builtin_amdgcn_update_dpp(0, (int)v, 0x138, 0xf, 0xf, false);
 }
@@ -556,13 +553,22 @@
     return (uint32_t)__builtin_amdgcn_update_dpp(0, (int)v, 0x130, 0xf, 0xf, false);
 }
 template <bool ZS>
-__global__ __launch_bounds__(kWorkgroup) void bloomw_up10r(DImg S1, DImg O, int nwx, int nwaves) {
+__global__ __launch_bounds__(kWorkgroup) void bloomw_up10r(DImg S1, DImg O, int nwx, int nwaves, const uint32_t* __restrict__ F3) {
     const int lane = (int)(threadIdx.x & 63);
-    const int wid = (int)blockIdx.x * (kWorkgroup / 64) + (int)(threadIdx.x >> 6);
+    const int wid = __builtin_amdgcn_readfirstlane((int)blockIdx.x * (kWorkgroup / 64) + (int)(threadIdx.x >> 6));
     if (wid >= nwaves) return;
     const int W0 = O.w, H0 = O.h, W1 = S1.w, H1 = S1.h;
     const int wx = wid % nwx, Y0 = (wid / nwx) * R_TH;
     const int x = wx * R_OW - 1 + lane;
+    if constexpr (ZS) {
+        static_assert(R_OW / 2 + 5 <= U_OW + 1 && R_TH / 2 + 7 <= U_OH + 1, "at most 2 x 2 F3 tiles");
+        if (F3 && rect2x2_zero(F3, tile_count(W1, U_OW), up10r_f3_rect(wx, Y0, W0, H0, W1, H1))) {
+            const uint2 zpx = pack3(C3{0.0f, 0.0f, 0.0f});
+            if (lane >= 1 && lane <= R_OW && x < W0)
+                for (int y = Y0; y < min(Y0 + R_TH, H0); ++y) row_ptr_w<uint2>(O, y)[x] = zpx;
+            return;
+        }
+    }
     const int cx = clampi(x, 0, W0 - 1);
     const int px = cx & 1, c0 = (cx >> 1) - 2 + px;
     int tc[4];
@@ -674,23 +680,40 @@
 
 }
 
-int launch_bloom_weighted(const soc_img& emissive, const soc_img* mips, const soc_img& output, hipStream_t s, int stage) {
+void bloom_flag_counts(const soc_img* mips, size_t count[3]) {
+    count[0] = (size_t)tile_count(mips[1].width, 30) * tile_count(mips[1].height, 8);
+    count[1] = (size_t)tile_count(mips[3].width, W2_OW) * tile_count(mips[3].height, W2_OH);
+    count[2] = (size_t)tile_count(mips[1].width, U_OW) * tile_count(mips[1].height, U_OH);
+}
+
+int launch_bloom_weighted(const soc_img& emissive, const soc_img* mips, const soc_img& output, hipStream_t s, int stage,
+                          const BloomFlags* flags) {
     const DImg E = dimg(emissive), M1 = dimg(mips[1]), M3 = dimg(mips[3]), O = dimg(output);
     const int swz = 1;
     const bool zero_skip = tuning_knob("SOC_BLOOM_ZERO_SKIP", 1) != 0;
+    ZeroFlags zf{nullptr, nullptr, nullptr, 0, 0};
+    const bool flagged = flags && flags->f1 && flags->f2 && flags->f3 && zero_skip;
+    const int w1_mode = flagged ? flags->w1_mode : stage <= 1 ? tuning_knob("SOC_BLOOM_W1_REG", 1) : 1;
+    if (flagged) {
+        zf.f1 = flags->f1;
+        zf.f2 = flags->f2;
+        zf.f3 = flags->f3;
+        zf.f1w = w1_mode == 2 ? W1<2>::OW : w1_mode == 1 ? W1<1>::OW : W1<0>::OW;
+        zf.f1h = w1_mode == 2 ? W1<2>::OH : w1_mode == 1 ? W1<1>::OH : W1<0>::OH;
+    }
     if (stage == 0 || stage == 1) {
         auto w1 = [&](auto mode, auto zs) {
             constexpr int R = decltype(mode)::value;
             constexpr bool Z = decltype(zs)::value;
             const int ntx = ceil_div(mips[1].width, W1<R>::OW), nty = ceil_div(mips[1].height, W1<R>::OH);
             const int grid = std::max(8, (std::min(ntx * nty, down01p_resident_set<R, Z>()) / 8) * 8);
-            launch("bloomw_down01p", kWorkgroup, bloomw_down01p<R, Z>, grid, kWorkgroup, 0, s, E, M1, ntx, nty);
+            launch("bloomw_down01p", kWorkgroup, bloomw_down01p<R, Z>, grid, kWorkgroup, 0, s, E, M1, ntx, nty, zf.f1);
         };
         auto w1z = [&](auto mode) {
             if (zero_skip) w1(mode, std::true_type{});
             else w1(mode, std::false_type{});
         };
-        const int mode = tuning_knob("SOC_BLOOM_W1_REG", 1);
+        const int mode = w1_mode;
         if (mode == 2) w1z(std::integral_constant<int, 2>{});
         else if (mode == 1) w1z(std::integral_constant<int, 1>{});
         else w1z(std::integral_constant<int, 0>{});
@@ -698,30 +721,30 @@
     if (stage == 0 || stage == 2) {
         dim3 g(ceil_div(mips[3].width, W2_OW), ceil_div(mips[3].height, W2_OH));
         if (tuning_knob("SOC_BLOOM_W2_REG", 1))
-            launch("bloomw_down23", kWorkgroup, bloomw_down23<true>, g, kWorkgroup, 0, s, M1, M3, mips[2].width, mips[2].height, swz);
+            launch("bloomw_down23", kWorkgroup, bloomw_down23<true>, g, kWorkgroup, 0, s, M1, M3, mips[2].width, mips[2].height, swz, zf);
         else
-            launch("bloomw_down23", kWorkgroup, bloomw_down23<false>, g, kWorkgroup, 0, s, M1, M3, mips[2].width, mips[2].height, swz);
+            launch("bloomw_down23", kWorkgroup, bloomw_down23<false>, g, kWorkgroup, 0, s, M1, M3, mips[2].width, mips[2].height, swz, zf);
     }
     if (stage == 0 || stage == 3) {
         dim3 g(ceil_div(mips[1].width, U_OW), ceil_div(mips[1].height, U_OH));
         if (tuning_knob("SOC_BLOOM_UP_SEP", 1))
             if (tuning_knob("SOC_BLOOM_W3_RUNS", 1))
-                launch("bloomw_up32s", kWorkgroup, bloomw_up32s<true>, g, kWorkgroup, 0, s, M3, M1, mips[2].width, mips[2].height, a16(mips[1]), swz);
+                launch("bloomw_up32s", kWorkgroup, bloomw_up32s<true>, g, kWorkgroup, 0, s, M3, M1, mips[2].width, mips[2].height, a16(mips[1]), swz, zf);
             else
-                launch("bloomw_up32s", kWorkgroup, bloomw_up32s<false>, g, kWorkgroup, 0, s, M3, M1, mips[2].width, mips[2].height, a16(mips[1]), swz);
+                launch("bloomw_up32s", kWorkgroup, bloomw_up32s<false>, g, kWorkgroup, 0, s, M3, M1, mips[2].width, mips[2].height, a16(mips[1]), swz, zf);
         else
-            launch("bloomw_up32", kWorkgroup, bloomw_up32, g, kWorkgroup, 0, s, M3, M1, mips[2].width, mips[2].height, a16(mips[1]), swz);
+            launch("bloomw_up32", kWorkgroup, bloomw_up32, g, kWorkgroup, 0, s, M3, M1, mips[2].width, mips[2].height, a16(mips[1]), swz, zf);
     }
     if (stage == 0 || stage == 4) {
         dim3 g(ceil_div(output.width, U_OW), ceil_div(output.height, U_OH));
         if (tuning_knob("SOC_BLOOM_UP10_REG", 1)) {
             const int nwx = ceil_div(output.width, R_OW), nwaves = nwx * ceil_div(output.height, R_TH);
             if (zero_skip)
-                launch("bloomw_up10r", kWorkgroup, bloomw_up10r<true>, ceil_div(nwaves, kWorkgroup / 64), kWorkgroup, 0, s, M1, O, nwx, nwaves);
+                launch("bloomw_up10r", kWorkgroup, bloomw_up10r<true>, ceil_div(nwaves, kWorkgroup / 64), kWorkgroup, 0, s, M1, O, nwx, nwaves, zf.f3);
             else
-                launch("bloomw_up10r", kWorkgroup, bloomw_up10r<false>, ceil_div(nwaves, kWorkgroup / 64), kWorkgroup, 0, s, M1, O, nwx, nwaves);
+                launch("bloomw_up10r", kWorkgroup, bloomw_up10r<false>, ceil_div(nwaves, kWorkgroup / 64), kWorkgroup, 0, s, M1, O, nwx, nwaves, zf.f3);
         } else if (tuning_knob("SOC_BLOOM_UP_SEP", 1))
-            launch("bloomw_up10s", kWorkgroup, bloomw_up10s, g, kWorkgroup, 0, s, M1, O, a16(output), swz, zero_skip);
+            launch("bloomw_up10s", kWorkgroup, bloomw_up10s, g, kWorkgroup, 0, s, M1, O, a16(output), swz, zero_skip, zf.f3);
         else
             launch("bloomw_up10", kWorkgroup, bloomw_up10, g, kWorkgroup, 0, s, M1, O, a16(output), swz);
     }
diff --git a/soc_real_time_renderer_amd/csrc/bloom_w.hpp b/soc_real_time_renderer_amd/csrc/bloom_w.hpp
--- a/soc_real_time_renderer_amd/csrc/bloom_w.hpp
+++ b/soc_real_time_renderer_amd/csrc/bloom_w.hpp
@@ -1,9 +1,95 @@
 #pragma once
 
+#include <stdint.h>
+
+#ifndef SOC_BLOOM_GEOMETRY_ONLY
 #include "soc_internal.hpp"
+#endif
+
+#if defined(__HIPCC__)
+#define SOC_HD __host__ __device__
+#else
+#define SOC_HD
+#endif
 
 namespace soc {
 namespace {
+
+template <int MODE>
+struct W1 {
+    static constexpr int OW = MODE ? 30 : 32, OH = MODE == 2 ? 16 : 8;
+    static constexpr int MW = 2 * OW + 4, MH = 2 * OH + 4;
+    static constexpr int EW = MW + 4, EH = MH + 4;
+    static constexpr int RUN = MH / 4;
+    static_assert(!MODE || (MW == 64 && MH % 4 == 0), "down11_runs: 64 columns x 2 row parities x 2 runs");
+};
+constexpr int W2_OW = 16, W2_OH = 8;
+constexpr int W2_MW = 2 * W2_OW + 4, W2_MH = 2 * W2_OH + 4;
+constexpr int W2_SW = 2 * W2_MW + 4, W2_SH = 2 * W2_MH + 4;
+constexpr int U_OW = 64, U_OH = 16;
+constexpr int W3_MW = U_OW / 2 + 4, W3_MH = U_OH / 2 + 4;
+constexpr int W3_SW = W3_MW / 2 + 4, W3_SH = W3_MH / 2 + 4;
+#ifndef SOC_BLOOM_UP10_ROWS
+#define SOC_BLOOM_UP10_ROWS 16
+#endif
+constexpr int R_OW = 62, R_TH = SOC_BLOOM_UP10_ROWS;
+template <int OW, int OH>
+struct Up10Geom {
+    static constexpr int MW = OW + 2, MH = OH + 2;
+    static constexpr int SW = OW / 2 + 6, SH = OH / 2 + 6;
+};
+
+struct TileRect {
+    int x0, y0, x1, y1;
+    constexpr SOC_HD int w() const { return x1 - x0 + 1; }
+    constexpr SOC_HD int count() const { return (x1 - x0 + 1) * (y1 - y0 + 1); }
+};
+constexpr SOC_HD int geo_clamp(int v, int lo, int hi) { return v < lo ? lo : v > hi ? hi : v; }
+constexpr SOC_HD int tile_count(int extent, int tile) { return (extent + tile - 1) / tile; }
+constexpr SOC_HD TileRect tiles_of(int tx, int ty, int tw, int th, int W, int H, int PW, int PH) {
+    return TileRect{geo_clamp(tx, 0, W - 1) / PW, geo_clamp(ty, 0, H - 1) / PH, geo_clamp(tx + tw - 1, 0, W - 1) / PW,
+                    geo_clamp(ty + th - 1, 0, H - 1) / PH};
+}
+constexpr SOC_HD TileRect w2_f1_rect(int tbx, int tby, int Wm1, int Hm1, int pw, int ph) {
+    return tiles_of(2 * (2 * tbx * W2_OW - 2) - 2, 2 * (2 * tby * W2_OH - 2) - 2, W2_SW, W2_SH, Wm1, Hm1, pw, ph);
+}
+constexpr SOC_HD TileRect w3_f2_rect(int tbx, int tby, int Wm3, int Hm3) {
+    return tiles_of((tbx * U_OW / 2 - 2) / 2 - 2, (tby * U_OH / 2 - 2) / 2 - 2, W3_SW, W3_SH, Wm3, Hm3, W2_OW, W2_OH);
+}
+template <int OW, int OH>
+constexpr SOC_HD TileRect up10_f3_rect(int X0, int Y0, int Wm1, int Hm1) {
+    return tiles_of(X0 / 2 - 3, Y0 / 2 - 3, Up10Geom<OW, OH>::SW, Up10Geom<OW, OH>::SH, Wm1, Hm1, U_OW, U_OH);
+}
+constexpr SOC_HD TileRect up10r_f3_rect(int wx, int Y0, int W0, int H0, int Wm1, int Hm1) {
+    const int xa = geo_clamp(wx * R_OW - 1, 0, W0 - 1), xb = geo_clamp(wx * R_OW + R_OW, 0, W0 - 1);
+    const int c0 = (xa >> 1) - 2 + (xa & 1), c1 = (xb >> 1) + 1 + (xb & 1);
+    const int ya = Y0 - 1 > 0 ? Y0 - 1 : 0, yb = Y0 + R_TH < H0 - 1 ? Y0 + R_TH : H0 - 1;
+    const int r0 = (ya >> 1) - 2, r1 = (yb >> 1) + 3;
+    return tiles_of(c0, r0, c1 - c0 + 1, r1 - r0 + 1, Wm1, Hm1, U_OW, U_OH);
+}
+
+#ifndef SOC_BLOOM_GEOMETRY_ONLY
+
+struct ZeroFlags {
+    uint32_t *f1, *f2, *f3;
+    int f1w, f1h;
+};
+__device__ __forceinline__ uint32_t rect_entry(const uint32_t* __restrict__ F, int nx, const TileRect& r, int i) {
+    if (i >= r.count()) return 1u;
+    const int ry = i / r.w();
+    return F[(r.y0 + ry) * nx + r.x0 + (i - ry * r.w())];
+}
+__device__ __forceinline__ bool rect_zero(const uint32_t* __restrict__ F, int nx, const TileRect& r) {
+    const int lane = (int)(threadIdx.x & 63u), n = r.count();
+    bool all = true;
+    for (int i0 = 0; i0 < n; i0 += 64) all = (__ballot(rect_entry(F, nx, r, i0 + lane) != 1u) == 0ull) && all;
+    return all;
+}
+__device__ __forceinline__ bool rect2x2_zero(const uint32_t* __restrict__ F, int nx, const TileRect& r) {
+    const uint32_t* r0 = F + r.y0 * nx;
+    const uint32_t* r1 = F + r.y1 * nx;
+    return (r0[r.x0] & r0[r.x1] & r1[r.x0] & r1[r.x1]) == 1u;
+}
 
 __device__ __forceinline__ int clampi(int v, int lo, int hi) { return min(max(v, lo), hi); }
 
@@ -50,8 +136,8 @@
 
 template <int OW, int OH>
 struct Up10Tile {
-    static constexpr int MW = OW + 2, MH = OH + 2;
-    static constexpr int SW = OW / 2 + 6, SH = OH / 2 + 6;
+    static constexpr int MW = Up10Geom<OW, OH>::MW, MH = Up10Geom<OW, OH>::MH;
+    static constexpr int SW = Up10Geom<OW, OH>::SW, SH = Up10Geom<OW, OH>::SH;
     static constexpr int HR = SH > MH ? SH : MH;
     union {
         uint2 st[SH][SW];
@@ -60,7 +146,9 @@
     float hr[HR][MW], hg[HR][MW], hb[HR][MW];
     uint32_t zv[4];
 
-    __device__ __forceinline__ bool build(const DImg& S1, int X0, int Y0, int W0, int H0, int tid, bool zs) {
+    __device__ __forceinline__ bool build(const DImg& S1, int X0, int Y0, int W0, int H0, int tid, bool zs,
+                                          bool flagged = false) {
+        if (flagged) return true;
         const int mx0 = X0 - 1, my0 = Y0 - 1;
         const int sx0 = X0 / 2 - 3, sy0 = Y0 / 2 - 3;
         const uint32_t nz = load_tile<SW, SH>(S1, sx0, sy0, st, tid);
@@ -119,5 +207,7 @@
     }
 };
 
-}
-}
+#endif
+
+}
+}
diff --git a/soc_real_time_renderer_amd/csrc/capi.cpp b/soc_real_time_renderer_amd/csrc/capi.cpp
--- a/soc_real_time_renderer_amd/csrc/capi.cpp
+++ b/soc_real_time_renderer_amd/csrc/capi.cpp
@@ -628,6 +628,10 @@
     hipEvent_t probe_ev[16] = {};
     hipEvent_t switch_ev = nullptr;
     uint32_t* hist_scratch = nullptr;
+    uint32_t* bloom_flag_mem = nullptr;
+    size_t bloom_flag_words = 0;
+    size_t bloom_flag_n[3] = {0, 0, 0};
+    int bloom_w1_mode = 1;
     void* shadow_ws = nullptr;
     size_t shadow_ws_bytes = 0;
     bool fold_in_resolve = false;
@@ -687,6 +691,30 @@
     if (hipMemsetAsync(r->hist_scratch, 0, SOC_HISTOGRAM_SCRATCH_WORDS * sizeof(uint32_t), s) != hipSuccess)
         return set_error(SOC_E_HIP, "soc_renderer_execute: histogram scratch clear failed");
     return SOC_OK;
+}
+
+int ensure_bloom_flags(soc_renderer* r, hipStream_t s) {
+    const size_t need = r->bloom_flag_n[0] + r->bloom_flag_n[1] + r->bloom_flag_n[2];
+    if (!need || (r->bloom_flag_mem && r->bloom_flag_words >= need)) return SOC_OK;
+    if (r->bloom_flag_mem) {
+        (void)hipStreamSynchronize(s);
+        (void)hipFree(r->bloom_flag_mem);
+        r->bloom_flag_mem = nullptr;
+    }
+    if (hipMalloc((void**)&r->bloom_flag_mem, need * sizeof(uint32_t)) != hipSuccess) {
+        r->bloom_flag_mem = nullptr;
+        r->bloom_flag_words = 0;
+        return set_error(SOC_E_HIP, "soc_renderer_execute: bloom flag map allocation failed");
+    }
+    r->bloom_flag_words = need;
+    if (hipMemsetAsync(r->bloom_flag_mem, 0, need * sizeof(uint32_t), s) != hipSuccess)
+        return set_error(SOC_E_HIP, "soc_renderer_execute: bloom flag map clear failed");
+    return SOC_OK;
+}
+soc::BloomFlags bloom_flags(const soc_renderer* r) {
+    if (!r->bloom_flag_n[0] || !r->bloom_flag_mem) return soc::BloomFlags{nullptr, nullptr, nullptr, 1};
+    uint32_t* f1 = r->bloom_flag_mem;
+    return soc::BloomFlags{f1, f1 + r->bloom_flag_n[0], f1 + r->bloom_flag_n[0] + r->bloom_flag_n[1], r->bloom_w1_mode};
 }
 
 void build_raster_passes(soc_renderer* r) {
@@ -725,6 +753,7 @@
     const int mip[4] = {SOC_RES_BLOOM_MIP0, SOC_RES_BLOOM_MIP1, SOC_RES_BLOOM_MIP2, SOC_RES_BLOOM_MIP3};
     const bool chain_ok = bloom_fused_applicable(I.emissive, I.bloom_mips, nm, bloom_dst);
     r->bloom_in_comp = false;
+    r->bloom_flag_n[0] = r->bloom_flag_n[1] = r->bloom_flag_n[2] = 0;
     if (chain_ok && !(r->flags & (SOC_RENDERER_EXACT_BLOOM | SOC_RENDERER_UNFUSED_BLOOM))) {
         static const char* names[4] = {"BloomDownsample - 0+1", "BloomDownsample - 2+3", "BloomUpsample - 3+2",
                                        "BloomUpsample - 1+0"};
@@ -735,11 +764,17 @@
         gres.resolution[1] = I.color.height;
         r->bloom_in_comp = (r->flags & SOC_RENDERER_BLOOM_IN_COMPOSITION) && !(r->flags & SOC_RENDERER_UNFUSED_HISTOGRAM) &&
                            soc::composition_pair_applicable(&gres, I.color, I.albedo, bloom_dst, I.normal, I.depth, I.clouds);
+        if (tuning_knob("SOC_BLOOM_TILE_FLAGS", 1) != 0 && tuning_knob("SOC_BLOOM_ZERO_SKIP", 1) != 0) {
+            soc::bloom_flag_counts(I.bloom_mips, r->bloom_flag_n);
+            r->bloom_w1_mode = tuning_knob("SOC_BLOOM_W1_REG", 1);
+        }
         for (int st = 1; st <= 4; ++st)
             add_pass(r, names[st - 1], "Bloom", pre, rd[st - 1], wr[st - 1], [r, st](const soc_globals* g, hipStream_t s) {
                 if (st == 4 && bloom_in_comp_active(r)) return (int)SOC_OK;
                 const soc_img& dst = r->img.bloom_output.data ? r->img.bloom_output : r->img.emissive;
-                return soc_bloom_weighted_stage(g, r->img.emissive, r->img.bloom_mips, 4, dst, st, (soc_stream)s);
+                (void)g;
+                const soc::BloomFlags fl = bloom_flags(r);
+                return soc::bloom_weighted_stage(r->img.emissive, r->img.bloom_mips, 4, dst, st, (soc_stream)s, fl.f1 ? &fl : nullptr);
             });
         return;
     }
@@ -808,7 +843,8 @@
                                                                  I.ssao_blur, I.shadow, I.clouds, I.auto_exposure,
                                                                  r->hist_scratch, false, (soc_stream)s,
                                                                  r->sky_split_active,
-                                                                 bloom_in_comp_active(r) ? &I.bloom_mips[1] : nullptr);
+                                                                 bloom_in_comp_active(r) ? &I.bloom_mips[1] : nullptr,
+                                                                 bloom_flags(r).f3);
                  });
         auto& fold = add_pass(r, "LuminanceHistogramFold", "Auto Exposure", pre, parts,
                               res_mask({SOC_RES_AUTO_EXPOSURE}) | parts,
@@ -1005,6 +1041,11 @@
     build_passes(r);
     build_passes_tail(r);
     int rc = insert_user_passes(r);
+    const uint64_t bloom_res = res_mask({SOC_RES_EMISSIVE, SOC_RES_BLOOM_MIP0, SOC_RES_BLOOM_MIP1, SOC_RES_BLOOM_MIP2,
+                                         SOC_RES_BLOOM_MIP3, SOC_RES_BLOOM_OUTPUT});
+    for (const auto& up : r->user_passes)
+        if (desc_mask(up.desc.writes, up.desc.write_count) & bloom_res)
+            r->bloom_flag_n[0] = r->bloom_flag_n[1] = r->bloom_flag_n[2] = 0;
     derive_dependencies(r);
     derive_signals(r);
     return rc;
@@ -1048,6 +1089,7 @@
     if (r->staging) (void)hipHostFree(r->staging);
     destroy_side_lane(r);
     if (r->hist_scratch) (void)hipFree(r->hist_scratch);
+    if (r->bloom_flag_mem) (void)hipFree(r->bloom_flag_mem);
     if (r->shadow_ws) (void)hipFree(r->shadow_ws);
     delete r;
 }
@@ -1245,6 +1287,7 @@
             int rc = ensure_hist_scratch(r, s);
             if (rc) return rc;
         }
+        if (int rc = ensure_bloom_flags(r, s)) return rc;
     }
     if ((phase & SOC_PHASE_PRE_EXPOSURE) && (g->point_light_count || g->spot_light_count)) {
         int rc = upload_lights(r, g, s);
diff --git a/soc_real_time_renderer_amd/csrc/composition.hip b/soc_real_time_renderer_amd/csrc/composition.hip
--- a/soc_real_time_renderer_amd/csrc/composition.hip
+++ b/soc_real_time_renderer_amd/csrc/composition.hip
@@ -25,6 +25,7 @@
     int sky_external;
     float rw, rh;
     int bloom_zero_skip;
+    const uint32_t* __restrict__ f3;
 };
 
 __device__ __forceinline__ float fast_pow(float x, float y) {
@@ -213,6 +214,9 @@
     const int x = bx * 32 + (wave & 1) * 16 + (lane & 7) * 2;
     const int y = by * 16 + (wave >> 1) * 8 + (lane >> 3);
     const bool inside = x < target.w && y < target.h;
+    static_assert(Up10Geom<32, 16>::SW <= U_OW + 1 && Up10Geom<32, 16>::SH <= U_OH + 1, "at most 2 x 2 F3 tiles");
+    const bool bloom_zero =
+        p.f3 && rect2x2_zero(p.f3, tile_count(target.w / 2, U_OW), up10_f3_rect<32, 16>(bx * 32, by * 16, target.w / 2, target.h / 2));
     if (!HIST && !inside) return;
     uint2 outp[2] = {uint2{0u, 0u}, uint2{0u, 0u}};
     uint32_t own = 3u;
@@ -226,14 +230,19 @@
     if (inside) {
         d2 = __builtin_bit_cast(float2, __builtin_amdgcn_raw_buffer_load_b64(bd.r, buf_row(bd, y) + x * 4, 0, ld_aux));
         a4 = __builtin_bit_cast(uint4, __builtin_amdgcn_raw_buffer_load_b128(ba.r, buf_row(ba, y) + x * 8, 0, ld_aux));
-        if (!BL) e4 = __builtin_bit_cast(uint4, __builtin_amdgcn_raw_buffer_load_b128(be.r, buf_row(be, y) + x * 8, 0, ld_aux));
+        if (!BL && !bloom_zero)
+            e4 = __builtin_bit_cast(uint4, __builtin_amdgcn_raw_buffer_load_b128(be.r, buf_row(be, y) + x * 8, 0, ld_aux));
         n4 = __builtin_bit_cast(uint4, __builtin_amdgcn_raw_buffer_load_b128(bn.r, buf_row(bn, y) + x * 8, 0, ld_aux));
         if (NT & 4) sample_r8_pair(bo, centre_uv_rn(x, target.w, p.rw), centre_uv_rn(x + 1, target.w, p.rw), v, aop[0], aop[1]);
+    }
+    if (!BL && bloom_zero) {
+        const uint2 b0 = pack3(C3{0.0f, 0.0f, 0.0f});
+        e4 = uint4{b0.x, b0.y, b0.x, b0.y};
     }
     if constexpr (BL) {
         __shared__ Up10Tile<32, 16> bl;
         const int X0 = bx * 32, Y0 = by * 16;
-        if (bl.build(mip1, X0, Y0, target.w, target.h, threadIdx.x, p.bloom_zero_skip != 0)) {
+        if (bl.build(mip1, X0, Y0, target.w, target.h, threadIdx.x, p.bloom_zero_skip != 0, bloom_zero)) {
             const uint2 b0 = pack3(C3{0.0f, 0.0f, 0.0f});
             e4 = uint4{b0.x, b0.y, b0.x, b0.y};
         } else {
@@ -401,7 +410,7 @@
 int composition_launch(const soc_globals* g, const soc_globals* d_globals, soc_img target, soc_img albedo, soc_img emissive,
                        soc_img normal, soc_img depth, soc_img ssao, soc_img shadow, soc_img clouds, uint32_t* bins,
                        uint32_t* scratch, soc_stream stream, bool fold = true, bool sky_external = false,
-                       const soc_img* bloom_mip1 = nullptr) {
+                       const soc_img* bloom_mip1 = nullptr, const uint32_t* bloom_f3 = nullptr) {
     static const char* P = "soc_composition";
     if (!g) return set_error(SOC_E_INVALID_ARG, "%s: null globals", P);
     int rc = check_img(target, SOC_FMT_RGBA16F, P, "target");
@@ -442,6 +451,7 @@
     p.bloom_zero_skip = tuning_knob("SOC_BLOOM_ZERO_SKIP", 1) != 0;
     p.bins = nullptr;
     p.sky_external = 0;
+    p.f3 = nullptr;
     if ((p.npl || p.nsl) && !d_globals)
         return set_error(SOC_E_INVALID_ARG, "%s: frame has lights but no device globals (soc_upload_globals)", P);
 
@@ -459,6 +469,7 @@
             return set_error(SOC_E_SHAPE, "%s: the in-kernel bloom needs the fused histogram's pair path and mip1 = W/2 x H/2", P);
     }
     if (fast) {
+        if (bloom_f3 && H % 2 == 0 && p.bloom_zero_skip) p.f3 = bloom_f3;
         dim3 grd(ceil_div(W, 32), ceil_div(H, 16));
         const bool lights = (p.npl | p.nsl) != 0;
 #define SOC_COMP_PAIR(HI, LI) launch("composition_pair", kWorkgroup, composition_pair<HI, LI>, grd, kWorkgroup, 0, hs(stream), dimg(target), dimg(albedo), \
@@ -551,11 +562,12 @@
 int soc::composition_luminance_histogram(const soc_globals* g, const soc_globals* d_globals, soc_img target,
                                          soc_img albedo, soc_img emissive, soc_img normal, soc_img depth, soc_img ssao,
                                          soc_img shadow, soc_img clouds, soc_auto_exposure* ae, uint32_t* scratch,
-                                         bool fold, soc_stream stream, bool sky_external, const soc_img* bloom_mip1) {
+                                         bool fold, soc_stream stream, bool sky_external, const soc_img* bloom_mip1,
+                                         const uint32_t* bloom_f3) {
     if (!g || !ae || !scratch)
         return set_error(SOC_E_INVALID_ARG, "soc_composition_luminance_histogram: null globals / auto exposure / scratch");
     int rc = composition_launch(g, d_globals, target, albedo, emissive, normal, depth, ssao, shadow, clouds,
-                                ae->histogram_buckets, scratch, stream, fold, sky_external, bloom_mip1);
+                                ae->histogram_buckets, scratch, stream, fold, sky_external, bloom_mip1, bloom_f3);
     if (rc <= 0) return rc;
     if (bloom_mip1) return set_error(SOC_E_SHAPE, "composition: the in-kernel bloom needs the pair path");
     if (sky_external) return set_error(SOC_E_INVALID_ARG, "composition: sky_external needs the pair path");
diff --git a/soc_real_time_renderer_amd/csrc/soc_internal.hpp b/soc_real_time_renderer_amd/csrc/soc_internal.hpp
--- a/soc_real_time_renderer_amd/csrc/soc_internal.hpp
+++ b/soc_real_time_renderer_amd/csrc/soc_internal.hpp
@@ -65,12 +65,21 @@
 void mat4_mul_host(float out[16], const float a[16], const float b[16]);
 
 bool bloom_fused_applicable(const soc_img& emissive, const soc_img* mips, int mip_count, const soc_img& output);
-int launch_bloom_weighted(const soc_img& emissive, const soc_img* mips, const soc_img& output, hipStream_t s, int stage);
+struct BloomFlags {
+    uint32_t *f1, *f2, *f3;
+    int w1_mode;
+};
+int bloom_weighted_stage(soc_img emissive, const soc_img* mips, int32_t mip_count, soc_img output, int32_t stage,
+                         soc_stream stream, const BloomFlags* flags);
+void bloom_flag_counts(const soc_img* mips, size_t count[3]);
+int launch_bloom_weighted(const soc_img& emissive, const soc_img* mips, const soc_img& output, hipStream_t s, int stage,
+                          const BloomFlags* flags = nullptr);
 
 int composition_luminance_histogram(const soc_globals* g, const soc_globals* d_globals, soc_img target, soc_img albedo,
                                     soc_img emissive, soc_img normal, soc_img depth, soc_img ssao, soc_img shadow,
                                     soc_img clouds, soc_auto_exposure* ae, uint32_t* scratch, bool fold, soc_stream stream,
-                                    bool sky_external = false, const soc_img* bloom_mip1 = nullptr);
+                                    bool sky_external = false, const soc_img* bloom_mip1 = nullptr,
+                                    const uint32_t* bloom_f3 = nullptr);
 bool composition_pair_applicable(const soc_globals* g, const soc_img& target, const soc_img& albedo,
                                  const soc_img& emissive, const soc_img& normal, const soc_img& depth,
                                  const soc_img& clouds);
```

New measurement: 1970 (median of 6 runs). About the same (+0.6%).
